# marqo-ai/marqo

Hardware: AMD Instinct MI355X
Metric: embeddings/sec (higher is better)
Workload: dtype bf16; 1 GPU; open_clip ViT-B/32 image tower, uint8 224x224 resident in HBM (tower-only), batch 256/GPU; global_batch=256, parallelism=dp1 (replicated weights, sharded items, RCCL all_gather of embeddings), weights=random-init (seed 0) ViT-B-32, last_block_rows=pooled

## Files before the change

### include/marqo_hip.h

```cpp
#ifndef MARQO_HIP_H
#define MARQO_HIP_H

#include <stddef.h>
#include <stdint.h>

#ifdef __cplusplus
extern "C" {
#endif

#define MQ_OK 0
#define MQ_ERR_INVALID (-1)
#define MQ_ERR_HIP (-2)
#define MQ_ERR_WORKSPACE (-3)
#define MQ_ERR_UNSUPPORTED (-4)

#define MQ_ABI_VERSION 15

#define MQ_ACT_NONE 0
#define MQ_ACT_GELU 1
#define MQ_ACT_QUICKGELU 2
#define MQ_ACT_SILU 3
#define MQ_ACT_RELU 4

#define MQ_MASK_NONE 0
// ... 8 lines not shown

#define MQ_VIT_POOL_CLS 0
#define MQ_VIT_POOL_MAP 1
#define MQ_VIT_POOL_AVG 2
#define MQ_VIT_POOL_QUERY 3

#define MQ_EPI_BIAS 1
#define MQ_EPI_GELU 2
#define MQ_EPI_QUICKGELU 4
#define MQ_EPI_RESIDUAL 8
#define MQ_EPI_OUT_F32 16
#define MQ_EPI_OUT_FP8 32


typedef struct mq_block_weights {
    const float* ln1_g; const float* ln1_b;
    const void*  qkv_w; const float* qkv_b;
    const void*  out_w; const float* out_b;
    const float* ln2_g; const float* ln2_b;
    const void*  fc1_w; const float* fc1_b;
    const void*  fc2_w; const float* fc2_b;
    const void*  qkv_w8; const float* qkv_ws;
    const void*  out_w8; const float* out_ws;
    const void*  fc1_w8; const float* fc1_ws;
    const void*  fc2_w8; const float* fc2_ws;
    const void*  qkv_wf; const float* qkv_sf; const float* qkv_bf;
    const void*  fc1_wf; const float* fc1_sf; const float* fc1_bf;
    const float* attn_ln_g; const float* attn_ln_b;
    const float* mlp_ln_g;  const float* mlp_ln_b;
    const void*  out_wf; const float* out_sf; const float* out_bf;
    const void*  fc2_wf; const float* fc2_sf; const float* fc2_bf;
} mq_block_weights;

typedef struct mq_encoder_cfg {
    int32_t width;
    int32_t layers;
    int32_t heads;
    int32_t mlp_dim;
    int32_t act;
    int32_t post_ln;
    int32_t mask;
    float   ln_eps;
    int32_t precision;
    int32_t attn_width;
    int32_t fp8_first_layer;
    int32_t mlp_glu;
    const float* d_fp8_act_scale;
    float*       d_fp8_act_amax;
    const float* d_rope_inv_freq;
    const float* d_rel_bias;
    int32_t      rel_span;
    int32_t      residual_stream;
    int32_t      fp8_mlp_extra;
    int32_t      rope_prefix;
    const float* d_rope_table;
    int32_t      mlp_ln_dim;
    int32_t      reserved2;
} mq_encoder_cfg;


typedef struct mq_map_head {
    const float* q;
    const void*  kv_w;   const float* kv_b;
    const void*  proj_w; const float* proj_b;
    const float* ln_g;   const float* ln_b;
    const void*  fc1_w;  const float* fc1_b;
    const void*  fc2_w;  const float* fc2_b;
} mq_map_head;

typedef struct mq_vit_weights {
    const void*  patch_w;
    const float* cls;
    const float* pos;
    const float* ln_pre_g; const float* ln_pre_b;
    const mq_block_weights* blocks;
    const float* ln_post_g; const float* ln_post_b;
    const void*  proj_w;
    const mq_map_head* map;
    const float* proj_b;
} mq_vit_weights;

typedef struct mq_vit_cfg {
    mq_encoder_cfg enc;
    int32_t image_size;
    int32_t patch_size;
    int32_t out_dim;
    float mean[3];
    float std[3];
    int32_t pool;
    int32_t map_mlp_dim;
    int32_t pool_dim;
    int32_t pool_heads;
} mq_vit_cfg;

typedef struct mq_clip_text_weights {
    const float* tok_emb;
    const float* pos;
    const mq_block_weights* blocks;
    const float* ln_final_g; const float* ln_final_b;
    const void*  proj_w;
    const float* proj_b;
} mq_clip_text_weights;

typedef struct mq_clip_text_cfg {
    mq_encoder_cfg enc;
    int32_t vocab;
    int32_t ctx;
    int32_t out_dim;
    int32_t cls_pos;
} mq_clip_text_cfg;

typedef struct mq_bert_weights {
    const float* word_emb;
    const float* pos_emb;
    const float* type_emb;
    const float* emb_ln_g; const float* emb_ln_b;
    const mq_block_weights* blocks;
    const void*  proj1_w;
    const float* proj1_b;
    const void*  proj2_w;
} mq_bert_weights;

typedef struct mq_bert_cfg {
    mq_encoder_cfg enc;
    int32_t vocab;
    int32_t max_pos;
    int32_t pool;
    int32_t proj_hidden;
    int32_t out_dim;
} mq_bert_cfg;

int         mq_abi_version(void);
const char* mq_last_error(void);
const char* mq_build_arch(void);
int mq_check_device(int device);

int mq_host_gather(const void* const* h_src, const int64_t* h_bytes, const int64_t* h_dst_off, int64_t n, void* h_dst, int32_t threads);
int mq_host_gather_checked(const void* const* h_src, const int64_t* h_bytes, const int64_t* h_dst_off, int64_t n, void* h_dst,
                           int64_t dst_bytes, int32_t threads);

size_t mq_encoder_workspace_bytes(const mq_encoder_cfg* cfg, int64_t rows, int64_t nseq);
size_t mq_vit_workspace_bytes(const mq_vit_cfg* cfg, int64_t n_images);
size_t mq_clip_text_workspace_bytes(const mq_clip_text_cfg* cfg, int64_t rows, int64_t nseq);
size_t mq_bert_workspace_bytes(const mq_bert_cfg* cfg, int64_t rows, int64_t nseq);


int mq_encode_image_u8(const mq_vit_cfg* cfg, const mq_vit_weights* w,
                       const uint8_t* d_pixels, int64_t n, float* d_out, int normalize,
                       void* d_workspace, size_t workspace_bytes, void* stream);

int mq_encode_image_f32(const mq_vit_cfg* cfg, const mq_vit_weights* w,
                        const float* d_pixels, int64_t n, float* d_out, int normalize,
                        void* d_workspace, size_t workspace_bytes, void* stream);

int mq_encode_clip_text(const mq_clip_text_cfg* cfg, const mq_clip_text_weights* w,
                        const int32_t* d_ids, const int32_t* d_cu_seqlens,
                        const int32_t* h_cu_seqlens, int64_t nseq,
                        const int32_t* d_pool_rows,
                        float* d_out, int normalize,
                        void* d_workspace, size_t workspace_bytes, void* stream);

int mq_encode_bert(const mq_bert_cfg* cfg, const mq_bert_weights* w,
                   const int32_t* d_ids, const int32_t* d_cu_seqlens,
                   const int32_t* h_cu_seqlens, int64_t nseq,
                   float* d_out, int normalize,
                   void* d_workspace, size_t workspace_bytes, void* stream);


size_t mq_clip_resize_workspace_bytes(const int32_t* h_heights, const int32_t* h_widths, int64_t n, int32_t S);
int mq_clip_resize_crop_u8(const uint8_t* d_src, const int64_t* h_src_off, const int32_t* h_heights,
                           const int32_t* h_widths, int64_t n, int32_t S, uint8_t* d_out,
                           void* d_workspace, size_t workspace_bytes, void* stream);

size_t mq_resize_workspace_bytes(const int32_t* h_heights, const int32_t* h_widths, int64_t n, int32_t out_h, int32_t out_w);
int mq_resize_u8(const uint8_t* d_src, const int64_t* h_src_off, const int32_t* h_heights, const int32_t* h_widths,
                 int64_t n, int32_t out_h, int32_t out_w, uint8_t* d_out, void* d_workspace, size_t workspace_bytes,
                 void* stream);

size_t mq_resize_filter_workspace_bytes(const int32_t* h_heights, const int32_t* h_widths, int64_t n, int32_t out_h, int32_t out_w,
                                        int32_t filter);
int mq_resize_filter_u8(const uint8_t* d_src, const int64_t* h_src_off, const int32_t* h_heights, const int32_t* h_widths,
                        int64_t n, int32_t out_h, int32_t out_w, int32_t filter, uint8_t* d_out, void* d_workspace,
                        size_t workspace_bytes, void* stream);

int    mq_chunk_grid_count(int32_t hn, int32_t wn, int32_t overlap);
size_t mq_chunk_grid_workspace_bytes(const int32_t* h_heights, const int32_t* h_widths, int64_t n,
                                     int32_t hn, int32_t wn, int32_t overlap, int32_t S);
int mq_chunk_grid_u8(const uint8_t* d_src, const int64_t* h_src_off, const int32_t* h_heights,
                     const int32_t* h_widths, int64_t n, int32_t hn, int32_t wn, int32_t overlap, int32_t S,
                     uint8_t* d_out, float* h_boxes, void* d_workspace, size_t workspace_bytes, void* stream);

#define MQ_IMG_RGB 0
#define MQ_IMG_NEAREST 1
#define MQ_IMG_RGBA 2
size_t mq_resize_mode_workspace_bytes(const int32_t* h_heights, const int32_t* h_widths, int64_t n, int32_t out_h, int32_t out_w,
                                      int32_t filter, int32_t crop, int32_t mode);
int mq_resize_mode_u8(const uint8_t* d_src, const int64_t* h_src_off, const int32_t* h_heights, const int32_t* h_widths, int64_t n,
                      int32_t out_h, int32_t out_w, int32_t filter, int32_t crop, int32_t mode, uint8_t* d_out,
                      void* d_workspace, size_t workspace_bytes, void* stream);

int mq_unpack_rgbx(const uint8_t* d_staging, int64_t jobs_off, int64_t n, int64_t max_npix, uint8_t* d_rgb, void* stream);

int mq_to_tensor_normalize(const uint8_t* d_u8, float* d_out, int64_t n, int32_t S,
                           const float* mean, const float* std, void* stream);

int mq_resample_ksize(int32_t in_size, int32_t out_size);
int mq_resample_coeffs(int32_t in_size, int32_t out_size, int32_t first, int32_t count,
                       int32_t* h_bounds, int32_t* h_kk);


int mq_gemm_fp8(const void* d_A8, int64_t lda, const void* d_W8, int64_t ldw, const float* d_a_scale,
                int a_scale_per_row, const float* d_w_scale, const float* d_bias, const float* d_residual,
                void* d_out, int64_t ldc, const float* d_out_scale, float* d_amax,
                int64_t M, int64_t N, int64_t K, int flags, void* stream);

int mq_quantize_weights_fp8(const void* d_W_bf16, int64_t ldw, void* d_W8, int64_t ld8, float* d_scale,
                            int64_t N, int64_t K, void* stream);

int mq_layernorm_fp8(const float* d_x, const float* d_g, const float* d_b, void* d_out_fp8, float* d_row_scale,
                     float* d_out_f32 ,
                     int64_t rows, int32_t W, float eps, void* stream);

int mq_layernorm_fp8_ex(const void* d_x, int x_bf16, const float* d_g, const float* d_b, void* d_out_fp8, float* d_row_scale,
                        float* d_out_f32, int64_t rows, int32_t W, float eps, void* stream);

int mq_rowquant_fp8(const float* d_x, void* d_out_fp8, float* d_row_scale, int64_t rows, int32_t W, void* stream);

int mq_gemm_bf16(const void* d_A, int64_t lda, const void* d_W, int64_t ldw,
                 const float* d_bias, const float* d_residual, void* d_out, int64_t ldc,
                 int64_t M, int64_t N, int64_t K, int flags, void* stream);

int mq_gemm_small_bf16(const void* d_A, int64_t lda, const void* d_W, int64_t ldw, const float* d_bias, const void* d_residual,
                       void* d_out, int64_t ldc, int64_t M, int64_t N, int64_t K, int flags, void* stream);
int mq_ln_gemm_small_bf16(const void* d_x, int64_t ldx, int x_bf16, const float* d_ln_g, const float* d_ln_b, float eps, const void* d_W,
                          int64_t ldw, const float* d_bias, void* d_out, int64_t ldc, int64_t M, int64_t N, int64_t K, int flags,
                          float* d_ln_out, void* stream);

#define MQ_EPI_ROW_STATS 64
#define MQ_EPI_LN_APPLY 128
#define MQ_EPI_GLU 256
#define MQ_EPI_RELU 512
int mq_gemm_bf16_rs(const void* d_A, int64_t lda, const void* d_W, int64_t ldw, const float* d_bias, const void* d_residual, void* d_out, int64_t ldc,
                    int64_t M, int64_t N, int64_t K, int flags, float* d_partials, void* stream);
int mq_row_stats_finalize(const float* d_partials, int32_t nslots, float* d_stats, int64_t rows, int32_t W, float eps, void* stream);
int mq_gemm_bf16_lnrs(const void* d_A, int64_t lda, const void* d_W, int64_t ldw, const float* d_bias, const float* d_colsum, const float* d_rowstats,
                      const void* d_residual, void* d_out, int64_t ldc, int64_t M, int64_t N, int64_t K, int flags, float* d_partials, void* stream);
int mq_attention_stats(const void* d_qkv, void* d_out, const int32_t* d_cu_seqlens, int64_t nseq, int32_t fixed_len, int32_t max_len, int32_t W,
                       int32_t heads, int32_t mask, float* d_row_part, int64_t rows, void* stream);
int mq_attention_proj_ok(int64_t nseq, int32_t fixed_len, int32_t W, int32_t heads);
int mq_attention_proj(const void* d_qkv, const void* d_w, const float* d_bias, void* d_x, float* d_rowstats, int64_t nseq, int32_t fixed_len, int32_t W,
                      int32_t heads, float eps, const void* d_pf_a, size_t pf_a_bytes, const void* d_pf_b, size_t pf_b_bytes, void* stream);
int mq_panel_gemm_ln_ok(int64_t nseq, int32_t fixed_len, int64_t N, int64_t K);
int mq_panel_gemm_ln(const void* d_x, const void* d_W, const float* d_bias, const float* d_colsum, const float* d_rowstats, void* d_out, int64_t ldc,
                     int64_t nseq, int32_t fixed_len, int64_t N, int64_t K, int flags, void* stream);
int64_t mq_gemm_band_counters(int64_t M);
int mq_gemm_bf16_rsf(const void* d_A, int64_t lda, const void* d_W, int64_t ldw, const float* d_bias, const void* d_residual, void* d_out, int64_t ldc,
                     int64_t M, int64_t N, int64_t K, int flags, float* d_partials, float* d_stats, float eps, uint32_t* d_band_ctr,
                     const void* d_pf_a, size_t pf_a_bytes, const void* d_pf_b, size_t pf_b_bytes, void* stream);
int mq_row_stats(const void* d_x_bf16, float* d_stats, int64_t rows, int32_t W, float eps, void* stream);
int mq_gemm_bf16_ln(const void* d_A, int64_t lda, const void* d_W, int64_t ldw, const float* d_bias, const float* d_colsum, const float* d_rowstats,
                    void* d_out, int64_t ldc, int64_t M, int64_t N, int64_t K, int flags, void* stream);

int mq_layernorm(const float* d_x, const int32_t* d_row_idx, const float* d_g, const float* d_b,
                 void* d_out_bf16, float* d_out_f32, int64_t rows, int32_t W, float eps, void* stream);
int mq_layernorm_ex(const void* d_x, int x_bf16, const int32_t* d_row_idx, const float* d_g, const float* d_b,
                    void* d_out_bf16, float* d_out_f32, int64_t rows, int32_t W, float eps, void* stream);

int mq_attention(const void* d_qkv, void* d_out, const int32_t* d_cu_seqlens, int64_t nseq,
                 int32_t fixed_len, int32_t max_len, int32_t W, int32_t heads, int32_t mask,
                 void* stream);

int mq_attention_bias(const void* d_qkv, void* d_out, const int32_t* d_cu_seqlens, int64_t nseq, int32_t fixed_len,
                      int32_t max_len, int32_t W, int32_t heads, const float* d_rel_bias, int32_t rel_span, void* stream);

int mq_attention_ex(const void* d_qkv, void* d_out, const int32_t* d_cu_seqlens, int64_t nseq,
                    int32_t fixed_len, int32_t max_len, int32_t W, int32_t heads, int32_t mask,
                    int32_t out_fp8, const float* d_out_scale, float* d_amax, void* stream);

int mq_encoder_forward(const mq_encoder_cfg* cfg, const mq_block_weights* blocks,
                       float* d_x, int64_t rows, const int32_t* d_cu_seqlens, int64_t nseq,
                       int32_t fixed_len, int32_t max_len,
                       void* d_workspace, size_t workspace_bytes, void* stream);

int mq_encoder_forward_rows(const mq_encoder_cfg* cfg, const mq_block_weights* blocks,
                            float* d_x, int64_t rows, const int32_t* d_cu_seqlens, int64_t nseq,
                            int32_t fixed_len, int32_t max_len,
                            const int32_t* d_out_rows, int64_t n_out_rows,
                            void* d_workspace, size_t workspace_bytes, void* stream);

int mq_l2_normalize(const float* d_x, float* d_out, int64_t rows, int32_t D, void* stream);

int mq_patchify(const void* d_in, int32_t is_u8, void* d_out, int64_t n, int32_t S, int32_t P, int32_t Kp, const float* mean, const float* std,
                void* stream);
int mq_vit_assemble(const float* d_patch_out, const float* d_cls, const float* d_pos, const float* d_g, const float* d_b, void* d_x, int64_t n,
                    int32_t T, int32_t W, float eps, int32_t x_bf16, void* stream);
int mq_embed_tokens(const int32_t* d_ids, const int32_t* d_cu, int64_t nseq, const float* d_tok, const float* d_pos, const float* d_type0,
                    const float* d_g, const float* d_b, float* d_x, void* d_xb, int32_t W, int32_t vocab, float eps, int32_t last_pos, void* stream);
int mq_pool(const float* d_x, const int32_t* d_cu, int64_t nseq, float* d_out, int32_t W, int32_t pool, int32_t normalize, void* stream);
int mq_map_pool(const void* d_kv, const float* d_q, void* d_out, int64_t n, int32_t T, int32_t W, int32_t heads, void* stream);
int mq_avg_tokens(const void* d_x, int32_t x_bf16, float* d_out, int64_t n, int32_t T, int32_t first, int32_t W, void* stream);
int mq_move_rows(void* d_sparse, const int32_t* d_idx, void* d_dense, int64_t n, int64_t row_bytes, int32_t scatter, void* stream);
int mq_last_rows(const int32_t* d_cu, int32_t* d_rows, int64_t nseq, void* stream);
int mq_cls_rows(int32_t* d_rows, int64_t n, int32_t T, void* stream);
int mq_rope(void* d_qkv, const int32_t* d_cu, int64_t nseq, int32_t fixed_len, int32_t Wa, int32_t heads, const float* d_inv_freq, void* stream);
int mq_rope_table(void* d_qkv, int64_t rows, int32_t T, int32_t prefix, int32_t Wa, int32_t heads, const float* d_table, void* stream);
int mq_glu(void* d_buf, int64_t rows, int32_t F, int32_t act, int32_t interleaved, void* stream);
// ... 727 lines not shown
```

### marqo_amd/_lib.py

```python
from __future__ import annotations

import ctypes as C
import os
import re
import subprocess
import sys
import sysconfig
import threading
from typing import Optional
from pathlib import Path

PKG_DIR = Path(__file__).resolve().parent
CSRC_DIR = PKG_DIR / "csrc"
LIB_DIR = PKG_DIR / "lib"
LIB_PATH = Path(os.environ["MARQO_AMD_LIB"]) if os.environ.get("MARQO_AMD_LIB") else LIB_DIR / "libmarqo_hip.so"
HEADER_PATH = PKG_DIR.parent / "include" / "marqo_hip.h"
TORCH_OPS_SRC = CSRC_DIR / "torch_ops.cpp"
TORCH_OPS_PATH = LIB_DIR / "libmarqo_torch_ops.so"
STAGE_SRC = CSRC_DIR / "py_stage.cpp"
STAGE_PATH = LIB_DIR / "_mq_stage.so"

MQ_OK = 0
NO_SCRATCH_UNITS = ("rowops", "gemm_bf16", "gemm_wd", "gemm_fp8", "gemm_small", "attention", "attention_window", "attention_gqa", "attention_gqa256", "attention_gqa256_causal", "attention_relbias", "attention_alibi", "attention_disentangled", "attention_full", "lora", "attn_proj", "panel_gemm", "embed", "convnext", "resnet", "patch_attn", "rerank", "owl_head", "temporal", "audio", "video")
ABI_VERSION = 15
MQ_PREC_BF16, MQ_PREC_FP8 = 0, 1
MQ_ACT_GELU, MQ_ACT_QUICKGELU, MQ_ACT_SILU, MQ_ACT_RELU = 1, 2, 3, 4
MQ_MASK_NONE, MQ_MASK_CAUSAL, MQ_MASK_CAUSAL_CLS = 0, 1, 2
MQ_POOL_MEAN, MQ_POOL_CLS, MQ_POOL_LAST = 0, 1, 2
MQ_VIT_POOL_CLS, MQ_VIT_POOL_MAP, MQ_VIT_POOL_AVG, MQ_VIT_POOL_QUERY = 0, 1, 2, 3
MQ_EPI_BIAS, MQ_EPI_GELU, MQ_EPI_QUICKGELU, MQ_EPI_RESIDUAL, MQ_EPI_OUT_F32, MQ_EPI_OUT_FP8 = 1, 2, 4, 8, 16, 32
MQ_EPI_ROW_STATS, MQ_EPI_LN_APPLY = 64, 128
MQ_COMBINE_RAW, MQ_COMBINE_NORMALIZE, MQ_COMBINE_NORMALIZE_IF_NONZERO = 0, 1, 2
MQ_IMG_RGB, MQ_IMG_NEAREST, MQ_IMG_RGBA = 0, 1, 2
MQ_PROF_FAMILIES = 6
MQ_FBANK_WS_BYTES = 2048
MQ_RESAMPLE_MAX_TAPS = 1 << 21
PROF_FAMILY_NAMES = ("gemm", "layernorm", "attention", "embed", "pool_head", "preprocess")


class MarqoHipUnavailableError(RuntimeError):
    """The HIP extension is missing / unloadable.  There is deliberately no fallback."""


class MarqoHipError(RuntimeError):
    """A libmarqo_hip entry point returned an error code."""


class BlockWeights(C.Structure):
    _fields_ = [(n, C.c_void_p) for n in (
        "ln1_g", "ln1_b", "qkv_w", "qkv_b", "out_w", "out_b",
        "ln2_g", "ln2_b", "fc1_w", "fc1_b", "fc2_w", "fc2_b",
        "qkv_w8", "qkv_ws", "out_w8", "out_ws", "fc1_w8", "fc1_ws", "fc2_w8", "fc2_ws",
        "qkv_wf", "qkv_sf", "qkv_bf", "fc1_wf", "fc1_sf", "fc1_bf",
        "attn_ln_g", "attn_ln_b", "mlp_ln_g", "mlp_ln_b",
        "out_wf", "out_sf", "out_bf", "fc2_wf", "fc2_sf", "fc2_bf")]


class EncoderCfg(C.Structure):
    _fields_ = [("width", C.c_int32), ("layers", C.c_int32), ("heads", C.c_int32), ("mlp_dim", C.c_int32),
                ("act", C.c_int32), ("post_ln", C.c_int32), ("mask", C.c_int32), ("ln_eps", C.c_float),
                ("precision", C.c_int32), ("attn_width", C.c_int32), ("fp8_first_layer", C.c_int32), ("mlp_glu", C.c_int32),
                ("d_fp8_act_scale", C.c_void_p), ("d_fp8_act_amax", C.c_void_p), ("d_rope_inv_freq", C.c_void_p),
                ("d_rel_bias", C.c_void_p), ("rel_span", C.c_int32), ("residual_stream", C.c_int32),
                ("fp8_mlp_extra", C.c_int32), ("rope_prefix", C.c_int32), ("d_rope_table", C.c_void_p), ("mlp_ln_dim", C.c_int32),
                ("reserved2", C.c_int32)]


class MapHead(C.Structure):
    _fields_ = [("q", C.c_void_p), ("kv_w", C.c_void_p), ("kv_b", C.c_void_p), ("proj_w", C.c_void_p), ("proj_b", C.c_void_p),
                ("ln_g", C.c_void_p), ("ln_b", C.c_void_p), ("fc1_w", C.c_void_p), ("fc1_b", C.c_void_p),
                ("fc2_w", C.c_void_p), ("fc2_b", C.c_void_p)]


class VitWeights(C.Structure):
    _fields_ = [("patch_w", C.c_void_p), ("cls", C.c_void_p), ("pos", C.c_void_p),
                ("ln_pre_g", C.c_void_p), ("ln_pre_b", C.c_void_p), ("blocks", C.POINTER(BlockWeights)),
                ("ln_post_g", C.c_void_p), ("ln_post_b", C.c_void_p), ("proj_w", C.c_void_p), ("map", C.POINTER(MapHead)),
                ("proj_b", C.c_void_p)]


class VitCfg(C.Structure):
    _fields_ = [("enc", EncoderCfg), ("image_size", C.c_int32), ("patch_size", C.c_int32), ("out_dim", C.c_int32),
                ("mean", C.c_float * 3), ("std", C.c_float * 3), ("pool", C.c_int32), ("map_mlp_dim", C.c_int32), ("pool_dim", C.c_int32),
                ("pool_heads", C.c_int32)]


class ClipTextWeights(C.Structure):
    _fields_ = [("tok_emb", C.c_void_p), ("pos", C.c_void_p), ("blocks", C.POINTER(BlockWeights)),
                ("ln_final_g", C.c_void_p), ("ln_final_b", C.c_void_p), ("proj_w", C.c_void_p), ("proj_b", C.c_void_p)]


class ClipTextCfg(C.Structure):
    _fields_ = [("enc", EncoderCfg), ("vocab", C.c_int32), ("ctx", C.c_int32), ("out_dim", C.c_int32), ("cls_pos", C.c_int32)]


class BertWeights(C.Structure):
    _fields_ = [("word_emb", C.c_void_p), ("pos_emb", C.c_void_p), ("type_emb", C.c_void_p),
                ("emb_ln_g", C.c_void_p), ("emb_ln_b", C.c_void_p), ("blocks", C.POINTER(BlockWeights)),
                ("proj1_w", C.c_void_p), ("proj1_b", C.c_void_p), ("proj2_w", C.c_void_p)]


class BertCfg(C.Structure):
    _fields_ = [("enc", EncoderCfg), ("vocab", C.c_int32), ("max_pos", C.c_int32), ("pool", C.c_int32),
                ("proj_hidden", C.c_int32), ("out_dim", C.c_int32)]


class ConvNextCfg(C.Structure):
    _fields_ = [("image_size", C.c_int32), ("depths", C.c_int32 * 4), ("dims", C.c_int32 * 4), ("ln_eps", C.c_float), ("head", C.c_int32),
                ("out_dim", C.c_int32), ("mean", C.c_float * 3), ("std", C.c_float * 3)]


class ConvNextBlockWeights(C.Structure):
    _fields_ = [(n, C.c_void_p) for n in ("dw_w", "dw_b", "fc1_w", "fc1_b", "fc1_s", "fc2_w", "fc2_b")]


class ConvNextWeights(C.Structure):
    _fields_ = [("stem_w", C.c_void_p), ("stem_b", C.c_void_p), ("stem_ln_g", C.c_void_p), ("stem_ln_b", C.c_void_p),
                ("ds_ln_g", C.c_void_p * 4), ("ds_ln_b", C.c_void_p * 4), ("ds_w", C.c_void_p * 4), ("ds_b", C.c_void_p * 4),
                ("blocks", C.POINTER(ConvNextBlockWeights)), ("head_ln_g", C.c_void_p), ("head_ln_b", C.c_void_p),
                ("proj_w", C.c_void_p), ("proj_b", C.c_void_p), ("proj2_w", C.c_void_p), ("proj2_b", C.c_void_p)]


MQ_CONVNEXT_HEAD_LINEAR, MQ_CONVNEXT_HEAD_MLP = 0, 1
MQ_EPI_RELU = 512


class ResNetCfg(C.Structure):
    _fields_ = [("image_size", C.c_int32), ("layers", C.c_int32 * 4), ("width", C.c_int32), ("heads", C.c_int32), ("out_dim", C.c_int32),
                ("mean", C.c_float * 3), ("std", C.c_float * 3)]


class ResNetBlockWeights(C.Structure):
    _fields_ = [(n, C.c_void_p) for n in ("conv1_w", "conv1_b", "conv2_w", "conv2_b", "conv3_w", "conv3_b", "ds_w", "ds_b")]


class ResNetWeights(C.Structure):
    _fields_ = [("stem_w", C.c_void_p * 3), ("stem_b", C.c_void_p * 3), ("blocks", C.POINTER(ResNetBlockWeights)), ("pos", C.c_void_p),
                ("q_w", C.c_void_p), ("q_b", C.c_void_p), ("kv_w", C.c_void_p), ("kv_b", C.c_void_p), ("c_w", C.c_void_p), ("c_b", C.c_void_p)]


class WordPieceVocab(C.Structure):
    _fields_ = [("d_slots", C.c_void_p), ("d_pool", C.c_void_p), ("n_slots", C.c_uint32), ("unk_id", C.c_int32), ("cls_id", C.c_int32),
                ("sep_id", C.c_int32), ("pad_id", C.c_int32), ("lower", C.c_int32), ("max_word_chars", C.c_int32), ("d_unicode", C.c_void_p)]


class ClipBpeVocab(C.Structure):
    _fields_ = [("d_slots", C.c_void_p), ("d_byte_id", C.c_void_p), ("d_byte_end_id", C.c_void_p), ("n_slots", C.c_uint32),
                ("sot_id", C.c_int32), ("eot_id", C.c_int32), ("lower", C.c_int32), ("d_unicode", C.c_void_p)]


class ByteBpeVocab(C.Structure):
    _fields_ = [("d_slots", C.c_void_p), ("d_byte_id", C.c_void_p), ("d_unicode", C.c_void_p), ("n_slots", C.c_uint32), ("cls_id", C.c_int32),
                ("sep_id", C.c_int32), ("pad_id", C.c_int32)]


class SentencePieceVocab(C.Structure):
    _fields_ = [("d_slots", C.c_void_p), ("d_pool", C.c_void_p), ("d_score", C.c_void_p), ("d_nmap", C.c_void_p), ("d_npool", C.c_void_p),
                ("d_ccc", C.c_void_p), ("n_slots", C.c_uint32), ("unk_id", C.c_int32), ("unk_score", C.c_float), ("add_dummy_prefix", C.c_int32),
                ("remove_extra_ws", C.c_int32), ("max_piece_bytes", C.c_int32), ("prefix_id", C.c_int32), ("suffix_id", C.c_int32),
                ("pad_id", C.c_int32), ("id_offset", C.c_int32), ("unk_out", C.c_int32)]


class QueueCfg(C.Structure):
    _fields_ = [("kind", C.c_int32), ("device", C.c_int32), ("max_seqs", C.c_int32), ("max_rows", C.c_int32), ("normalize", C.c_int32),
                ("depth", C.c_int32), ("window_us", C.c_int32), ("graphs", C.c_int32), ("helper_seqs", C.c_int32), ("reserved", C.c_int32)]


class QueueStats(C.Structure):
    _fields_ = [("requests", C.c_uint64), ("calls", C.c_uint64), ("merged_calls", C.c_uint64), ("failed_calls", C.c_uint64),
                ("sequences", C.c_uint64), ("rows", C.c_uint64), ("max_call_sequences", C.c_uint64), ("graphs", C.c_uint64), ("graph_replays", C.c_uint64)]


QUEUE_CLIP_TEXT, QUEUE_BERT, QUEUE_IMAGE_F32 = 0, 1, 2


class ScoreHeadWeights(C.Structure):
# ... 6 lines not shown


class ModernBertWeights(C.Structure):
    _fields_ = [("tok_emb", C.c_void_p), ("emb_ln_g", C.c_void_p), ("final_ln_g", C.c_void_p), ("zeros", C.c_void_p), ("d_inv_freq_global", C.c_void_p),
                ("d_inv_freq_local", C.c_void_p), ("layers", C.POINTER(ModernBertLayer))]


class ModernBertCfg(C.Structure):
    _fields_ = [("width", C.c_int32), ("layers", C.c_int32), ("heads", C.c_int32), ("mlp_dim", C.c_int32), ("vocab", C.c_int32), ("max_pos", C.c_int32),
                ("half_window", C.c_int32), ("pool", C.c_int32), ("ln_eps", C.c_float), ("reserved", C.c_int32)]


class ScoreHeadLnWeights(C.Structure):
    _fields_ = [("dense_w", C.c_void_p), ("dense_b", C.c_void_p), ("norm_g", C.c_void_p), ("norm_b", C.c_void_p), ("cls_w", C.c_void_p),
                ("cls_b", C.c_float), ("ln_eps", C.c_float)]


class QwenLayer(C.Structure):
    _fields_ = [(n, C.c_void_p) for n in ("input_norm_g", "qkv_w", "qkv_b", "q_norm_g", "k_norm_g", "out_w", "post_norm_g", "ug_w", "down_w")]


class QwenWeights(C.Structure):
    _fields_ = [("tok_emb", C.c_void_p), ("final_norm_g", C.c_void_p), ("zeros", C.c_void_p), ("d_inv_freq", C.c_void_p), ("layers", C.POINTER(QwenLayer))]


class QwenCfg(C.Structure):
    _fields_ = [("width", C.c_int32), ("layers", C.c_int32), ("q_heads", C.c_int32), ("kv_heads", C.c_int32), ("head_dim", C.c_int32), ("mlp_dim", C.c_int32),
                ("vocab", C.c_int32), ("max_pos", C.c_int32), ("pool", C.c_int32), ("rms_eps", C.c_float)]


class GemmaLayer(C.Structure):
    _fields_ = [(n, C.c_void_p) for n in ("input_norm_g", "qkv_w", "q_norm_g", "k_norm_g", "out_w", "post_attn_norm_g", "pre_ffn_norm_g", "ug_w", "down_w",
                                          "post_ffn_norm_g")] + [("sliding", C.c_int32), ("reserved", C.c_int32)]


class GemmaWeights(C.Structure):
    _fields_ = [("tok_emb", C.c_void_p), ("final_norm_g", C.c_void_p), ("d_inv_freq_global", C.c_void_p), ("d_inv_freq_local", C.c_void_p),
                ("layers", C.POINTER(GemmaLayer))]


class GemmaCfg(C.Structure):
    _fields_ = [("width", C.c_int32), ("layers", C.c_int32), ("q_heads", C.c_int32), ("kv_heads", C.c_int32), ("head_dim", C.c_int32), ("mlp_dim", C.c_int32),
                ("vocab", C.c_int32), ("max_pos", C.c_int32), ("half_window", C.c_int32), ("pool", C.c_int32), ("rms_eps", C.c_float), ("attn_scale", C.c_float)]


class GemmaCausalLayer(C.Structure):
    _fields_ = [(n, C.c_void_p) for n in ("input_norm_g", "qkv_w", "out_w", "post_norm_g", "ug_w", "down_w")]


class GemmaCausalWeights(C.Structure):
    _fields_ = [("tok_emb", C.c_void_p), ("final_norm_g", C.c_void_p), ("zeros", C.c_void_p), ("d_inv_freq", C.c_void_p),
                ("layers", C.POINTER(GemmaCausalLayer))]


class GemmaCausalCfg(C.Structure):
    _fields_ = [("width", C.c_int32), ("layers", C.c_int32), ("q_heads", C.c_int32), ("kv_heads", C.c_int32), ("head_dim", C.c_int32), ("mlp_dim", C.c_int32),
                ("vocab", C.c_int32), ("max_pos", C.c_int32), ("rms_eps", C.c_float), ("attn_scale", C.c_float)]


class T5Layer(C.Structure):
    _fields_ = [(n, C.c_void_p) for n in ("attn_norm_g", "qkv_w", "out_w", "ff_norm_g", "wi_w", "wo_w")]


class T5Weights(C.Structure):
    _fields_ = [("tok_emb", C.c_void_p), ("final_norm_g", C.c_void_p), ("zeros", C.c_void_p), ("d_rel_bias", C.c_void_p), ("layers", C.POINTER(T5Layer))]


class T5Cfg(C.Structure):
    _fields_ = [("width", C.c_int32), ("layers", C.c_int32), ("heads", C.c_int32), ("head_dim", C.c_int32), ("mlp_dim", C.c_int32), ("vocab", C.c_int32),
                ("max_pos", C.c_int32), ("pool", C.c_int32), ("max_distance", C.c_int32), ("gated", C.c_int32), ("rms_eps", C.c_float), ("reserved", C.c_int32)]


class JinaBertLayer(C.Structure):
    _fields_ = [(n, C.c_void_p) for n in ("qkv_w", "qkv_b", "out_w", "out_b", "attn_ln_g", "attn_ln_b", "wg_w", "wo_w", "wo_b", "mlp_ln_g", "mlp_ln_b")]


class JinaBertWeights(C.Structure):
    _fields_ = [("tok_emb", C.c_void_p), ("type0", C.c_void_p), ("emb_ln_g", C.c_void_p), ("emb_ln_b", C.c_void_p), ("d_slopes", C.c_void_p),
                ("layers", C.POINTER(JinaBertLayer))]


class JinaBertCfg(C.Structure):
    _fields_ = [("width", C.c_int32), ("layers", C.c_int32), ("heads", C.c_int32), ("head_dim", C.c_int32), ("mlp_dim", C.c_int32), ("vocab", C.c_int32),
                ("max_pos", C.c_int32), ("pool", C.c_int32), ("ln_eps", C.c_float), ("reserved", C.c_int32)]


class DebertaLayer(C.Structure):
    _fields_ = [(n, C.c_void_p) for n in ("qkv_w", "qkv_b", "out_w", "out_b", "attn_ln_g", "attn_ln_b", "fc1_w", "fc1_b", "fc2_w", "fc2_b", "mlp_ln_g",
                                          "mlp_ln_b", "pos_key", "pos_query")]


class DebertaWeights(C.Structure):
    _fields_ = [("tok_emb", C.c_void_p), ("emb_ln_g", C.c_void_p), ("emb_ln_b", C.c_void_p), ("d_idx", C.c_void_p), ("h_idx", C.c_void_p),
                ("layers", C.POINTER(DebertaLayer))]


class DebertaCfg(C.Structure):
    _fields_ = [("width", C.c_int32), ("layers", C.c_int32), ("heads", C.c_int32), ("head_dim", C.c_int32), ("mlp_dim", C.c_int32), ("vocab", C.c_int32),
                ("max_pos", C.c_int32), ("pool", C.c_int32), ("span", C.c_int32), ("reach", C.c_int32), ("ln_eps", C.c_float), ("reserved", C.c_int32)]


class NomicBertLayer(C.Structure):
    _fields_ = [(n, C.c_void_p) for n in ("qkv_w", "out_w", "attn_ln_g", "attn_ln_b", "ug_w", "down_w", "mlp_ln_g", "mlp_ln_b")]


class NomicBertWeights(C.Structure):
    _fields_ = [("tok_emb", C.c_void_p), ("type0", C.c_void_p), ("emb_ln_g", C.c_void_p), ("emb_ln_b", C.c_void_p), ("zeros", C.c_void_p),
                ("d_inv_freq", C.c_void_p), ("layers", C.POINTER(NomicBertLayer))]


class NomicBertCfg(C.Structure):
    _fields_ = [("width", C.c_int32), ("layers", C.c_int32), ("heads", C.c_int32), ("head_dim", C.c_int32), ("mlp_dim", C.c_int32), ("vocab", C.c_int32),
                ("max_pos", C.c_int32), ("pool", C.c_int32), ("ln_eps", C.c_float), ("reserved", C.c_int32)]


MQ_LORA_ACCUM, MQ_LORA_WRITE, MQ_LORA_INPLACE = 0, 1, 2


class JinaV3Layer(C.Structure):
    _fields_ = [(n, C.c_void_p) for n in ("qkv_w", "qkv_b", "out_w", "out_b", "attn_ln_g", "attn_ln_b", "fc1_w", "fc1_b", "fc2_w", "fc2_b", "mlp_ln_g",
                                          "mlp_ln_b")]


class JinaV3Weights(C.Structure):
    _fields_ = [("tok_emb", C.c_void_p), ("type0", C.c_void_p), ("emb_ln_g", C.c_void_p), ("emb_ln_b", C.c_void_p), ("d_inv_freq", C.c_void_p),
                ("layers", C.POINTER(JinaV3Layer))]


class JinaV3LoraLayer(C.Structure):
    _fields_ = [(n, C.c_void_p) for n in ("qkv_a", "qkv_b", "out_a", "out_b", "fc1_a", "fc1_b", "fc2_a", "fc2_b")]


class JinaV3Lora(C.Structure):
    _fields_ = [("tasks", C.c_int32), ("rank", C.c_int32), ("d_scale", C.c_void_p), ("emb_a", C.c_void_p), ("emb_b", C.c_void_p),
                ("layers", C.POINTER(JinaV3LoraLayer))]


class JinaV3Cfg(C.Structure):
    _fields_ = [("width", C.c_int32), ("layers", C.c_int32), ("heads", C.c_int32), ("head_dim", C.c_int32), ("mlp_dim", C.c_int32), ("vocab", C.c_int32),
                ("max_pos", C.c_int32), ("pool", C.c_int32), ("ln_eps", C.c_float), ("reserved", C.c_int32)]


_P = C.c_void_p
_SIGNATURES = {
    "mq_abi_version": (C.c_int, []),
    "mq_last_error": (C.c_char_p, []),
    "mq_build_arch": (C.c_char_p, []),
    "mq_encoder_workspace_bytes": (C.c_size_t, [C.POINTER(EncoderCfg), C.c_int64, C.c_int64]),
    "mq_vit_workspace_bytes": (C.c_size_t, [C.POINTER(VitCfg), C.c_int64]),
    "mq_clip_text_workspace_bytes": (C.c_size_t, [C.POINTER(ClipTextCfg), C.c_int64, C.c_int64]),
    "mq_bert_workspace_bytes": (C.c_size_t, [C.POINTER(BertCfg), C.c_int64, C.c_int64]),
    "mq_encode_image_u8": (C.c_int, [C.POINTER(VitCfg), C.POINTER(VitWeights), _P, C.c_int64, _P, C.c_int, _P, C.c_size_t, _P]),
    "mq_encode_image_f32": (C.c_int, [C.POINTER(VitCfg), C.POINTER(VitWeights), _P, C.c_int64, _P, C.c_int, _P, C.c_size_t, _P]),
    "mq_encode_clip_text": (C.c_int, [C.POINTER(ClipTextCfg), C.POINTER(ClipTextWeights), _P, _P, _P, C.c_int64, _P, _P,
                                      C.c_int, _P, C.c_size_t, _P]),
    "mq_encode_bert": (C.c_int, [C.POINTER(BertCfg), C.POINTER(BertWeights), _P, _P, _P, C.c_int64, _P, C.c_int, _P,
                                 C.c_size_t, _P]),
    "mq_gemm_bf16": (C.c_int, [_P, C.c_int64, _P, C.c_int64, _P, _P, _P, C.c_int64, C.c_int64, C.c_int64, C.c_int64,
                               C.c_int, _P]),
    "mq_gemm_small_bf16": (C.c_int, [_P, C.c_int64, _P, C.c_int64, _P, _P, _P, C.c_int64, C.c_int64, C.c_int64, C.c_int64, C.c_int, _P]),
    "mq_ln_gemm_small_bf16": (C.c_int, [_P, C.c_int64, C.c_int, _P, _P, C.c_float, _P, C.c_int64, _P, _P, C.c_int64, C.c_int64, C.c_int64,
                                        C.c_int64, C.c_int, _P, _P]),
    "mq_gemm_bf16_ln": (C.c_int, [_P, C.c_int64, _P, C.c_int64, _P, _P, _P, _P, C.c_int64, C.c_int64, C.c_int64, C.c_int64, C.c_int, _P]),
    "mq_row_stats": (C.c_int, [_P, _P, C.c_int64, C.c_int32, C.c_float, _P]),
    "mq_row_stats_finalize": (C.c_int, [_P, C.c_int32, _P, C.c_int64, C.c_int32, C.c_float, _P]),
    "mq_gemm_bf16_lnrs": (C.c_int, [_P, C.c_int64, _P, C.c_int64, _P, _P, _P, _P, _P, C.c_int64, C.c_int64, C.c_int64, C.c_int64, C.c_int, _P, _P]),
    "mq_attention_stats": (C.c_int, [_P, _P, _P, C.c_int64, C.c_int32, C.c_int32, C.c_int32, C.c_int32, C.c_int32, _P, C.c_int64, _P]),
    "mq_attention_proj_ok": (C.c_int, [C.c_int64, C.c_int32, C.c_int32, C.c_int32]),
    "mq_panel_gemm_ln_ok": (C.c_int, [C.c_int64, C.c_int32, C.c_int64, C.c_int64]),
    "mq_panel_gemm_ln": (C.c_int, [_P, _P, _P, _P, _P, _P, C.c_int64, C.c_int64, C.c_int32, C.c_int64, C.c_int64, C.c_int, _P]),
    "mq_attention_proj": (C.c_int, [_P, _P, _P, _P, _P, C.c_int64, C.c_int32, C.c_int32, C.c_int32, C.c_float, _P, C.c_size_t, _P, C.c_size_t, _P]),
    "mq_gemm_bf16_rs": (C.c_int, [_P, C.c_int64, _P, C.c_int64, _P, _P, _P, C.c_int64, C.c_int64, C.c_int64, C.c_int64, C.c_int, _P, _P]),
    "mq_check_device": (C.c_int, [C.c_int]),
    "mq_gemm_band_counters": (C.c_int64, [C.c_int64]),
    "mq_gemm_bf16_rsf": (C.c_int, [_P, C.c_int64, _P, C.c_int64, _P, _P, _P, C.c_int64, C.c_int64, C.c_int64, C.c_int64, C.c_int, _P, _P, C.c_float, _P,
                                   _P, C.c_size_t, _P, C.c_size_t, _P]),
    "mq_gemm_fp8": (C.c_int, [_P, C.c_int64, _P, C.c_int64, _P, C.c_int, _P, _P, _P, _P, C.c_int64, _P, _P, C.c_int64, C.c_int64,
                              C.c_int64, C.c_int, _P]),
    "mq_quantize_weights_fp8": (C.c_int, [_P, C.c_int64, _P, C.c_int64, _P, C.c_int64, C.c_int64, _P]),
    "mq_layernorm_fp8": (C.c_int, [_P, _P, _P, _P, _P, _P, C.c_int64, C.c_int32, C.c_float, _P]),
    "mq_layernorm_fp8_ex": (C.c_int, [_P, C.c_int, _P, _P, _P, _P, _P, C.c_int64, C.c_int32, C.c_float, _P]),
    "mq_rowquant_fp8": (C.c_int, [_P, _P, _P, C.c_int64, C.c_int32, _P]),
    "mq_layernorm": (C.c_int, [_P, _P, _P, _P, _P, _P, C.c_int64, C.c_int32, C.c_float, _P]),
    "mq_layernorm_ex": (C.c_int, [_P, C.c_int, _P, _P, _P, _P, _P, C.c_int64, C.c_int32, C.c_float, _P]),
    "mq_attention_ex": (C.c_int, [_P, _P, _P, C.c_int64, C.c_int32, C.c_int32, C.c_int32, C.c_int32, C.c_int32, C.c_int32, _P, _P, _P]),
    "mq_attention_bias": (C.c_int, [_P, _P, _P, C.c_int64, C.c_int32, C.c_int32, C.c_int32, C.c_int32, _P, C.c_int32, _P]),
    "mq_attention": (C.c_int, [_P, _P, _P, C.c_int64, C.c_int32, C.c_int32, C.c_int32, C.c_int32, C.c_int32, _P]),
    "mq_encoder_forward": (C.c_int, [C.POINTER(EncoderCfg), C.POINTER(BlockWeights), _P, C.c_int64, _P, C.c_int64,
                                     C.c_int32, C.c_int32, _P, C.c_size_t, _P]),
    "mq_encoder_forward_rows": (C.c_int, [C.POINTER(EncoderCfg), C.POINTER(BlockWeights), _P, C.c_int64, _P, C.c_int64,
                                          C.c_int32, C.c_int32, _P, C.c_int64, _P, C.c_size_t, _P]),
    "mq_l2_normalize": (C.c_int, [_P, _P, C.c_int64, C.c_int32, _P]),
    "mq_clip_resize_workspace_bytes": (C.c_size_t, [_P, _P, C.c_int64, C.c_int32]),
    "mq_clip_resize_crop_u8": (C.c_int, [_P, _P, _P, _P, C.c_int64, C.c_int32, _P, _P, C.c_size_t, _P]),
    "mq_resize_workspace_bytes": (C.c_size_t, [_P, _P, C.c_int64, C.c_int32, C.c_int32]),
    "mq_resize_u8": (C.c_int, [_P, _P, _P, _P, C.c_int64, C.c_int32, C.c_int32, _P, _P, C.c_size_t, _P]),
    "mq_resize_filter_workspace_bytes": (C.c_size_t, [_P, _P, C.c_int64, C.c_int32, C.c_int32, C.c_int32]),
    "mq_resize_filter_u8": (C.c_int, [_P, _P, _P, _P, C.c_int64, C.c_int32, C.c_int32, C.c_int32, _P, _P, C.c_size_t, _P]),
    "mq_resize_mode_workspace_bytes": (C.c_size_t, [_P, _P, C.c_int64, C.c_int32, C.c_int32, C.c_int32, C.c_int32, C.c_int32]),
    "mq_resize_mode_u8": (C.c_int, [_P, _P, _P, _P, C.c_int64, C.c_int32, C.c_int32, C.c_int32, C.c_int32, C.c_int32, _P, _P, C.c_size_t, _P]),
    "mq_chunk_grid_count": (C.c_int, [C.c_int32, C.c_int32, C.c_int32]),
    "mq_chunk_grid_workspace_bytes": (C.c_size_t, [_P, _P, C.c_int64, C.c_int32, C.c_int32, C.c_int32, C.c_int32]),
    "mq_chunk_grid_u8": (C.c_int, [_P, _P, _P, _P, C.c_int64, C.c_int32, C.c_int32, C.c_int32, C.c_int32, _P, _P, _P,
                                   C.c_size_t, _P]),
    "mq_host_gather": (C.c_int, [_P, _P, _P, C.c_int64, _P, C.c_int32]),
    "mq_host_gather_checked": (C.c_int, [_P, _P, _P, C.c_int64, _P, C.c_int64, C.c_int32]),
    "mq_unpack_rgbx": (C.c_int, [_P, C.c_int64, C.c_int64, C.c_int64, _P, _P]),
    "mq_to_tensor_normalize": (C.c_int, [_P, _P, C.c_int64, C.c_int32, C.POINTER(C.c_float), C.POINTER(C.c_float), _P]),
    "mq_resample_ksize": (C.c_int, [C.c_int32, C.c_int32]),
    "mq_resample_coeffs": (C.c_int, [C.c_int32, C.c_int32, C.c_int32, C.c_int32, _P, _P]),
    "mq_tokenize_workspace_bytes": (C.c_size_t, [C.c_int64, C.c_int64, C.c_int32]),
    "mq_tokenize_wordpiece": (C.c_int, [C.POINTER(WordPieceVocab), _P, _P, C.c_int64, C.c_int64, C.c_int32, _P, C.c_int64, _P, _P, _P,
                                        C.c_size_t, _P]),
    "mq_tokenize_clip_bpe": (C.c_int, [C.POINTER(ClipBpeVocab), _P, _P, C.c_int64, C.c_int64, C.c_int32, _P, _P, _P, _P, C.c_size_t, _P]),
    "mq_tokenize_byte_bpe": (C.c_int, [C.POINTER(ByteBpeVocab), _P, _P, C.c_int64, C.c_int64, C.c_int32, _P, C.c_int64, _P, _P, _P, C.c_size_t, _P]),
    "mq_tokenize_sentencepiece_workspace_bytes": (C.c_size_t, [C.c_int64, C.c_int64, C.c_int32]),
    "mq_tokenize_sentencepiece": (C.c_int, [C.POINTER(SentencePieceVocab), _P, _P, C.c_int64, C.c_int64, C.c_int32, _P, C.c_int64, _P, _P, _P,
                                            C.c_size_t, _P]),
    "mq_tokenize_sentencepiece_bpe": (C.c_int, [C.POINTER(SentencePieceVocab), _P, _P, C.c_int64, C.c_int64, C.c_int32, _P, C.c_int64, _P, _P, _P,
                                                C.c_size_t, _P]),
    "mq_pack_ids": (C.c_int, [_P, C.c_int64, _P, C.c_int64, _P, _P]),
    "mq_weighted_combine": (C.c_int, [_P, C.c_int64, _P, _P, _P, C.c_int64, C.c_int32, C.c_int32, _P, _P]),
    "mq_queue_create": (C.c_int, [C.POINTER(QueueCfg), _P, _P, C.POINTER(_P)]),
    "mq_queue_encode": (C.c_int, [_P, _P, _P, C.c_int64, _P]),
    "mq_queue_encode_images": (C.c_int, [_P, _P, C.c_int64, _P]),
    "mq_queue_get_stats": (C.c_int, [_P, C.POINTER(QueueStats)]),
    "mq_queue_destroy": (C.c_int, [_P]),
    "mq_convnext_workspace_bytes": (C.c_size_t, [C.POINTER(ConvNextCfg), C.c_int64]),
    "mq_encode_convnext_u8": (C.c_int, [C.POINTER(ConvNextCfg), C.POINTER(ConvNextWeights), _P, C.c_int64, _P, C.c_int, _P, C.c_size_t, _P]),
    "mq_encode_convnext_f32": (C.c_int, [C.POINTER(ConvNextCfg), C.POINTER(ConvNextWeights), _P, C.c_int64, _P, C.c_int, _P, C.c_size_t, _P]),
    "mq_convnext_dwconv": (C.c_int, [_P, _P, _P, _P, _P, C.c_int64, C.c_int32, C.c_int32, C.c_int32, _P]),
    "mq_convnext_downsample": (C.c_int, [_P, _P, _P, _P, _P, C.c_int64, C.c_int32, C.c_int32, C.c_int32, _P]),
    "mq_convnext_pool_ln": (C.c_int, [_P, _P, _P, _P, _P, C.c_int64, C.c_int32, C.c_int32, C.c_float, _P]),
    "mq_resnet_workspace_bytes": (C.c_size_t, [C.POINTER(ResNetCfg), C.c_int64]),
    "mq_encode_resnet_u8": (C.c_int, [C.POINTER(ResNetCfg), C.POINTER(ResNetWeights), _P, C.c_int64, _P, C.c_int, _P, C.c_size_t, _P]),
    "mq_encode_resnet_f32": (C.c_int, [C.POINTER(ResNetCfg), C.POINTER(ResNetWeights), _P, C.c_int64, _P, C.c_int, _P, C.c_size_t, _P]),
    "mq_resnet_conv3x3": (C.c_int, [_P, _P, _P, _P, C.c_int64, C.c_int64, C.c_int32, C.c_int32, C.c_int32, C.c_int32, C.c_int32, _P]),
    "mq_resnet_stem_gather": (C.c_int, [_P, C.c_int32, _P, C.c_int64, C.c_int32, _P, _P, _P]),
    "mq_resnet_avgpool2": (C.c_int, [_P, _P, C.c_int64, C.c_int32, C.c_int32, C.c_int32, _P]),
    "mq_resnet_attnpool_tokens": (C.c_int, [_P, _P, _P, C.c_int64, C.c_int32, C.c_int32, _P]),
    "mq_resnet_attnpool_attend": (C.c_int, [_P, _P, _P, C.c_int64, C.c_int32, C.c_int32, _P]),
    "mq_attention_cls_probs": (C.c_int, [_P, _P, C.c_int64, C.c_int32, C.c_int32, C.c_int32, _P]),
    "mq_attn_boxes": (C.c_int, [_P, C.c_int64, C.c_int32, C.c_int32, C.c_int32, _P, _P, C.c_int32, _P]),
    "mq_patchify": (C.c_int, [_P, C.c_int32, _P, C.c_int64, C.c_int32, C.c_int32, C.c_int32, _P, _P, _P]),
    "mq_vit_assemble": (C.c_int, [_P, _P, _P, _P, _P, _P, C.c_int64, C.c_int32, C.c_int32, C.c_float, C.c_int32, _P]),
    "mq_embed_tokens": (C.c_int, [_P, _P, C.c_int64, _P, _P, _P, _P, _P, _P, _P, C.c_int32, C.c_int32, C.c_float, C.c_int32, _P]),
    "mq_pool": (C.c_int, [_P, _P, C.c_int64, _P, C.c_int32, C.c_int32, C.c_int32, _P]),
    "mq_map_pool": (C.c_int, [_P, _P, _P, C.c_int64, C.c_int32, C.c_int32, C.c_int32, _P]),
    "mq_avg_tokens": (C.c_int, [_P, C.c_int32, _P, C.c_int64, C.c_int32, C.c_int32, C.c_int32, _P]),
    "mq_move_rows": (C.c_int, [_P, _P, _P, C.c_int64, C.c_int64, C.c_int32, _P]),
    "mq_last_rows": (C.c_int, [_P, _P, C.c_int64, _P]),
    "mq_cls_rows": (C.c_int, [_P, C.c_int64, C.c_int32, _P]),
    "mq_rope": (C.c_int, [_P, _P, C.c_int64, C.c_int32, C.c_int32, C.c_int32, _P, _P]),
    "mq_rope_table": (C.c_int, [_P, C.c_int64, C.c_int32, C.c_int32, C.c_int32, C.c_int32, _P, _P]),
    "mq_glu": (C.c_int, [_P, C.c_int64, C.c_int32, C.c_int32, C.c_int32, _P]),
    "mq_glu_ln": (C.c_int, [_P, C.c_int64, C.c_int32, C.c_int32, C.c_int32, _P, _P, C.c_float, C.c_int32, _P]),
    "mq_pair_plan": (C.c_int, [C.c_int32, _P, C.c_int64, C.c_int32, C.c_int32, _P, _P, _P, _P]),
    "mq_pair_plan_n": (C.c_int, [C.c_int32, _P, C.c_int64, C.c_int32, C.c_int32, C.c_int32, _P, _P, _P, _P]),
    "mq_pack_pairs_xlmr": (C.c_int, [_P, C.c_int32, _P, C.c_int32, _P, _P, _P, C.c_int64, C.c_int32, C.c_int32, _P, C.c_int64, _P]),
    "mq_pack_pairs": (C.c_int, [_P, C.c_int32, _P, C.c_int32, _P, _P, _P, C.c_int64, C.c_int32, C.c_int32, _P, _P, C.c_int64, _P]),
    "mq_embed_tokens_typed": (C.c_int, [_P, _P, _P, C.c_int64, _P, _P, _P, C.c_int32, _P, _P, _P, _P, C.c_int32, C.c_int32, C.c_float, C.c_int32, _P]),
    "mq_score_head_workspace_bytes": (C.c_size_t, [C.c_int64, C.c_int32]),
    "mq_score_head": (C.c_int, [_P, C.c_int64, C.c_int32, C.POINTER(ScoreHeadWeights), _P, _P, _P, C.c_size_t, _P]),
    "mq_score_pairs_workspace_bytes": (C.c_size_t, [C.POINTER(BertCfg), C.c_int64, C.c_int64]),
    "mq_score_pairs_bert": (C.c_int, [C.POINTER(BertCfg), C.POINTER(BertWeights), C.POINTER(ScoreHeadWeights), _P, _P, _P, _P, C.c_int64, _P, _P, _P,
                                      _P, C.c_size_t, _P]),
    "mq_score_pairs_xlmr": (C.c_int, [C.POINTER(BertCfg), C.POINTER(BertWeights), C.POINTER(ScoreHeadWeights), _P, _P, _P, C.c_int64, _P, _P, _P, _P,
                                      C.c_size_t, _P]),
    "mq_owl_merge_ln": (C.c_int, [_P, _P, _P, _P, _P, _P, _P, C.c_int64, C.c_int32, C.c_int32, C.c_float, _P]),
    "mq_owl_class_head": (C.c_int, [_P, _P, _P, _P, C.c_int32, _P, C.c_float, _P, C.c_float, _P, _P, _P, C.c_int64, C.c_int32, C.c_int32, C.c_int32,
                                    C.c_int32, _P]),
    "mq_owl_box_head": (C.c_int, [_P, _P, _P, _P, _P, C.c_int64, C.c_int32, C.c_int32, C.c_float, C.c_float, _P]),
    "mq_owl_topk": (C.c_int, [_P, _P, C.c_int64, C.c_int32, C.c_int32, _P, _P, _P, _P]),
    "mq_temporal_embed_ln": (C.c_int, [_P, _P, _P, _P, _P, C.c_int64, C.c_int32, C.c_int32, C.c_int32, C.c_float, _P]),
    "mq_temporal_attention": (C.c_int, [_P, _P, C.c_int64, C.c_int32, C.c_int32, C.c_int32, C.c_int32, _P]),
    "mq_patchify_clip": (C.c_int, [_P, _P, C.c_int64, C.c_int32, C.c_int32, C.c_int32, C.c_int32, _P]),
    "mq_fbank": (C.c_int, [_P, C.c_int64, C.c_int64, C.c_int32, C.c_int32, _P, _P, _P]),
    "mq_mel_fusion": (C.c_int, [_P, C.c_int64, C.c_int32, C.c_int64, C.c_int64, C.c_int64, C.c_float, C.c_float, _P, C.c_int32, _P]),
    "mq_patchify_rect": (C.c_int, [_P, _P, C.c_int64, C.c_int32, C.c_int32, C.c_int32, C.c_int32, _P]),
    "mq_video_preprocess": (C.c_int, [_P, C.c_int64, C.c_int32, C.c_int32, _P, C.c_int32, C.c_int32, C.c_int32, C.c_int32, C.c_int32, C.c_int32,
                                      C.POINTER(C.c_float), C.POINTER(C.c_float), C.c_int32, _P, _P]),
    "mq_resample": (C.c_int, [_P, C.c_int64, C.c_int64, _P, C.c_int32, C.c_int32, C.c_int32, _P, _P]),
    "mq_attention_window": (C.c_int, [_P, _P, _P, C.c_int64, C.c_int32, C.c_int32, C.c_int32, C.c_int32, C.c_int32, _P]),
    "mq_modernbert_workspace_bytes": (C.c_size_t, [C.POINTER(ModernBertCfg), C.c_int64, C.c_int64]),
    "mq_encode_modernbert": (C.c_int, [C.POINTER(ModernBertCfg), C.POINTER(ModernBertWeights), _P, _P, _P, C.c_int64, _P, C.c_int, _P, C.c_size_t, _P]),
    "mq_score_head_ln_workspace_bytes": (C.c_size_t, [C.c_int64, C.c_int32]),
    "mq_score_head_ln": (C.c_int, [_P, C.c_int64, C.c_int32, C.POINTER(ScoreHeadLnWeights), _P, _P, _P, C.c_size_t, _P]),
    "mq_score_pairs_modernbert_workspace_bytes": (C.c_size_t, [C.POINTER(ModernBertCfg), C.c_int64, C.c_int64]),
    "mq_score_pairs_modernbert": (C.c_int, [C.POINTER(ModernBertCfg), C.POINTER(ModernBertWeights), C.POINTER(ScoreHeadLnWeights), _P, _P, _P, C.c_int64,
                                            _P, _P, _P, _P, C.c_size_t, _P]),
    "mq_attention_gqa": (C.c_int, [_P, _P, _P, C.c_int64, C.c_int32, C.c_int32, C.c_int32, C.c_int32, C.c_int32, C.c_int32, _P]),
    "mq_rmsnorm": (C.c_int, [_P, _P, _P, _P, _P, C.c_int64, C.c_int32, C.c_float, _P]),
    "mq_qk_norm_rope": (C.c_int, [_P, _P, C.c_int64, C.c_int32, C.c_int32, C.c_int32, C.c_int32, _P, _P, C.c_float, _P, _P]),
    "mq_qwen_workspace_bytes": (C.c_size_t, [C.POINTER(QwenCfg), C.c_int64, C.c_int64]),
    "mq_encode_qwen": (C.c_int, [C.POINTER(QwenCfg), C.POINTER(QwenWeights), _P, _P, _P, C.c_int64, _P, C.c_int, _P, C.c_size_t, _P]),
    "mq_attention_gqa_prefix": (C.c_int, [_P, _P, _P, C.c_int64, C.c_int32, C.c_int32, C.c_int32, C.c_int32, C.c_int32, _P]),
    "mq_qk_norm_rope_at": (C.c_int, [_P, _P, C.c_int64, C.c_int32, C.c_int32, C.c_int32, C.c_int32, _P, _P, C.c_float, _P, C.c_int32, _P]),
    "mq_score_dot": (C.c_int, [_P, _P, C.c_int64, C.c_int32, _P, _P, _P]),
    "mq_score_qwen_pairs_workspace_bytes": (C.c_size_t, [C.POINTER(QwenCfg), C.c_int64, C.c_int64]),
    "mq_score_qwen_pairs": (C.c_int, [C.POINTER(QwenCfg), C.POINTER(QwenWeights), _P, _P, _P, _P, C.c_int64, C.c_int32, _P, _P, _P, C.c_size_t, _P]),
    "mq_attention_gqa_band": (C.c_int, [_P, _P, _P, C.c_int64, C.c_int32, C.c_int32, C.c_int32, C.c_int32, C.c_int32, C.c_int32, C.c_float, _P]),
    "mq_rmsnorm_add_norm": (C.c_int, [_P, _P, _P, _P, _P, C.c_int64, C.c_int32, C.c_float, _P]),
    "mq_glu_tanh": (C.c_int, [_P, C.c_int64, C.c_int32, _P]),
    "mq_gemma_workspace_bytes": (C.c_size_t, [C.POINTER(GemmaCfg), C.c_int64, C.c_int64]),
    "mq_encode_gemma": (C.c_int, [C.POINTER(GemmaCfg), C.POINTER(GemmaWeights), _P, _P, _P, C.c_int64, _P, C.c_int, _P, C.c_size_t, _P]),
    "mq_attention_relbias": (C.c_int, [_P, _P, _P, C.c_int64, C.c_int32, C.c_int32, C.c_int32, C.c_int32, _P, C.c_int32, C.c_float, _P]),
# ... 291 lines not shown
```

### marqo_amd/csrc/knobs.h

```cpp
#pragma once
#include <atomic>
#include <stdint.h>

typedef std::atomic<int> mq_knob;

struct GemmTune { mq_knob mt, cgroup, nh, fp8_big, tail, wd, rs_fin; };
extern GemmTune g_tune;
extern std::atomic<uint64_t> mq_gemm_addr_limit;

extern mq_knob mq_tower_row_select, mq_tower_ln_fold, mq_tower_subln_fold, mq_tower_attn_proj, mq_tower_panel_gemm, mq_tower_residual_bf16,
    mq_tower_pool_strided, mq_tower_assemble_stats;
extern mq_knob mq_gemm_small_max_rows, mq_gemm_small_group_rows;
extern mq_knob mq_ln_prefetch, mq_ln_rows_per_wave, mq_ln_bf16_wide;
extern mq_knob mq_xcd_band;
extern mq_knob mq_attention_waves;
```

### marqo_amd/csrc/knobs.hip

```cpp
#include <stdlib.h>
#include <string.h>
#include "common.h"
#include "knobs.h"

GemmTune g_tune;
std::atomic<uint64_t> mq_gemm_addr_limit{0xffffffffull};
mq_knob mq_tower_row_select, mq_tower_ln_fold, mq_tower_subln_fold, mq_tower_attn_proj, mq_tower_panel_gemm, mq_tower_residual_bf16,
    mq_tower_pool_strided, mq_tower_assemble_stats;
mq_knob mq_gemm_small_max_rows, mq_gemm_small_group_rows;
mq_knob mq_ln_prefetch, mq_ln_rows_per_wave, mq_ln_bf16_wide;
mq_knob mq_xcd_band;
mq_knob mq_attention_waves;

namespace {

struct Knob { const char* key; const char* env; int def; mq_knob* var; };
const Knob g_knobs[] = {
    {"gemm_mt", "MQ_GEMM_MT", 0, &g_tune.mt},
    {"gemm_cgroup", "MQ_GEMM_CGROUP", 8, &g_tune.cgroup},
    {"gemm_nh", "MQ_GEMM_NH", 0, &g_tune.nh},
    {nullptr, "MQ_GEMM_FP8_NH", 0, &g_tune.fp8_big},
    {"gemm_tail", "MQ_GEMM_TAIL", 0, &g_tune.tail},
    {"gemm_wd", "MQ_GEMM_WD", 0, &g_tune.wd},
    {"rs_finalize", "MQ_GEMM_RS_FIN", 0, &g_tune.rs_fin},
    {"row_select", "MQ_ROW_SELECT", 1, &mq_tower_row_select},
    {"ln_fold", "MQ_LN_FOLD", 2, &mq_tower_ln_fold},
    {"subln_fold", "MQ_SUBLN_FOLD", 1, &mq_tower_subln_fold},
    {"attn_proj", "MQ_ATTN_PROJ", 128, &mq_tower_attn_proj},
    {"panel_gemm", "MQ_PANEL_GEMM", 0, &mq_tower_panel_gemm},
    {"residual_bf16", "MQ_RESIDUAL_BF16", 0, &mq_tower_residual_bf16},
    {"pool_strided", "MQ_POOL_STRIDED", 1, &mq_tower_pool_strided},
    {"assemble_stats", "MQ_ASSEMBLE_STATS", 1, &mq_tower_assemble_stats},
    {"small_m", "MQ_SMALL_M", 80, &mq_gemm_small_max_rows},
    {"small_m_grouped", "MQ_SMALL_M_GROUPED", 320, &mq_gemm_small_group_rows},
    {"ln_prefetch", "MQ_LN_PREFETCH", 1, &mq_ln_prefetch},
    {"ln_rows", "MQ_LN_ROWS", 2, &mq_ln_rows_per_wave},
    {"ln_bf16_wide", "MQ_LN_BF16_WIDE", 1, &mq_ln_bf16_wide},
    {"xcd_band", "MQ_XCD_BAND", 1, &mq_xcd_band},
    {"attn_waves", nullptr, 0, &mq_attention_waves},
    {"gemm_addr_limit_mb", nullptr, 0, nullptr},
};

const bool g_knobs_from_env = [] {
    for (const Knob& k : g_knobs) {
        const char* v = k.env ? getenv(k.env) : nullptr;
        if (k.var) *k.var = v ? atoi(v) : k.def;
    }
    return true;
}();

const Knob* find_knob(const char* who, const char* key) {
    for (const Knob& k : g_knobs)
        if (key && k.key && !strcmp(k.key, key)) return &k;
    mq_set_error("%s: unknown key %s", who, key ? key : "(null)");
    return nullptr;
}

}

extern "C" int mq_tune(const char* key, int value) {
    const Knob* k = find_knob("mq_tune", key);
    if (!k) return MQ_ERR_INVALID;
    if (k->var) *k->var = value;
    else mq_gemm_addr_limit = value > 0 ? ((uint64_t)value << 20) - 1 : 0xffffffffull;
    if (k->var == &g_tune.nh) g_tune.fp8_big = value == 4 ? 0 : value;
    return MQ_OK;
}

extern "C" int mq_tune_get(const char* key, int* value) {
    const Knob* k = find_knob("mq_tune_get", key);
    if (!k) return MQ_ERR_INVALID;
    MQ_CHECK_ARG(value, "mq_tune_get: null value");
    const uint64_t lim = mq_gemm_addr_limit;
    *value = k->var ? (int)*k->var : lim == 0xffffffffull ? 0 : (int)((lim + 1) >> 20);
    return MQ_OK;
}
```

### marqo_amd/csrc/torch_ops.cpp

```cpp
#include <Python.h>
#include <stdlib.h>

#include <ATen/ATen.h>
#include <c10/hip/HIPStream.h>
#include <torch/library.h>

#include "../../include/marqo_hip.h"

namespace {

void* stream_of(const at::Tensor& t) {
    return (void*)c10::hip::getCurrentHIPStream(t.device().index()).stream();
}

const bool g_release_gil = [] { const char* v = getenv("MARQO_AMD_OPS_RELEASE_GIL"); return v && v[0] == '1'; }();
struct NoGil {
    PyThreadState* st;
    NoGil() : st(g_release_gil && Py_IsInitialized() && PyGILState_Check() ? PyEval_SaveThread() : nullptr) {}
    ~NoGil() { if (st) PyEval_RestoreThread(st); }
    NoGil(const NoGil&) = delete;
    NoGil& operator=(const NoGil&) = delete;
};

void check_rc(int rc, const char* what) {
    TORCH_CHECK(rc == MQ_OK, "marqo_hip::", what, " failed (", rc, "): ", mq_last_error());
}

void need_dev(const at::Tensor& t, at::ScalarType dt, const char* name) {
    TORCH_CHECK(t.is_cuda(), "marqo_hip: ", name, " must live on the GPU (there is no CPU path)");
    TORCH_CHECK(t.scalar_type() == dt, "marqo_hip: ", name, " must be ", dt, ", got ", t.scalar_type());
    TORCH_CHECK(t.is_contiguous(), "marqo_hip: ", name, " must be contiguous");
}

template <typename T>
const T* blob(const at::Tensor& t, const char* name) {
    TORCH_CHECK(t.device().is_cpu() && t.scalar_type() == at::kByte && t.is_contiguous() && (size_t)t.numel() == sizeof(T),
                "marqo_hip: ", name, " must be a CPU uint8 tensor of ", sizeof(T), " bytes (the ", name, " struct of include/marqo_hip.h)");
    return (const T*)t.data_ptr();
}

void encode_image_u8(const at::Tensor& cfg, const at::Tensor& weights, const at::Tensor& pixels, at::Tensor out, bool normalize,
                     at::Tensor workspace) {
    need_dev(pixels, at::kByte, "pixels");
    need_dev(out, at::kFloat, "out");
    need_dev(workspace, at::kByte, "workspace");
    TORCH_CHECK(pixels.dim() == 4 && out.dim() == 2 && out.size(0) == pixels.size(0), "marqo_hip::encode_image_u8: pixels [n,S,S,3], out [n,D]");
    NoGil nogil;
    check_rc(mq_encode_image_u8(blob<mq_vit_cfg>(cfg, "mq_vit_cfg"), blob<mq_vit_weights>(weights, "mq_vit_weights"),
                                (const uint8_t*)pixels.data_ptr(), pixels.size(0), (float*)out.data_ptr(), normalize ? 1 : 0,
                                workspace.data_ptr(), (size_t)workspace.numel(), stream_of(pixels)), "encode_image_u8");
}

void encode_image_f32(const at::Tensor& cfg, const at::Tensor& weights, const at::Tensor& pixels, at::Tensor out, bool normalize,
                      at::Tensor workspace) {
    need_dev(pixels, at::kFloat, "pixels");
    need_dev(out, at::kFloat, "out");
    need_dev(workspace, at::kByte, "workspace");
    TORCH_CHECK(pixels.dim() == 4 && out.dim() == 2 && out.size(0) == pixels.size(0), "marqo_hip::encode_image_f32: pixels [n,3,S,S], out [n,D]");
    NoGil nogil;
    check_rc(mq_encode_image_f32(blob<mq_vit_cfg>(cfg, "mq_vit_cfg"), blob<mq_vit_weights>(weights, "mq_vit_weights"),
                                 (const float*)pixels.data_ptr(), pixels.size(0), (float*)out.data_ptr(), normalize ? 1 : 0,
                                 workspace.data_ptr(), (size_t)workspace.numel(), stream_of(pixels)), "encode_image_f32");
}

void check_packed(const at::Tensor& ids, const at::Tensor& cu, const at::Tensor& cu_host, const at::Tensor& out) {
    need_dev(ids, at::kInt, "ids");
    need_dev(cu, at::kInt, "cu_seqlens");
    need_dev(out, at::kFloat, "out");
    TORCH_CHECK(cu_host.device().is_cpu() && cu_host.scalar_type() == at::kInt && cu_host.is_contiguous() && cu_host.numel() == cu.numel(),
                "marqo_hip: cu_seqlens_host must be the CPU int32 copy of cu_seqlens");
    TORCH_CHECK(cu.numel() >= 1 && out.dim() == 2 && out.size(0) == cu.numel() - 1, "marqo_hip: out must be [nseq, D] with nseq = len(cu_seqlens) - 1");
}

void encode_clip_text(const at::Tensor& cfg, const at::Tensor& weights, const at::Tensor& ids, const at::Tensor& cu,
                      const at::Tensor& cu_host, const c10::optional<at::Tensor>& pool_rows, at::Tensor out, bool normalize,
                      at::Tensor workspace) {
    check_packed(ids, cu, cu_host, out);
    need_dev(workspace, at::kByte, "workspace");
    const int32_t* pr = nullptr;
    if (pool_rows.has_value()) {
        need_dev(*pool_rows, at::kInt, "pool_rows");
        pr = (const int32_t*)pool_rows->data_ptr();
    }
    NoGil nogil;
    check_rc(mq_encode_clip_text(blob<mq_clip_text_cfg>(cfg, "mq_clip_text_cfg"), blob<mq_clip_text_weights>(weights, "mq_clip_text_weights"),
                                 (const int32_t*)ids.data_ptr(), (const int32_t*)cu.data_ptr(), (const int32_t*)cu_host.data_ptr(),
                                 cu.numel() - 1, pr, (float*)out.data_ptr(), normalize ? 1 : 0, workspace.data_ptr(),
                                 (size_t)workspace.numel(), stream_of(ids)), "encode_clip_text");
}

void encode_bert(const at::Tensor& cfg, const at::Tensor& weights, const at::Tensor& ids, const at::Tensor& cu, const at::Tensor& cu_host,
                 at::Tensor out, bool normalize, at::Tensor workspace) {
    check_packed(ids, cu, cu_host, out);
    need_dev(workspace, at::kByte, "workspace");
    NoGil nogil;
    check_rc(mq_encode_bert(blob<mq_bert_cfg>(cfg, "mq_bert_cfg"), blob<mq_bert_weights>(weights, "mq_bert_weights"),
                            (const int32_t*)ids.data_ptr(), (const int32_t*)cu.data_ptr(), (const int32_t*)cu_host.data_ptr(),
                            cu.numel() - 1, (float*)out.data_ptr(), normalize ? 1 : 0, workspace.data_ptr(), (size_t)workspace.numel(),
                            stream_of(ids)), "encode_bert");
}

void clip_resize_crop_u8(const at::Tensor& packed, const at::Tensor& offsets, const at::Tensor& heights, const at::Tensor& widths,
                         int64_t S, at::Tensor out, at::Tensor workspace) {
    need_dev(packed, at::kByte, "packed");
    need_dev(out, at::kByte, "out");
    need_dev(workspace, at::kByte, "workspace");
    const int64_t n = heights.numel();
    TORCH_CHECK(offsets.device().is_cpu() && offsets.scalar_type() == at::kLong && offsets.is_contiguous() && offsets.numel() == n &&
                heights.device().is_cpu() && heights.scalar_type() == at::kInt && heights.is_contiguous() &&
                widths.device().is_cpu() && widths.scalar_type() == at::kInt && widths.is_contiguous() && widths.numel() == n,
                "marqo_hip::clip_resize_crop_u8: offsets int64 [n], heights / widths int32 [n] on the CPU (the resampling plan is host work)");
    TORCH_CHECK(out.dim() == 4 && out.size(0) == n && out.size(1) == S && out.size(2) == S && out.size(3) == 3, "marqo_hip::clip_resize_crop_u8: out uint8 [n,S,S,3]");
    NoGil nogil;
    check_rc(mq_clip_resize_crop_u8((const uint8_t*)packed.data_ptr(), (const int64_t*)offsets.data_ptr(), (const int32_t*)heights.data_ptr(),
                                    (const int32_t*)widths.data_ptr(), n, (int32_t)S, (uint8_t*)out.data_ptr(), workspace.data_ptr(),
                                    (size_t)workspace.numel(), stream_of(packed)), "clip_resize_crop_u8");
}

int64_t clip_resize_workspace_bytes(const at::Tensor& heights, const at::Tensor& widths, int64_t S) {
    TORCH_CHECK(heights.device().is_cpu() && heights.scalar_type() == at::kInt && heights.is_contiguous() && widths.device().is_cpu() &&
                widths.scalar_type() == at::kInt && widths.is_contiguous() && widths.numel() == heights.numel(), "heights / widths: CPU int32 [n]");
    return (int64_t)mq_clip_resize_workspace_bytes((const int32_t*)heights.data_ptr(), (const int32_t*)widths.data_ptr(), heights.numel(), (int32_t)S);
}

at::Tensor gemm_bf16(const at::Tensor& A, const at::Tensor& W, const c10::optional<at::Tensor>& bias,
                     const c10::optional<at::Tensor>& residual, int64_t flags) {
    need_dev(A, at::kBFloat16, "A");
    need_dev(W, at::kBFloat16, "W");
    TORCH_CHECK(A.dim() == 2 && W.dim() == 2 && A.size(1) == W.size(1), "marqo_hip::gemm_bf16: A [M,K], W [N,K]");
    const int64_t M = A.size(0), K = A.size(1), N = W.size(0);
    const bool f32 = (flags & MQ_EPI_OUT_F32) != 0;
    const float* b = nullptr;
    const void* r = nullptr;
    if (flags & MQ_EPI_BIAS) {
        TORCH_CHECK(bias.has_value(), "marqo_hip::gemm_bf16: MQ_EPI_BIAS without bias");
        need_dev(*bias, at::kFloat, "bias");
        TORCH_CHECK(bias->numel() == N, "bias must be [N]");
        b = (const float*)bias->data_ptr();
    }
    if (flags & MQ_EPI_RESIDUAL) {
        TORCH_CHECK(residual.has_value(), "marqo_hip::gemm_bf16: MQ_EPI_RESIDUAL without residual");
        need_dev(*residual, f32 ? at::kFloat : at::kBFloat16, "residual");
        TORCH_CHECK(residual->dim() == 2 && residual->size(0) == M && residual->size(1) == N, "residual must be [M,N]");
        r = residual->data_ptr();
    }
    at::Tensor out = at::empty({M, N}, A.options().dtype(f32 ? at::kFloat : at::kBFloat16));
    check_rc(mq_gemm_bf16(A.data_ptr(), K, W.data_ptr(), K, b, (const float*)r, out.data_ptr(), N, M, N, K, (int)flags, stream_of(A)), "gemm_bf16");
    return out;
}

at::Tensor layernorm(const at::Tensor& x, const at::Tensor& gamma, const at::Tensor& beta, double eps, bool out_bf16) {
    need_dev(x, at::kFloat, "x");
    need_dev(gamma, at::kFloat, "gamma");
    need_dev(beta, at::kFloat, "beta");
    TORCH_CHECK(x.dim() == 2 && gamma.numel() == x.size(1) && beta.numel() == x.size(1), "marqo_hip::layernorm: x [rows,W], gamma / beta [W]");
    at::Tensor out = at::empty_like(x, x.options().dtype(out_bf16 ? at::kBFloat16 : at::kFloat));
    check_rc(mq_layernorm((const float*)x.data_ptr(), nullptr, (const float*)gamma.data_ptr(), (const float*)beta.data_ptr(),
                          out_bf16 ? out.data_ptr() : nullptr, out_bf16 ? nullptr : (float*)out.data_ptr(), x.size(0), (int32_t)x.size(1),
                          (float)eps, stream_of(x)), "layernorm");
    return out;
}

at::Tensor attention(const at::Tensor& qkv, const c10::optional<at::Tensor>& cu_seqlens, int64_t nseq, int64_t fixed_len, int64_t max_len,
                     int64_t heads, int64_t mask) {
    need_dev(qkv, at::kBFloat16, "qkv");
    TORCH_CHECK(qkv.dim() == 2 && qkv.size(1) % 3 == 0, "marqo_hip::attention: qkv [rows, 3W]");
    const int64_t W = qkv.size(1) / 3;
    const int32_t* cu = nullptr;
    if (cu_seqlens.has_value()) {
        need_dev(*cu_seqlens, at::kInt, "cu_seqlens");
        TORCH_CHECK(cu_seqlens->numel() == nseq + 1, "cu_seqlens must be [nseq + 1]");
        cu = (const int32_t*)cu_seqlens->data_ptr();
    }
    at::Tensor out = at::empty({qkv.size(0), W}, qkv.options());
    check_rc(mq_attention(qkv.data_ptr(), out.data_ptr(), cu, nseq, (int32_t)fixed_len, (int32_t)max_len, (int32_t)W, (int32_t)heads,
                          (int32_t)mask, stream_of(qkv)), "attention");
    return out;
}

at::Tensor l2_normalize(const at::Tensor& x) {
    need_dev(x, at::kFloat, "x");
    TORCH_CHECK(x.dim() == 2, "marqo_hip::l2_normalize: x [rows, D]");
    at::Tensor out = at::empty_like(x);
    check_rc(mq_l2_normalize((const float*)x.data_ptr(), (float*)out.data_ptr(), x.size(0), (int32_t)x.size(1), stream_of(x)), "l2_normalize");
    return out;
}

const int32_t* check_lora_seqs(const at::Tensor& seq_task, const at::Tensor& seq_task_host, const c10::optional<at::Tensor>& cu_seqlens, int64_t fixed_len) {
    need_dev(seq_task, at::kInt, "seq_task");
    TORCH_CHECK(seq_task_host.device().is_cpu() && seq_task_host.scalar_type() == at::kInt && seq_task_host.is_contiguous() &&
                seq_task_host.numel() == seq_task.numel(), "marqo_hip: seq_task_host must be the CPU int32 copy of seq_task");
    if (!cu_seqlens.has_value()) {
        TORCH_CHECK(fixed_len > 0, "marqo_hip: packed sequences need cu_seqlens (or give fixed_len > 0)");
        return nullptr;
    }
    need_dev(*cu_seqlens, at::kInt, "cu_seqlens");
    TORCH_CHECK(cu_seqlens->numel() == seq_task.numel() + 1, "cu_seqlens must be [nseq + 1]");
    return (const int32_t*)cu_seqlens->data_ptr();
}

at::Tensor lora_down(const at::Tensor& x, const at::Tensor& A, const at::Tensor& scale, const at::Tensor& seq_task, const at::Tensor& seq_task_host,
                     const c10::optional<at::Tensor>& cu_seqlens, int64_t fixed_len) {
    need_dev(x, at::kBFloat16, "x");
    need_dev(A, at::kBFloat16, "A");
    need_dev(scale, at::kFloat, "scale");
    TORCH_CHECK(x.dim() == 2 && A.dim() == 3 && A.size(2) == x.size(1) && scale.numel() == A.size(0), "marqo_hip::mq_lora_down: x [rows,K], A [tasks,R,K], scale [tasks]");
    const int32_t* cu = check_lora_seqs(seq_task, seq_task_host, cu_seqlens, fixed_len);
    at::Tensor T = at::zeros({x.size(0), A.size(1)}, x.options().dtype(at::kFloat));
    check_rc(mq_lora_down(x.data_ptr(), x.size(1), A.data_ptr(), (const float*)scale.data_ptr(), (const int32_t*)seq_task.data_ptr(),
                          (const int32_t*)seq_task_host.data_ptr(), cu, seq_task.numel(), (int32_t)fixed_len, x.size(0), (int32_t)A.size(0),
                          (int32_t)A.size(1), (int32_t)x.size(1), (float*)T.data_ptr(), stream_of(x)), "mq_lora_down");
    return T;
}

void lora_up(const at::Tensor& T, const at::Tensor& B, int64_t nblocks, const at::Tensor& seq_task, const at::Tensor& seq_task_host,
             const c10::optional<at::Tensor>& cu_seqlens, int64_t fixed_len, at::Tensor out, int64_t mode, int64_t act) {
    need_dev(T, at::kFloat, "T");
    need_dev(B, at::kBFloat16, "B");
    need_dev(out, mode == MQ_LORA_INPLACE ? at::kBFloat16 : at::kFloat, "out");
    TORCH_CHECK(T.dim() == 2 && B.dim() == 3 && out.dim() == 2 && out.size(0) == T.size(0) && out.size(1) >= B.size(1),
                "marqo_hip::mq_lora_up: T [rows,R], B [tasks,N,r], out [rows, ldc >= N]");
    const int32_t* cu = check_lora_seqs(seq_task, seq_task_host, cu_seqlens, fixed_len);
    check_rc(mq_lora_up((const float*)T.data_ptr(), (int32_t)T.size(1), B.data_ptr(), (int32_t)B.size(2), (int32_t)nblocks, (const int32_t*)seq_task.data_ptr(),
                        (const int32_t*)seq_task_host.data_ptr(), cu, seq_task.numel(), (int32_t)fixed_len, T.size(0), (int32_t)B.size(0), out.data_ptr(),
                        out.size(1), (int32_t)B.size(1), (int32_t)mode, (int32_t)act, stream_of(T)), "mq_lora_up");
}

void attention_gqa_prefix(const at::Tensor& qkv, const at::Tensor& cu_seqlens, int64_t prefix_len, int64_t max_len, int64_t q_heads, int64_t kv_heads,
                          int64_t head_dim, at::Tensor out) {
    need_dev(qkv, at::kBFloat16, "qkv");
    need_dev(out, at::kBFloat16, "out");
    need_dev(cu_seqlens, at::kInt, "cu_seqlens");
    TORCH_CHECK(q_heads >= 1 && kv_heads >= 1 && head_dim >= 1 && qkv.dim() == 2 && out.dim() == 2 && cu_seqlens.numel() >= 1 &&
                qkv.size(1) == (q_heads + 2 * kv_heads) * head_dim && out.size(0) == qkv.size(0) && out.size(1) == q_heads * head_dim,
                "marqo_hip::mq_attention_gqa_prefix: qkv [rows, (Q + 2 KV) hd], out [rows, Q hd], cu_seqlens [nseq + 1]");
    check_rc(mq_attention_gqa_prefix(qkv.data_ptr(), out.data_ptr(), (const int32_t*)cu_seqlens.data_ptr(), cu_seqlens.numel() - 1, (int32_t)prefix_len,
                                     (int32_t)max_len, (int32_t)q_heads, (int32_t)kv_heads, (int32_t)head_dim, stream_of(qkv)), "mq_attention_gqa_prefix");
}

void qk_norm_rope_at(at::Tensor qkv, const c10::optional<at::Tensor>& cu_seqlens, int64_t nseq, int64_t fixed_len, int64_t q_heads, int64_t kv_heads,
                     int64_t head_dim, const c10::optional<at::Tensor>& q_norm, const c10::optional<at::Tensor>& k_norm, double eps, const at::Tensor& inv_freq,
                     int64_t offset) {
    need_dev(qkv, at::kBFloat16, "qkv");
    need_dev(inv_freq, at::kFloat, "inv_freq");
    TORCH_CHECK(q_heads >= 1 && kv_heads >= 1 && head_dim >= 2 && qkv.dim() == 2 && qkv.size(1) == (q_heads + 2 * kv_heads) * head_dim &&
                inv_freq.numel() == head_dim / 2, "marqo_hip::mq_qk_norm_rope_at: qkv [rows, (Q + 2 KV) hd], inv_freq [hd / 2]");
    const int32_t* cu = nullptr;
    if (cu_seqlens.has_value()) {
        need_dev(*cu_seqlens, at::kInt, "cu_seqlens");
        TORCH_CHECK(cu_seqlens->numel() == nseq + 1, "cu_seqlens must be [nseq + 1]");
        cu = (const int32_t*)cu_seqlens->data_ptr();
    } else {
        TORCH_CHECK(fixed_len > 0 && nseq * fixed_len <= qkv.size(0), "marqo_hip::mq_qk_norm_rope_at: nseq * fixed_len rows must lie in qkv");
    }
    const float *qg = nullptr, *kg = nullptr;
    if (q_norm.has_value()) { need_dev(*q_norm, at::kFloat, "q_norm"); TORCH_CHECK(q_norm->numel() == head_dim, "q_norm must be [head_dim]"); qg = (const float*)q_norm->data_ptr(); }
    if (k_norm.has_value()) { need_dev(*k_norm, at::kFloat, "k_norm"); TORCH_CHECK(k_norm->numel() == head_dim, "k_norm must be [head_dim]"); kg = (const float*)k_norm->data_ptr(); }
    check_rc(mq_qk_norm_rope_at(qkv.data_ptr(), cu, nseq, (int32_t)fixed_len, (int32_t)q_heads, (int32_t)kv_heads, (int32_t)head_dim, qg, kg, (float)eps,
                                (const float*)inv_freq.data_ptr(), (int32_t)offset, stream_of(qkv)), "mq_qk_norm_rope_at");
}

void attention_gqa256_prefix(const at::Tensor& qkv, const at::Tensor& cu_seqlens, int64_t prefix_len, int64_t max_len, int64_t q_heads, int64_t kv_heads,
                             int64_t head_dim, double scale, at::Tensor out) {
    need_dev(qkv, at::kBFloat16, "qkv");
    need_dev(out, at::kBFloat16, "out");
    need_dev(cu_seqlens, at::kInt, "cu_seqlens");
    TORCH_CHECK(q_heads >= 1 && kv_heads >= 1 && head_dim >= 1 && qkv.dim() == 2 && out.dim() == 2 && cu_seqlens.numel() >= 1 &&
                qkv.size(1) == (q_heads + 2 * kv_heads) * head_dim && out.size(0) == qkv.size(0) && out.size(1) == q_heads * head_dim,
                "marqo_hip::mq_attention_gqa256_prefix: qkv [rows, (Q + 2 KV) hd], out [rows, Q hd], cu_seqlens [nseq + 1]");
    check_rc(mq_attention_gqa256_prefix(qkv.data_ptr(), out.data_ptr(), (const int32_t*)cu_seqlens.data_ptr(), cu_seqlens.numel() - 1, (int32_t)prefix_len,
                                        (int32_t)max_len, (int32_t)q_heads, (int32_t)kv_heads, (int32_t)head_dim, (float)scale, stream_of(qkv)),
             "mq_attention_gqa256_prefix");
}

int64_t abi_version() { return mq_abi_version(); }

}

TORCH_LIBRARY(marqo_hip, m) {
    m.def("encode_image_u8(Tensor cfg, Tensor weights, Tensor pixels, Tensor(a!) out, bool normalize, Tensor(b!) workspace) -> ()");
    m.def("encode_image_f32(Tensor cfg, Tensor weights, Tensor pixels, Tensor(a!) out, bool normalize, Tensor(b!) workspace) -> ()");
    m.def("encode_clip_text(Tensor cfg, Tensor weights, Tensor ids, Tensor cu_seqlens, Tensor cu_seqlens_host, Tensor? pool_rows, "
          "Tensor(a!) out, bool normalize, Tensor(b!) workspace) -> ()");
    m.def("encode_bert(Tensor cfg, Tensor weights, Tensor ids, Tensor cu_seqlens, Tensor cu_seqlens_host, Tensor(a!) out, bool normalize, "
          "Tensor(b!) workspace) -> ()");
    m.def("clip_resize_crop_u8(Tensor packed, Tensor offsets, Tensor heights, Tensor widths, int S, Tensor(a!) out, Tensor(b!) workspace) -> ()");
    m.def("clip_resize_workspace_bytes(Tensor heights, Tensor widths, int S) -> int", &clip_resize_workspace_bytes);
    m.def("gemm_bf16(Tensor A, Tensor W, Tensor? bias, Tensor? residual, int flags) -> Tensor");
    m.def("layernorm(Tensor x, Tensor gamma, Tensor beta, float eps, bool out_bf16) -> Tensor");
    m.def("attention(Tensor qkv, Tensor? cu_seqlens, int nseq, int fixed_len, int max_len, int heads, int mask) -> Tensor");
    m.def("l2_normalize(Tensor x) -> Tensor");
    m.def("mq_lora_down(Tensor x, Tensor A, Tensor scale, Tensor seq_task, Tensor seq_task_host, Tensor? cu_seqlens, int fixed_len) -> Tensor");
    m.def("mq_lora_up(Tensor T, Tensor B, int nblocks, Tensor seq_task, Tensor seq_task_host, Tensor? cu_seqlens, int fixed_len, Tensor(a!) out, "
          "int mode, int act) -> ()");
    m.def("mq_attention_gqa_prefix(Tensor qkv, Tensor cu_seqlens, int prefix_len, int max_len, int q_heads, int kv_heads, int head_dim, "
          "Tensor(a!) out) -> ()");
    m.def("mq_qk_norm_rope_at(Tensor(a!) qkv, Tensor? cu_seqlens, int nseq, int fixed_len, int q_heads, int kv_heads, int head_dim, Tensor? q_norm, "
          "Tensor? k_norm, float eps, Tensor inv_freq, int offset) -> ()");
    m.def("mq_attention_gqa256_prefix(Tensor qkv, Tensor cu_seqlens, int prefix_len, int max_len, int q_heads, int kv_heads, int head_dim, float scale, "
          "Tensor(a!) out) -> ()");
    m.def("abi_version() -> int", &abi_version);
}

TORCH_LIBRARY_IMPL(marqo_hip, CUDA, m) {
    m.impl("encode_image_u8", &encode_image_u8);
    m.impl("encode_image_f32", &encode_image_f32);
    m.impl("encode_clip_text", &encode_clip_text);
    m.impl("encode_bert", &encode_bert);
    m.impl("clip_resize_crop_u8", &clip_resize_crop_u8);
    m.impl("gemm_bf16", &gemm_bf16);
    m.impl("layernorm", &layernorm);
    m.impl("attention", &attention);
    m.impl("l2_normalize", &l2_normalize);
    m.impl("mq_lora_down", &lora_down);
    m.impl("mq_lora_up", &lora_up);
    m.impl("mq_attention_gqa_prefix", &attention_gqa_prefix);
    m.impl("mq_qk_norm_rope_at", &qk_norm_rope_at);
    m.impl("mq_attention_gqa256_prefix", &attention_gqa256_prefix);
}
```

### marqo_amd/csrc/towers.hip

```cpp
#include "packed_text.h"
#include "knobs.h"

int mq_cast_bf16(const float* d_x, void* d_out, int64_t n, hipStream_t s);
extern "C" int mq_rowquant_fp8(const float* d_x, void* d_out_fp8, float* d_row_scale, int64_t rows, int32_t W, void* stream);

static_assert(sizeof(mq_block_weights) == 36 * 8, "mq_block_weights layout");
static_assert(sizeof(mq_encoder_cfg) == 112, "mq_encoder_cfg layout");
static_assert(sizeof(mq_vit_cfg) == 168 && sizeof(mq_clip_text_cfg) == 128 && sizeof(mq_bert_cfg) == 136, "tower cfg layouts");
static_assert(sizeof(mq_vit_weights) == 11 * 8 && sizeof(mq_map_head) == 11 * 8 && sizeof(mq_clip_text_weights) == 7 * 8, "tower weight layouts");

static bool attn_proj_fill_ok(int64_t nseq) {
    const int64_t rounds = (nseq + 255) / 256;
    return mq_tower_attn_proj > 0 && nseq >= mq_tower_attn_proj && (rounds == 1 || nseq * 4 >= rounds * 256 * 3);
}
static bool panel_fill_ok(int64_t nseq) {
    const int64_t rounds = (nseq + 255) / 256;
    return mq_tower_panel_gemm > 0 && nseq >= mq_tower_panel_gemm && nseq * 4 >= rounds * 256 * 3;
}
extern "C" int mq_layernorm_ex(const void* d_x, int x_bf16, const int32_t* d_row_idx, const float* d_g, const float* d_b, void* d_out_bf16,
                               float* d_out_f32, int64_t rows, int32_t W, float eps, void* stream);
bool mq_gemm_small_ok(int64_t M, int64_t N, int64_t K, bool ln);
int mq_ln_gemm_small(const void* d_x, int64_t ldx, int x_bf16, const float* ln_g, const float* ln_b, float eps, const void* d_W, int64_t ldw,
                     const float* d_bias, void* d_out, int64_t ldc, int64_t M, int64_t N, int64_t K, int flags, float* d_ln_out,
                     const int32_t* d_rows, hipStream_t s);
// ... 444 lines not shown
    const bool feeds_selected = select_last && l == cfg->layers - 2;
    MQ_TRY(mq_layernorm_pf(h, 1, nullptr, b.ln2_g, b.ln2_b, last ? nullptr : h, last || feeds_selected ? d_x : nullptr, rows, W, cfg->ln_eps,
                           pf(nb ? nb->qkv_w : nullptr), (size_t)3 * Wa * W * 2, pf(nb ? nb->out_w : nullptr), (size_t)W * Wa * 2, s));
    return MQ_OK;
}

int EncoderPass::block_post_ln(const mq_block_weights& b, int l) {
    MQ_TRY(mq_gemm_bf16(h, W, b.qkv_w, W, b.qkv_b, nullptr, qf, 3 * Wa, rows, 3 * Wa, W, MQ_EPI_BIAS, s));
    if (cfg->d_rope_inv_freq) MQ_TRY(mq_rope(qf, d_cu_seqlens, nseq, fixed_len, Wa, cfg->heads, cfg->d_rope_inv_freq, s));
    MQ_TRY(attn_bf16(cfg, qf, a, d_cu_seqlens, nseq, fixed_len, max_len, Wa, s));
    MQ_TRY(mq_gemm_bf16(a, Wa, b.out_w, Wa, b.out_b, d_x, d_x, W, rows, W, Wa, res_flags, s));
    MQ_TRY(mq_layernorm_pf(d_x, 0, nullptr, b.ln1_g, b.ln1_b, h, d_x, rows, W, cfg->ln_eps, pf(b.fc1_w), (size_t)(cfg->mlp_glu ? 2 : 1) * F * W * 2,
                           pf(b.fc2_w), (size_t)W * F * 2, s));
    if (cfg->mlp_glu) {
        MQ_TRY(mq_gemm_bf16(h, W, b.fc1_w, W, b.fc1_b, nullptr, qf, 2 * F, rows, 2 * F, W, b.fc1_b ? MQ_EPI_BIAS : 0, s));
        MQ_TRY(mq_glu(qf, rows, F, cfg->act, 0, s));
        MQ_TRY(mq_gemm_bf16(qf, 2 * F, b.fc2_w, F, b.fc2_b, d_x, d_x, W, rows, W, F, res_flags, s));
    } else {
        MQ_TRY(mq_gemm_bf16(h, W, b.fc1_w, W, b.fc1_b, nullptr, qf, F, rows, F, W, MQ_EPI_BIAS | act_flag, s));
        MQ_TRY(mq_gemm_bf16(qf, F, b.fc2_w, F, b.fc2_b, d_x, d_x, W, rows, W, F, res_flags, s));
    }
    const mq_block_weights* nb = l + 1 < cfg->layers && l + 1 < first8 ? &blocks[l + 1] : nullptr;
    MQ_TRY(mq_layernorm_pf(d_x, 0, nullptr, b.ln2_g, b.ln2_b, h, d_x, rows, W, cfg->ln_eps, pf(nb ? nb->qkv_w : nullptr), (size_t)3 * Wa * W * 2,
                           pf(nb ? nb->out_w : nullptr), (size_t)W * Wa * 2, s));
    return MQ_OK;
}

int encoder_forward_impl(const mq_encoder_cfg* cfg, const mq_block_weights* blocks, float* d_x, int64_t rows,
                         const int32_t* d_cu_seqlens, int64_t nseq, int32_t fixed_len, int32_t max_len,
                         const int32_t* d_sel, int64_t nsel, void* d_workspace, size_t workspace_bytes, hipStream_t s, int64_t sel_stride = 0,
                         const float* stats0 = nullptr) {
    MQ_TRY(check_encoder_cfg(cfg));
    MQ_CHECK_ARG(sel_stride == 0 || (sel_strided_ok(cfg, nsel, sel_stride) && (nsel - 1) * sel_stride < rows), "mq_encoder_forward: bad pooled-row pitch");
    const bool has_sel = (d_sel || sel_stride > 0) && nsel > 0;
    MQ_CHECK_ARG(d_x && (blocks || cfg->layers == 0), "mq_encoder_forward: null pointer");
    if (rows <= 0 || cfg->layers == 0) return MQ_OK;
    if (workspace_bytes < encoder_ws(cfg, rows)) {
        mq_set_error("mq_encoder_forward: workspace %zu < required %zu", workspace_bytes, encoder_ws(cfg, rows));
        return MQ_ERR_WORKSPACE;
    }
    const int W = cfg->width, F = cfg->mlp_dim, Wa = attn_width(cfg);
    const int fcols = cfg->mlp_glu ? 2 * F : F;
    const size_t big = (size_t)(3 * Wa > fcols ? 3 * Wa : fcols);
    Off cv;
    char* wsb = (char*)d_workspace;
    void* h = wsb + cv.take((size_t)rows * W * 2);
    void* a = wsb + cv.take((size_t)rows * Wa * 2);
    void* qf = wsb + cv.take((size_t)rows * big * 2);
    float* row_scale = (float*)(wsb + cv.take((size_t)rows * 4));
    float* row_stats = (float*)(wsb + cv.take((size_t)rows * 8));
    float* row_part = (float*)(wsb + cv.take((size_t)rows * part_slots(cfg) * 8));
    float* xn = (float*)(wsb + cv.take((size_t)(rows < SMALL_LN_ROWS ? rows : SMALL_LN_ROWS) * W * 4));
    uint32_t* band_ctr = (uint32_t*)(wsb + cv.take((size_t)mq_gemm_band_counters(rows) * 4));
    if (stream_bf16(cfg) && mq_gemm_rs_in_launch()) MQ_CHECK_HIP(hipMemsetAsync(band_ctr, 0, (size_t)mq_gemm_band_counters(rows) * 4, s));
    else band_ctr = nullptr;

    const size_t xsel_off = align_up((size_t)(nsel > 0 ? nsel : 0) * F * 2, WS_ALIGN);
    const bool select_last = has_sel && nsel * 2 <= rows && mq_tower_row_select && !cfg->mlp_glu && !cfg->d_rope_inv_freq && !cfg->d_rope_table &&
                             !mq_gemm_small_ok(rows, W, W, false) &&
                             !(cfg->precision == MQ_PREC_FP8 && (cfg->d_fp8_act_amax || cfg->post_ln)) &&
                             xsel_off + (size_t)nsel * W * 4 <= (size_t)rows * big * 2;

    t_ln_prefetch = weights_outlive_cache(cfg, Wa);
    const int first8 = cfg->precision == MQ_PREC_FP8 ? (cfg->fp8_first_layer < cfg->layers ? cfg->fp8_first_layer : cfg->layers) : cfg->layers;

    const bool small_post_ln = cfg->post_ln && first8 >= cfg->layers && !cfg->mlp_glu && !cfg->d_rope_inv_freq && rows <= SMALL_LN_ROWS &&
                               mq_gemm_small_ok(rows, 3 * Wa, W, true) && mq_gemm_small_ok(rows, F, W, true) && mq_gemm_small_ok(rows, W, F, false);
    const bool post16 = stream_post16(cfg) && !small_post_ln && !mq_gemm_small_ok(rows, W, W, false);
    if (cfg->post_ln && first8 == 0) MQ_TRY(mq_rowquant_fp8(d_x, h, row_scale, rows, W, s));
    else if (cfg->post_ln) MQ_TRY(mq_cast_bf16(d_x, h, rows * W, s));

    EncoderPass p{cfg, blocks, d_x, rows, d_cu_seqlens, nseq, fixed_len, max_len, d_sel, nsel, s, W, F, Wa, h, a, qf, row_scale, row_stats, row_part, xn, band_ctr,
                   false, act_epi(cfg->act), MQ_EPI_BIAS | MQ_EPI_RESIDUAL | MQ_EPI_OUT_F32, first8, stats0, has_sel, select_last};
    for (int l = 0; l < cfg->layers; ++l) {
        const mq_block_weights& b = blocks[l];
        const bool f8 = l >= first8;
        MQ_CHECK_ARG(b.qkv_w && b.out_w && b.fc1_w && b.fc2_w && b.ln1_g && b.ln2_g, "mq_encoder_forward: layer %d has null weights", l);
        if (f8)
            MQ_CHECK_ARG(b.qkv_w8 && b.qkv_ws && b.out_w8 && b.out_ws && b.fc1_w8 && b.fc1_ws && b.fc2_w8 && b.fc2_ws,
                         "mq_encoder_forward: layer %d has no fp8 weights", l);
        if (cfg->post_ln && f8 && l == first8 && l > 0) MQ_TRY(mq_rowquant_fp8(d_x, h, row_scale, rows, W, s));
        if (select_last && l == cfg->layers - 1) {
            MQ_TRY(last_block_selected(cfg, b, l, d_x, rows, d_cu_seqlens, nseq, fixed_len, max_len, d_sel, sel_stride, nsel, h, a, qf, row_scale, row_stats,
                                       p.x_has_partials, (float*)((char*)qf + xsel_off), f8, s));
            break;
        }
        if (f8) MQ_TRY(p.block_fp8(b, l));
        else if (eva_form(cfg)) MQ_TRY(p.block_eva(b, l));
        else if (!cfg->post_ln) MQ_TRY(p.block_pre_ln(b, l));
        else if (small_post_ln) MQ_TRY(p.block_post_ln_small(b, l));
        else if (post16) MQ_TRY(p.block_post_ln_bf16(b, l));
        else MQ_TRY(p.block_post_ln(b, l));
    }
    return MQ_OK;
}
}

extern "C" int mq_encoder_forward(const mq_encoder_cfg* cfg, const mq_block_weights* blocks, float* d_x, int64_t rows,
                                  const int32_t* d_cu_seqlens, int64_t nseq, int32_t fixed_len, int32_t max_len,
                                  void* d_workspace, size_t workspace_bytes, void* stream) {
    return encoder_forward_impl(cfg, blocks, d_x, rows, d_cu_seqlens, nseq, fixed_len, max_len, nullptr, 0, d_workspace, workspace_bytes,
                                (hipStream_t)stream);
}

extern "C" int mq_encoder_forward_rows(const mq_encoder_cfg* cfg, const mq_block_weights* blocks, float* d_x, int64_t rows,
                                       const int32_t* d_cu_seqlens, int64_t nseq, int32_t fixed_len, int32_t max_len,
                                       const int32_t* d_out_rows, int64_t n_out_rows, void* d_workspace, size_t workspace_bytes,
                                       void* stream) {
    MQ_CHECK_ARG(d_out_rows && n_out_rows > 0, "mq_encoder_forward_rows: empty row selection");
    return encoder_forward_impl(cfg, blocks, d_x, rows, d_cu_seqlens, nseq, fixed_len, max_len, d_out_rows, n_out_rows, d_workspace,
                                workspace_bytes, (hipStream_t)stream);
}

namespace {
struct VitPlan {
    int T, np, Kp; int64_t rows;
    size_t off_x, off_rows, off_cls, off_stats0, off_enc, off_patches, off_patch_out, total;
    size_t off_map_y, off_map_z, off_map_h, off_tok, off_kv;
};
VitPlan vit_plan(const mq_vit_cfg* c, int64_t n) {
    VitPlan p;
    const int G = c->image_size / c->patch_size;
    const bool map = c->pool == MQ_VIT_POOL_MAP || c->pool == MQ_VIT_POOL_QUERY;
    p.np = G * G; p.T = p.np + (c->pool == MQ_VIT_POOL_MAP ? 0 : 1); p.Kp = ceil64(3 * c->patch_size * c->patch_size); p.rows = n * p.T;
    const int W = c->enc.width;
    Off cv;
    p.off_x = cv.take((size_t)p.rows * W * 4);
    p.off_rows = cv.take((size_t)n * 4);
    p.off_cls = cv.take((size_t)n * W * 2);
    p.off_stats0 = cv.take((size_t)p.rows * 8);
    p.off_map_y = p.off_map_z = p.off_map_h = p.off_tok = p.off_kv = 0;
    if (map) {
        p.off_map_y = cv.take((size_t)n * W * 4);
        p.off_map_z = cv.take((size_t)n * W * 2);
        p.off_map_h = cv.take((size_t)n * c->map_mlp_dim * 2);
    }
    p.off_enc = cv.end();
    size_t enc = encoder_ws(&c->enc, p.rows);
    if (map) {
        Off mv;
        p.off_tok = p.off_enc + mv.take((size_t)p.rows * W * 2);
        p.off_kv = p.off_enc + mv.take((size_t)p.rows * 2 * W * 2);
        if (mv.end() > enc) enc = mv.end();
    }
    Off pv;
    p.off_patches = p.off_enc + pv.take((size_t)n * p.np * p.Kp * 2);
    p.off_patch_out = p.off_enc + pv.take((size_t)n * p.np * W * 4);
    const size_t patches = pv.end();
    p.total = p.off_enc + (enc > patches ? enc : patches);
    return p;
}

int encode_image_impl(const mq_vit_cfg* cfg, const mq_vit_weights* w, const void* d_pixels, bool is_u8, int64_t n,
                      float* d_out, int normalize, void* ws, size_t ws_bytes, hipStream_t s) {
    MQ_CHECK_ARG(cfg && w && d_out, "mq_encode_image: null pointer");
    MQ_TRY(check_encoder_cfg(&cfg->enc));
    MQ_CHECK_ARG(cfg->patch_size > 0 && cfg->image_size >= cfg->patch_size, "mq_encode_image: image %d smaller than patch %d",
                 cfg->image_size, cfg->patch_size);
    MQ_CHECK_ARG(cfg->out_dim >= 4 && cfg->out_dim % 4 == 0, "mq_encode_image: out_dim %d must be a multiple of 4", cfg->out_dim);
    const bool map = cfg->pool == MQ_VIT_POOL_MAP;
    const bool avg = cfg->pool == MQ_VIT_POOL_AVG;
    const bool qpool = cfg->pool == MQ_VIT_POOL_QUERY;
    MQ_CHECK_ARG(cfg->pool == MQ_VIT_POOL_CLS || map || avg || qpool, "mq_encode_image: bad pool %d", cfg->pool);
    MQ_CHECK_ARG(w->patch_w && w->pos && w->ln_post_g && w->ln_post_b, "mq_encode_image: null weight pointer");
    const int W = cfg->enc.width;
    if (map) {
        const mq_map_head* m = w->map;
        MQ_CHECK_ARG(m && m->q && m->kv_w && m->kv_b && m->proj_w && m->proj_b && m->ln_g && m->ln_b && m->fc1_w && m->fc1_b && m->fc2_w && m->fc2_b,
                     "mq_encode_image: MQ_VIT_POOL_MAP needs the attention-pool head's weights");
        MQ_CHECK_ARG(!w->cls && !w->ln_pre_g && !w->ln_pre_b, "mq_encode_image: MQ_VIT_POOL_MAP has no class token / ln_pre");
        MQ_CHECK_ARG(cfg->map_mlp_dim >= 64 && cfg->map_mlp_dim % 64 == 0, "mq_encode_image: map_mlp_dim %d must be a multiple of 64", cfg->map_mlp_dim);
        MQ_CHECK_ARG(w->proj_w || cfg->out_dim == W, "mq_encode_image: without a projection out_dim (%d) must equal the width (%d)", cfg->out_dim, W);
    } else {
        MQ_CHECK_ARG(w->cls && w->proj_w && (avg || eva_form(&cfg->enc) || (w->ln_pre_g && w->ln_pre_b)) && (!w->ln_pre_g == !w->ln_pre_b),
                     "mq_encode_image: null weight pointer (ln_pre may be absent only with MQ_VIT_POOL_AVG and in the EVA02 form)");
        MQ_CHECK_ARG(!w->proj_b || cfg->pool == MQ_VIT_POOL_CLS, "mq_encode_image: proj_b goes with MQ_VIT_POOL_CLS");
    }
    if (qpool) {
        const mq_map_head* m = w->map;
        MQ_CHECK_ARG(m && m->q && m->kv_w && m->kv_b && m->proj_w && m->proj_b && m->ln_g && m->ln_b, "mq_encode_image: MQ_VIT_POOL_QUERY needs the pooler's weights");
        MQ_CHECK_ARG(cfg->pool_dim >= 64 && cfg->pool_dim % 64 == 0 && cfg->pool_dim <= W && cfg->pool_heads >= 1 && cfg->pool_dim % cfg->pool_heads == 0,
                     "mq_encode_image: pool_dim %d / pool_heads %d unsupported (pool_dim a multiple of 64, <= the width %d)", cfg->pool_dim, cfg->pool_heads, W);
    }
    if (n <= 0) return MQ_OK;
    MQ_CHECK_ARG(d_pixels && ws, "mq_encode_image: null input / workspace");
    const VitPlan p = vit_plan(cfg, n);
    if (ws_bytes < p.total) { mq_set_error("mq_encode_image: workspace %zu < required %zu", ws_bytes, p.total); return MQ_ERR_WORKSPACE; }
    char* base = (char*)ws;
    float* x = (float*)(base + p.off_x);
    int32_t* rows_idx = (int32_t*)(base + p.off_rows);
    void* cls_ln = base + p.off_cls;
    void* patches = base + p.off_patches;
    float* patch_out = (float*)(base + p.off_patch_out);

    MQ_TRY(mq_patchify(d_pixels, is_u8, patches, n, cfg->image_size, cfg->patch_size, p.Kp, cfg->mean, cfg->std, s));
    MQ_TRY(mq_gemm_bf16(patches, p.Kp, w->patch_w, p.Kp, nullptr, nullptr, patch_out, W, n * p.np, W, p.Kp, MQ_EPI_OUT_F32, s));
    const int xb = stream_bf16(&cfg->enc) ? 1 : 0;
    const float* stats0 = nullptr;
    if (mq_tower_assemble_stats && xb && w->ln_pre_g && cfg->pool == MQ_VIT_POOL_CLS && cfg->enc.precision == MQ_PREC_BF16 && !cfg->enc.post_ln &&
        !eva_form(&cfg->enc) && cfg->enc.layers >= 2 && mq_tower_ln_fold && mq_tower_panel_gemm == 0 && mq_vit_assemble_stats_ok(W) && w->blocks &&
        fold_ok(xb, w->blocks[0].qkv_wf, w->blocks[0].qkv_bf, w->blocks[0].qkv_sf, p.rows, 3 * attn_width(&cfg->enc), W) &&
        !mq_gemm_small_ok(p.rows, 3 * attn_width(&cfg->enc), W, true))
        stats0 = (const float*)(base + p.off_stats0);
    if (stats0) {
        const int Wa = attn_width(&cfg->enc);
        const bool wpf = weights_outlive_cache(&cfg->enc, Wa);
        MQ_TRY(mq_vit_assemble_stats(patch_out, w->cls, w->pos, w->ln_pre_g, w->ln_pre_b, x, const_cast<float*>(stats0), n, p.T, W, cfg->enc.ln_eps,
                                     wpf ? w->blocks[0].qkv_wf : nullptr, (size_t)3 * Wa * W * 2, wpf ? w->blocks[0].out_w : nullptr, (size_t)W * Wa * 2, s));
    }
    else MQ_TRY(mq_vit_assemble(patch_out, w->cls, w->pos, w->ln_pre_g, w->ln_pre_b, x, n, p.T, W, cfg->enc.ln_eps, xb, s));
    if (map) {
        const mq_map_head* m = w->map;
        const int F = cfg->map_mlp_dim;
        MQ_TRY(encoder_forward_impl(&cfg->enc, w->blocks, x, p.rows, nullptr, n, p.T, p.T, nullptr, 0, base + p.off_enc,
                                    ws_bytes - p.off_enc, s));
        void* tok = base + p.off_tok;
        void* kv = base + p.off_kv;
        float* y = (float*)(base + p.off_map_y);
        void* z = base + p.off_map_z;
        void* hmid = base + p.off_map_h;
        MQ_TRY(mq_layernorm_ex(x, xb, nullptr, w->ln_post_g, w->ln_post_b, tok, nullptr, p.rows, W, cfg->enc.ln_eps, s));
        MQ_TRY(mq_gemm_bf16(tok, W, m->kv_w, W, m->kv_b, nullptr, kv, 2 * W, p.rows, 2 * W, W, MQ_EPI_BIAS, s));
        MQ_TRY(mq_map_pool(kv, m->q, cls_ln, n, p.T, W, cfg->enc.heads, s));
        MQ_CHECK_HIP(hipMemsetAsync(y, 0, (size_t)n * W * 4, s));
        MQ_TRY(mq_gemm_bf16(cls_ln, W, m->proj_w, W, m->proj_b, y, y, W, n, W, W, MQ_EPI_BIAS | MQ_EPI_RESIDUAL | MQ_EPI_OUT_F32, s));
        MQ_TRY(mq_layernorm(y, nullptr, m->ln_g, m->ln_b, z, nullptr, n, W, cfg->enc.ln_eps, s));
        MQ_TRY(mq_gemm_bf16(z, W, m->fc1_w, W, m->fc1_b, nullptr, hmid, F, n, F, W, MQ_EPI_BIAS | MQ_EPI_GELU, s));
        MQ_TRY(mq_gemm_bf16(hmid, F, m->fc2_w, F, m->fc2_b, y, y, W, n, W, F, MQ_EPI_BIAS | MQ_EPI_RESIDUAL | MQ_EPI_OUT_F32, s));
        if (w->proj_w) {
            MQ_TRY(mq_cast_bf16(y, z, (int64_t)n * W, s));
            MQ_TRY(mq_gemm_bf16(z, W, w->proj_w, W, nullptr, nullptr, d_out, cfg->out_dim, n, cfg->out_dim, W, MQ_EPI_OUT_F32, s));
            if (normalize) MQ_TRY(mq_l2_normalize(d_out, d_out, n, cfg->out_dim, s));
        } else if (normalize) {
            MQ_TRY(mq_l2_normalize(y, d_out, n, W, s));
        } else {
            MQ_CHECK_HIP(hipMemcpyAsync(d_out, y, (size_t)n * W * 4, hipMemcpyDeviceToDevice, s));
        }
        return MQ_OK;
    }
    if (qpool) {
        const mq_map_head* m = w->map;
        const int Dp = cfg->pool_dim;
        MQ_TRY(encoder_forward_impl(&cfg->enc, w->blocks, x, p.rows, nullptr, n, p.T, p.T, nullptr, 0, base + p.off_enc, ws_bytes - p.off_enc, s));
        void* tok = base + p.off_tok;
        void* kv = base + p.off_kv;
        float* y = (float*)(base + p.off_map_y);
        void* z = base + p.off_map_z;
        MQ_TRY(mq_layernorm_ex(x, xb, nullptr, w->ln_post_g, w->ln_post_b, tok, nullptr, p.rows, W, cfg->enc.ln_eps, s));
        MQ_TRY(mq_gemm_bf16(tok, W, m->kv_w, W, m->kv_b, nullptr, kv, 2 * Dp, p.rows, 2 * Dp, W, MQ_EPI_BIAS, s));
        MQ_TRY(mq_map_pool(kv, m->q, cls_ln, n, p.T, Dp, cfg->pool_heads, s));
        MQ_CHECK_HIP(hipMemsetAsync(y, 0, (size_t)n * Dp * 4, s));
        MQ_TRY(mq_gemm_bf16(cls_ln, Dp, m->proj_w, Dp, m->proj_b, y, y, Dp, n, Dp, Dp, MQ_EPI_BIAS | MQ_EPI_RESIDUAL | MQ_EPI_OUT_F32, s));
        MQ_TRY(mq_layernorm(y, nullptr, m->ln_g, m->ln_b, z, nullptr, n, Dp, cfg->enc.ln_eps, s));
        MQ_TRY(mq_gemm_bf16(z, Dp, w->proj_w, Dp, nullptr, nullptr, d_out, cfg->out_dim, n, cfg->out_dim, Dp, MQ_EPI_OUT_F32, s));
        if (normalize) MQ_TRY(mq_l2_normalize(d_out, d_out, n, cfg->out_dim, s));
        return MQ_OK;
    }
    if (avg) {
        MQ_TRY(encoder_forward_impl(&cfg->enc, w->blocks, x, p.rows, nullptr, n, p.T, p.T, nullptr, 0, base + p.off_enc, ws_bytes - p.off_enc, s));
        float* pooled = (float*)(base + p.off_enc);
        MQ_TRY(mq_avg_tokens(x, xb, pooled, n, p.T, 1, W, s));
        MQ_TRY(mq_layernorm(pooled, nullptr, w->ln_post_g, w->ln_post_b, cls_ln, nullptr, n, W, cfg->enc.ln_eps, s));
        MQ_TRY(mq_gemm_bf16(cls_ln, W, w->proj_w, W, nullptr, nullptr, d_out, cfg->out_dim, n, cfg->out_dim, W, MQ_EPI_OUT_F32, s));
        if (normalize) MQ_TRY(mq_l2_normalize(d_out, d_out, n, cfg->out_dim, s));
        return MQ_OK;
    }
    const int64_t pitch = sel_strided_ok(&cfg->enc, n, p.T) ? p.T : 0;
    if (!pitch) MQ_TRY(mq_cls_rows(rows_idx, n, p.T, s));
    else rows_idx = nullptr;
    MQ_TRY(encoder_forward_impl(&cfg->enc, w->blocks, x, p.rows, nullptr, n, p.T, p.T, rows_idx, n, base + p.off_enc,
                                ws_bytes - p.off_enc, s, pitch, stats0));
    if (mq_gemm_small_ok(n, cfg->out_dim, W, true))
        MQ_TRY(mq_ln_gemm_small(x, pitch ? pitch * W : W, xb, w->ln_post_g, w->ln_post_b, cfg->enc.ln_eps, w->proj_w, W, w->proj_b, d_out, cfg->out_dim, n, cfg->out_dim,
                                W, MQ_EPI_OUT_F32 | (w->proj_b ? MQ_EPI_BIAS : 0), nullptr, rows_idx, s));
    else {
        MQ_TRY(mq_layernorm_rows_pf(x, xb, rows_idx, pitch ? pitch : 1, w->ln_post_g, w->ln_post_b, cls_ln, nullptr, n, W, cfg->enc.ln_eps, nullptr, 0, nullptr, 0, s));
        MQ_TRY(mq_gemm_bf16(cls_ln, W, w->proj_w, W, w->proj_b, nullptr, d_out, cfg->out_dim, n, cfg->out_dim, W, MQ_EPI_OUT_F32 | (w->proj_b ? MQ_EPI_BIAS : 0), s));
    }
    if (normalize) MQ_TRY(mq_l2_normalize(d_out, d_out, n, cfg->out_dim, s));
    return MQ_OK;
}
}

extern "C" size_t mq_vit_workspace_bytes(const mq_vit_cfg* cfg, int64_t n_images) {
    if (!cfg || n_images <= 0 || cfg->patch_size <= 0) return 0;
    return vit_plan(cfg, n_images).total;
}

extern "C" int mq_encode_image_u8(const mq_vit_cfg* cfg, const mq_vit_weights* w, const uint8_t* d_pixels, int64_t n,
                                  float* d_out, int normalize, void* d_workspace, size_t workspace_bytes, void* stream) {
    return encode_image_impl(cfg, w, d_pixels, true, n, d_out, normalize, d_workspace, workspace_bytes, (hipStream_t)stream);
}

extern "C" int mq_encode_image_f32(const mq_vit_cfg* cfg, const mq_vit_weights* w, const float* d_pixels, int64_t n,
                                   float* d_out, int normalize, void* d_workspace, size_t workspace_bytes, void* stream) {
    return encode_image_impl(cfg, w, d_pixels, false, n, d_out, normalize, d_workspace, workspace_bytes, (hipStream_t)stream);
}

namespace {
struct TextPlan { size_t off_x, off_rows, off_pool, off_enc, total; };
TextPlan text_plan(const mq_encoder_cfg* enc, int64_t rows, int64_t nseq) {
    TextPlan p;
    Off cv;
    p.off_x = cv.take((size_t)rows * enc->width * 4);
    p.off_rows = cv.take((size_t)nseq * 4);
    p.off_pool = cv.take((size_t)nseq * enc->width * 4);
    p.off_enc = cv.end();
    p.total = p.off_enc + encoder_ws(enc, rows);
    return p;
}
}

extern "C" size_t mq_clip_text_workspace_bytes(const mq_clip_text_cfg* cfg, int64_t rows, int64_t nseq) {
    if (!cfg || rows <= 0 || nseq <= 0) return 0;
    return text_plan(&cfg->enc, rows, nseq).total;
}

extern "C" int mq_encode_clip_text(const mq_clip_text_cfg* cfg, const mq_clip_text_weights* w, const int32_t* d_ids,
                                   const int32_t* d_cu_seqlens, const int32_t* h_cu_seqlens, int64_t nseq,
                                   const int32_t* d_pool_rows, float* d_out, int normalize, void* d_workspace,
                                   size_t workspace_bytes, void* stream) {
    MQ_CHECK_ARG(cfg && w && d_out, "mq_encode_clip_text: null pointer");
    MQ_TRY(check_encoder_cfg(&cfg->enc));
    MQ_CHECK_ARG(cfg->out_dim >= 4 && cfg->out_dim % 4 == 0, "mq_encode_clip_text: out_dim %d must be a multiple of 4", cfg->out_dim);
    MQ_CHECK_ARG(w->tok_emb && w->pos && w->ln_final_g && w->ln_final_b && w->proj_w, "mq_encode_clip_text: null weight pointer");
    if (nseq <= 0) return MQ_OK;
    MQ_CHECK_ARG(d_ids && d_cu_seqlens && h_cu_seqlens && d_workspace, "mq_encode_clip_text: null input / workspace");
    MQ_CHECK_ARG(h_cu_seqlens[0] == 0, "mq_encode_clip_text: cu_seqlens[0] must be 0");
    int64_t rows = 0;
    const int maxl = max_seq_len(h_cu_seqlens, nseq, &rows);
    MQ_CHECK_ARG(maxl >= 1 && maxl <= cfg->ctx + (cfg->cls_pos > 0 ? 1 : 0), "mq_encode_clip_text: sequence lengths must be in [1, ctx=%d]", cfg->ctx);
    MQ_CHECK_ARG(cfg->cls_pos >= 0 && cfg->cls_pos < cfg->ctx, "mq_encode_clip_text: cls_pos %d outside the position table [0, %d)", cfg->cls_pos, cfg->ctx);
    const TextPlan p = text_plan(&cfg->enc, rows, nseq);
    MQ_TRY(packed_workspace("mq_encode_clip_text", workspace_bytes, p.total));
    hipStream_t s = (hipStream_t)stream;
    char* base = (char*)d_workspace;
    float* x = (float*)(base + p.off_x);
    int32_t* rows_idx = (int32_t*)(base + p.off_rows);
    void* pooled = base + p.off_pool;
    const int W = cfg->enc.width;

    const int xb = stream_bf16(&cfg->enc) ? 1 : 0;
    MQ_TRY(mq_embed_tokens(d_ids, d_cu_seqlens, nseq, w->tok_emb, w->pos, nullptr, nullptr, nullptr, xb ? nullptr : x, xb ? (void*)x : nullptr, W,
                           cfg->vocab, 0.f, cfg->cls_pos, s));
    const int32_t* pool_rows = d_pool_rows;
    if (!pool_rows) { MQ_TRY(mq_last_rows(d_cu_seqlens, rows_idx, nseq, s)); pool_rows = rows_idx; }
    MQ_TRY(encoder_forward_impl(&cfg->enc, w->blocks, x, rows, d_cu_seqlens, nseq, 0, maxl, pool_rows, nseq, base + p.off_enc,
                                workspace_bytes - p.off_enc, s));
    if (!w->proj_b && mq_gemm_small_ok(nseq, cfg->out_dim, W, true)) {
        MQ_TRY(mq_ln_gemm_small(x, W, xb, w->ln_final_g, w->ln_final_b, cfg->enc.ln_eps, w->proj_w, W, nullptr, d_out, cfg->out_dim, nseq,
                                cfg->out_dim, W, MQ_EPI_OUT_F32, nullptr, pool_rows, s));
        if (normalize) MQ_TRY(mq_l2_normalize(d_out, d_out, nseq, cfg->out_dim, s));
        return MQ_OK;
    }
    MQ_TRY(mq_layernorm_ex(x, xb, pool_rows, w->ln_final_g, w->ln_final_b, pooled, nullptr, nseq, W, cfg->enc.ln_eps, s));
    if (w->proj_b) {
        MQ_CHECK_HIP(hipMemsetAsync(d_out, 0, (size_t)nseq * cfg->out_dim * 4, s));
        MQ_TRY(mq_gemm_bf16(pooled, W, w->proj_w, W, w->proj_b, d_out, d_out, cfg->out_dim, nseq, cfg->out_dim, W,
                            MQ_EPI_BIAS | MQ_EPI_RESIDUAL | MQ_EPI_OUT_F32, s));
    } else
        MQ_TRY(mq_gemm_bf16(pooled, W, w->proj_w, W, nullptr, nullptr, d_out, cfg->out_dim, nseq, cfg->out_dim, W, MQ_EPI_OUT_F32, s));
    if (normalize) MQ_TRY(mq_l2_normalize(d_out, d_out, nseq, cfg->out_dim, s));
    return MQ_OK;
}

extern "C" size_t mq_bert_workspace_bytes(const mq_bert_cfg* cfg, int64_t rows, int64_t nseq) {
    if (!cfg || rows <= 0 || nseq <= 0) return 0;
    return text_plan(&cfg->enc, rows, nseq).total;
}

extern "C" int mq_encode_bert(const mq_bert_cfg* cfg, const mq_bert_weights* w, const int32_t* d_ids,
                              const int32_t* d_cu_seqlens, const int32_t* h_cu_seqlens, int64_t nseq, float* d_out,
                              int normalize, void* d_workspace, size_t workspace_bytes, void* stream) {
    MQ_CHECK_ARG(cfg && w && d_out, "mq_encode_bert: null pointer");
    MQ_TRY(check_encoder_cfg(&cfg->enc));
    MQ_CHECK_ARG(cfg->enc.post_ln == 1 && cfg->enc.mask == MQ_MASK_NONE, "mq_encode_bert: BERT is post-LN with full attention");
    MQ_CHECK_ARG(cfg->pool == MQ_POOL_MEAN || cfg->pool == MQ_POOL_CLS, "mq_encode_bert: bad pooling %d", cfg->pool);
    if (cfg->out_dim)
        MQ_CHECK_ARG(cfg->out_dim >= 4 && cfg->out_dim % 4 == 0 && w->proj1_w && w->proj1_b &&
                     (w->proj2_w ? (cfg->proj_hidden >= 64 && cfg->proj_hidden % 64 == 0 && cfg->proj_hidden <= 3 * cfg->enc.width) : cfg->proj_hidden == 0),
                     "mq_encode_bert: projection head needs out_dim %% 4 == 0, proj1_w / proj1_b, and either proj2_w with proj_hidden %% 64 == 0 "
                     "(<= 3 W: the MLP head) or neither (one biased Linear)");
    MQ_CHECK_ARG(w->word_emb && (w->pos_emb || cfg->enc.d_rope_inv_freq) && w->emb_ln_g && w->emb_ln_b, "mq_encode_bert: null weight pointer");
    if (nseq <= 0) return MQ_OK;
    int maxl = 0;
    int64_t rows = 0;
    MQ_TRY(packed_begin("mq_encode_bert", d_ids, d_cu_seqlens, h_cu_seqlens, nseq, cfg->max_pos, d_workspace, &maxl, &rows));
    const TextPlan p = text_plan(&cfg->enc, rows, nseq);
    MQ_TRY(packed_workspace("mq_encode_bert", workspace_bytes, p.total));
    hipStream_t s = (hipStream_t)stream;
    char* base = (char*)d_workspace;
    float* x = (float*)(base + p.off_x);
    const int W = cfg->enc.width;

    MQ_TRY(mq_embed_tokens(d_ids, d_cu_seqlens, nseq, w->word_emb, w->pos_emb, w->type_emb, w->emb_ln_g, w->emb_ln_b, x, nullptr, W,
                           cfg->vocab, cfg->enc.ln_eps, 0, s));
    const int32_t* sel = cfg->pool == MQ_POOL_CLS ? d_cu_seqlens : nullptr;
    MQ_TRY(encoder_forward_impl(&cfg->enc, w->blocks, x, rows, d_cu_seqlens, nseq, 0, maxl, sel, sel ? nseq : 0, base + p.off_enc,
                                workspace_bytes - p.off_enc, s));
    if (!cfg->out_dim) {
        MQ_TRY(mq_pool(x, d_cu_seqlens, nseq, d_out, W, cfg->pool, normalize, s));
        return MQ_OK;
    }
    float* pooled = (float*)(base + p.off_pool);
    bf16_t* pb = (bf16_t*)(base + p.off_enc);
    bf16_t* h1 = pb + (size_t)nseq * W;
    MQ_TRY(mq_pool(x, d_cu_seqlens, nseq, pooled, W, cfg->pool, 0, s));
    MQ_TRY(mq_cast_bf16(pooled, pb, (int64_t)nseq * W, s));
    if (!w->proj2_w) {
        MQ_TRY(mq_gemm_bf16(pb, W, w->proj1_w, W, w->proj1_b, nullptr, d_out, cfg->out_dim, nseq, cfg->out_dim, W, MQ_EPI_BIAS | MQ_EPI_OUT_F32, s));
    } else {
        MQ_TRY(mq_gemm_bf16(pb, W, w->proj1_w, W, w->proj1_b, nullptr, h1, cfg->proj_hidden, nseq, cfg->proj_hidden, W, MQ_EPI_BIAS | MQ_EPI_GELU, s));
        MQ_TRY(mq_gemm_bf16(h1, cfg->proj_hidden, w->proj2_w, cfg->proj_hidden, nullptr, nullptr, d_out, cfg->out_dim, nseq, cfg->out_dim,
                            cfg->proj_hidden, MQ_EPI_OUT_F32, s));
    }
    if (normalize) MQ_TRY(mq_l2_normalize(d_out, d_out, nseq, cfg->out_dim, s));
    return MQ_OK;
}
```

### marqo_amd/engine/towers.py

```python
from __future__ import annotations

import ctypes as C
import logging
import os
import threading
from typing import Dict, Optional, Sequence, Tuple

import numpy as np
import torch

from marqo_amd import _lib as L
from marqo_amd.engine import native_queue as NQ
from marqo_amd.engine.archs import BertArch, ClipTextArch, VitArch, OPENAI_DATASET_MEAN, OPENAI_DATASET_STD
from marqo_amd.engine.tower_weights import (
    EVA_GLU_EPILOGUE, KERNEL_HEAD_DIMS, LN_FOLD, RESNET_BN_EPS, _OPEN_CLIP_KEYS, _TIMM_KEYS, _Holder, _bert_blocks, _ceil64, _clip_blocks,
    _eva_blocks, _head_dim, _kernel_head_dim, _need, _pad_heads, _pad_mlp, convnext_downsample_gather, convnext_downsample_weight,
    convnext_dw_taps, convnext_fold_gamma_fc2, convnext_fold_ln_fc1, fold_layernorm, nllb_clip_state_dict, patch_embed_weight, resnet_attnpool_weights,
    resnet_conv1x1_weight, resnet_conv3x3_weight, resnet_fold_bn, resnet_pad64, resnet_pad_vec, resnet_stem_weight)

Tensor = torch.Tensor
_log = logging.getLogger(__name__)

MAX_ROWS_PER_CALL = 1 << 18

# ... 291 lines not shown
                else:
                    lo = mid
            first = hi
        extra = 0
        self.fp8_policy_trace = [(first, 0, e)]
        if not enc.post_ln and os.environ.get("MARQO_AMD_FP8_MLP_ONLY", "1") != "0":
            best = (self._fp8_share(layers, first, 0), first, 0, e)
            step = max(1, layers // 8)
            for s_ in sorted({min(layers, first + k * step) for k in range(0, 9)} | {layers}):
                if s_ == 0:
                    continue
                lo_x, hi_x = 0, s_
                e_s = err_split(s_, 0) if s_ != first else e
                if e_s > budget:
                    continue
                e_at = {0: e_s}
                while hi_x - lo_x > 0:
                    mid = (lo_x + hi_x + 1) // 2
                    em = err_split(s_, mid)
                    e_at[mid] = em
                    if em <= budget:
                        lo_x = mid
                    else:
                        hi_x = mid - 1
                share = self._fp8_share(layers, s_, lo_x)
                self.fp8_policy_trace.append((s_, lo_x, e_at[lo_x]))
                if share > best[0] + 1e-9:
                    best = (share, s_, lo_x, e_at[lo_x])
            _, first, extra, e = best
        enc.fp8_first_layer, enc.fp8_mlp_extra = first, extra
        self.fp8_first_layer, self.fp8_mlp_extra, self.fp8_calibration_error = first, extra, e
        self._fp8.calibrated = True
        _log.info("fp8 policy: blocks [%d, %d) on e4m3 + the MLP halves of blocks [%d, %d), %s residual stream, 1 - cos vs bf16 on the calibration "
                  "batch %.2e (all blocks: %.2e, budget %.1e)", first, layers, first - extra, first, self.residual_stream, e, e0, budget)
        return first

    def release_unused_folded(self) -> int:
        blocks = getattr(self, "_blocks", None)
        if blocks is None or not hasattr(blocks[0], "qkv_wf"):
            return 0
        enc = self.cfg.enc
        layers = len(blocks)
        bf16_stream = enc.residual_stream == 1
        fp8 = self.precision == "fp8"
        first = enc.fp8_first_layer if fp8 else layers
        first_mlp = first - (enc.fp8_mlp_extra if fp8 else 0)
        freed = 0
        for i in range(layers):
            b = blocks[i]
            for name, alive in (("qkv", bf16_stream and i < first), ("fc1", bf16_stream and i < first_mlp)):
                if alive:
                    continue
                for suffix in ("_wf", "_bf", "_sf"):
                    ptr = getattr(b, name + suffix)
                    if ptr:
                        freed += self._h.drop(ptr)
                        setattr(b, name + suffix, None)
        if freed:
            getattr(self, "_graphs", {}).clear()
            for _, q in (self._queues or {}).values():
                q.close()
            if self._queues:
                self._queues = {}
        return freed

    def _calibration_run(self):
        raise NotImplementedError(f"{type(self).__name__} has no calibration batch")

    def tune_residual_default(self) -> str:
        return self.tune_residual_stream(self._calibration_run())

    def tune_fp8_default(self, budget: Optional[float] = None) -> int:
        return self.tune_fp8(self._calibration_run(), budget=budget)

    pools_one_row = False

    def _fp8_share(self, layers: int, split: int, extra: int) -> float:
        share = (layers - split) + (2.0 / 3.0) * extra
        if self.pools_one_row:
            if split < layers:
                share -= 0.75
            elif extra >= 1:
                share -= 2.0 / 3.0
        return share

    def __init__(self, device: str):
        self.device = _require_gpu(device)
        self.lib = L.load()
        self._h = _Holder(self.device)
        self._tls = threading.local()
        self._lock = threading.Lock()
        self._graphs: Dict[tuple, "_GraphedCall"] = {}
        self._graphs_off = False
        self._ops = L.load_torch_ops() if L.boundary() == "torch_ops" else None
        self._blobs = None

    _queues: Optional[Dict[bool, tuple]] = None
    _queues_off = False

    def _cached_queue(self, normalize: bool, make, what: str, *how):
        sig = bytes(self.cfg)
        ent = (self._queues or {}).get(bool(normalize))
        if ent is not None and ent[0] == sig:
            return ent[1]
        with self._lock:
            if self._queues is None:
                self._queues = {}
            ent = self._queues.get(bool(normalize))
            if ent is not None and ent[0] == sig:
                return ent[1]
            if ent is not None:
                ent[1].close()
            try:
                q = make(self.device.index if self.device.index is not None else torch.cuda.current_device(), normalize, *how)
            except (L.MarqoHipUnavailableError, L.MarqoHipError) as e:
                self._queues_off = True
                _log.warning("native request queue unavailable (%s); small %s calls keep the direct path", e, what)
                return None
            self._queues[bool(normalize)] = (sig, q)
            return q

    def tune(self, key: str, value: int) -> None:
        L.check(self.lib.mq_tune(key.encode(), int(value)), "mq_tune")
        with self._lock:
            getattr(self, "_graphs", {}).clear()
            for ent in (self._queues or {}).values():
                ent[1].close()
            self._queues = None

    def _forget_queue(self, q) -> None:
        with self._lock:
            for k, ent in list((self._queues or {}).items()):
                if ent[1] is q:
                    del self._queues[k]

    def _through_queue(self, q, encode, *args):
        try:
            return encode(*args)
        except L.MarqoHipError as e:
            if NQ.gone(e):
                self._forget_queue(q)
                return None
            raise

    def queue_stats(self) -> Dict[bool, Dict[str, int]]:
        return {k: ent[1].stats() for k, ent in (self._queues or {}).items()}

    def _desc(self):
        if self._blobs is None:
            self._blobs = (L.struct_blob(self.cfg), L.struct_blob(self.w))
        return self._blobs

    def _call_image(self, kind: str, pixels: Tensor, n: int, out: Tensor, normalize: bool, ws: Tensor) -> None:
        if self._ops is not None:
            cfg, w = self._desc()
            (self._ops.encode_image_u8 if kind == "u8" else self._ops.encode_image_f32)(cfg, w, pixels, out, bool(normalize), ws)
            return
        fn = self.lib.mq_encode_image_u8 if kind == "u8" else self.lib.mq_encode_image_f32
        L.check(fn(C.byref(self.cfg), C.byref(self.w), pixels.data_ptr(), n, out.data_ptr(), 1 if normalize else 0, ws.data_ptr(),
                   ws.numel(), self._stream()), "mq_encode_image")

    def _call_text(self, clip: bool, d_packed: Tensor, d_cu: Tensor, cu: Tensor, nseq: int, d_pool: Optional[Tensor], out: Tensor,
                   normalize: bool, ws: Tensor) -> None:
        if self._ops is not None:
            cfg, w = self._desc()
            if clip:
                self._ops.encode_clip_text(cfg, w, d_packed, d_cu, cu, d_pool, out, bool(normalize), ws)
            else:
                self._ops.encode_bert(cfg, w, d_packed, d_cu, cu, out, bool(normalize), ws)
            return
        if clip:
            L.check(self.lib.mq_encode_clip_text(C.byref(self.cfg), C.byref(self.w), d_packed.data_ptr(), d_cu.data_ptr(), cu.data_ptr(), nseq,
                                                 L.ptr(d_pool), out.data_ptr(), 1 if normalize else 0, ws.data_ptr(), ws.numel(),
                                                 self._stream()), "mq_encode_clip_text")
        else:
            L.check(self.lib.mq_encode_bert(C.byref(self.cfg), C.byref(self.w), d_packed.data_ptr(), d_cu.data_ptr(), cu.data_ptr(), nseq,
                                            out.data_ptr(), 1 if normalize else 0, ws.data_ptr(), ws.numel(), self._stream()),
                    "mq_encode_bert")

    def _graphs_ok(self) -> bool:
        return GRAPHS and not self._graphs_off and (self._fp8 is None or self._fp8.calibrated)

    def _capture(self, key: tuple, make) -> Optional["_GraphedCall"]:
        g = self._graphs.get(key)
        if g is None:
            if len(self._graphs) >= MAX_GRAPHS_PER_TOWER:
                return None
            try:
                g = self._graphs[key] = make()
            except RuntimeError as e:
                self._graphs_off = True
                _log.warning("hipGraph capture failed (%s); this tower keeps launching eagerly", e)
                return None
        return g

    def _workspace(self, nbytes: int) -> Tensor:
        by_stream = getattr(self._tls, "ws", None)
        if by_stream is None:
            by_stream = self._tls.ws = {}
        key = torch.cuda.current_stream(self.device).cuda_stream
        ws = by_stream.get(key)
        if ws is None or ws.numel() < nbytes:
            if len(by_stream) >= 4:
                by_stream.clear()
            ws = by_stream[key] = torch.empty(int(nbytes * 1.25) + 256, dtype=torch.uint8, device=self.device)
        return ws

    def _stream(self) -> int:
        return torch.cuda.current_stream(self.device).cuda_stream

    def weight_bytes(self) -> int:
        return self._h.nbytes()


class _ImageTowerBase(_TowerBase):

    def _run_chunks(self, kind: str, pixels: Tensor, normalize: bool) -> Tensor:
        n = pixels.shape[0]
        out = torch.empty(n, self.arch.out_dim, dtype=torch.float32, device=self.device)
        for i in range(0, n, self.max_images_per_call):
            m = min(self.max_images_per_call, n - i)
            ws = self._workspace(self._image_workspace_bytes(m))
            self._launch_images(kind, pixels[i:i + m], m, out[i:i + m], normalize, ws)
        return out

    def _run(self, kind: str, pixels: Tensor, normalize: bool) -> Tensor:
        with torch.cuda.device(self.device):
            return self._run_chunks(kind, pixels, normalize)

    def _check_u8(self, images_u8: Tensor) -> Tensor:
        S = self.arch.image_size
        if images_u8.dtype != torch.uint8 or images_u8.ndim != 4 or tuple(images_u8.shape[1:]) != (S, S, 3):
            raise ValueError(f"expected uint8 [n, {S}, {S}, 3], got {images_u8.dtype} {tuple(images_u8.shape)}")
        return images_u8.to(self.device, non_blocking=True).contiguous()

    def encode_u8(self, images_u8: Tensor, normalize: bool = True) -> Tensor:
        return self._run("u8", self._check_u8(images_u8), normalize)

    def encode_f32(self, pixels: Tensor, normalize: bool = True) -> Tensor:
        S = self.arch.image_size
        if pixels.ndim != 4 or tuple(pixels.shape[1:]) != (3, S, S):
            raise ValueError(f"expected float [n, 3, {S}, {S}], got {tuple(pixels.shape)}")
        return self._run("f32", pixels.to(device=self.device, dtype=torch.float32, non_blocking=True).contiguous(), normalize)


class VitTower(_ImageTowerBase):

    def __init__(self, arch: VitArch, sd: Dict[str, Tensor], device: str,
                 mean: Sequence[float] = OPENAI_DATASET_MEAN, std: Sequence[float] = OPENAI_DATASET_STD,
                 precision: str = "bf16"):
        super().__init__(device)
        _check_precision(precision)
        self.precision = precision
        self.arch = arch
        W, P = arch.width, arch.patch_size
        if arch.image_size < P:
            raise ValueError("image_size must be at least one patch")
        h = self._h
        patch_w = patch_embed_weight(sd, "visual.trunk.patch_embed.proj.weight" if arch.pool == "map" or arch.eva else "visual.conv1.weight", W, P)
        if arch.pool == "map":
            t = "visual.trunk."
            F = arch.mlp_dim
            hd = _head_dim(W, arch.heads)
            if arch.out_dim != W:
                raise ValueError(f"SigLIP towers have no visual projection: out_dim {arch.out_dim} must equal the width {W}")
            pos = _need(sd, t + "pos_embed", (1, arch.tokens, W)).detach().to(torch.float32)[0] + \
                _need(sd, t + "patch_embed.proj.bias", (W,)).detach().to(torch.float32)
            self._blocks = _clip_blocks(h, sd, t, arch.layers, W, F, arch.heads, keys=_TIMM_KEYS)
            a = t + "attn_pool."
            f32 = lambda k, shape: _need(sd, a + k, shape).detach().to(torch.float32)
            q = (f32("latent", (1, 1, W)).reshape(W) @ f32("q.weight", (W, W)).t() + f32("q.bias", (W,))) * hd ** -0.5
            m1_w, m1_b, m2_w = _pad_mlp(f32("mlp.fc1.weight", (F, W)), f32("mlp.fc1.bias", (F,)), f32("mlp.fc2.weight", (W, F)))
            self._map = L.MapHead(q=h.f32(q), kv_w=h.bf16(f32("kv.weight", (2 * W, W))), kv_b=h.f32(f32("kv.bias", (2 * W,))),
                                  proj_w=h.bf16(f32("proj.weight", (W, W))), proj_b=h.f32(f32("proj.bias", (W,))),
                                  ln_g=h.f32(f32("norm.weight", (W,))), ln_b=h.f32(f32("norm.bias", (W,))),
                                  fc1_w=h.bf16(m1_w), fc1_b=h.f32(m1_b), fc2_w=h.bf16(m2_w), fc2_b=h.f32(f32("mlp.fc2.bias", (W,))))
            self.w = L.VitWeights(patch_w=h.bf16(patch_w), cls=None, pos=h.f32(pos), ln_pre_g=None, ln_pre_b=None, blocks=self._blocks,
                                  ln_post_g=h.f32(_need(sd, t + "norm.weight", (W,))), ln_post_b=h.f32(_need(sd, t + "norm.bias", (W,))),
                                  proj_w=None, map=C.pointer(self._map))
            pool, map_mlp = L.MQ_VIT_POOL_MAP, _ceil64(F)
        elif arch.pool == "query":
            D, Hp = arch.out_dim, arch.pool_heads
            if D % Hp or (D // Hp) % 8 or D // Hp > 128 or D % 64 or D > W:
                raise ValueError(f"attentional pooler of width {D} with {Hp} heads is not runnable (head dim a multiple of 8, <= 128; width a multiple of 64, <= {W})")
            self._blocks = _clip_blocks(h, sd, "visual.transformer.", arch.layers, W, arch.mlp_dim, arch.heads)
            a = "visual.attn_pool."
            f32 = lambda k, shape: _need(sd, a + k, shape).detach().to(torch.float32)
            bias = f32("attn.in_proj_bias", (3 * D,))
            query = _need(sd, a + "query", None).detach().to(torch.float32)
            if query.ndim != 2 or query.shape[1] != D:
                raise ValueError(f"checkpoint tensor '{a}query' has shape {tuple(query.shape)}, expected [n_queries, {D}]")
            q0 = torch.nn.functional.layer_norm(query[:1], (D,), f32("ln_q.weight", (D,)), f32("ln_q.bias", (D,)), arch.ln_eps)[0]
            q0 = (q0 @ f32("attn.q_proj_weight", (D, D)).t() + bias[:D]) * (D // Hp) ** -0.5
            kv_w = torch.cat([f32("attn.k_proj_weight", (D, W)), f32("attn.v_proj_weight", (D, W))], dim=0)
            self._map = L.MapHead(q=h.f32(q0), kv_w=h.bf16(kv_w), kv_b=h.f32(bias[D:]),
                                  proj_w=h.bf16(f32("attn.out_proj.weight", (D, D))), proj_b=h.f32(f32("attn.out_proj.bias", (D,))),
                                  ln_g=h.f32(_need(sd, "visual.ln_post.weight", (D,))), ln_b=h.f32(_need(sd, "visual.ln_post.bias", (D,))),
                                  fc1_w=None, fc1_b=None, fc2_w=None, fc2_b=None)
            self.w = L.VitWeights(
                patch_w=h.bf16(patch_w), cls=h.f32(_need(sd, "visual.class_embedding", (W,))),
                pos=h.f32(_need(sd, "visual.positional_embedding", (arch.tokens, W))),
                ln_pre_g=h.f32(_need(sd, "visual.ln_pre.weight", (W,))), ln_pre_b=h.f32(_need(sd, "visual.ln_pre.bias", (W,))),
                blocks=self._blocks, ln_post_g=h.f32(f32("ln_k.weight", (W,))), ln_post_b=h.f32(f32("ln_k.bias", (W,))),
                proj_w=h.bf16(_need(sd, "visual.proj", (D, D)).detach().to(torch.float32).t()), map=C.pointer(self._map))
            pool, map_mlp = L.MQ_VIT_POOL_QUERY, 0
        elif arch.eva:
            if precision != "bf16" or arch.pool != "cls":
                raise ValueError("EVA02 towers run on the bf16 path with the class-token head")
            t = "visual.trunk."
            f32 = lambda k, shape: _need(sd, t + k, shape).detach().to(torch.float32)
            pos = f32("pos_embed", (1, arch.tokens, W))[0].clone()
            pos[1:] += f32("patch_embed.proj.bias", (W,))
            self._blocks = _eva_blocks(h, sd, t, arch.layers, W, arch.mlp_dim, arch.heads)
            self._rope = h.f32(arch.rope_table())
            self.w = L.VitWeights(patch_w=h.bf16(patch_w), cls=h.f32(f32("cls_token", (1, 1, W)).reshape(W)), pos=h.f32(pos), ln_pre_g=None, ln_pre_b=None,
                                  blocks=self._blocks, ln_post_g=h.f32(f32("norm.weight", (W,))), ln_post_b=h.f32(f32("norm.bias", (W,))),
                                  proj_w=h.bf16(f32("head.weight", (arch.out_dim, W))), map=None, proj_b=h.f32(f32("head.bias", (arch.out_dim,))))
            pool, map_mlp = L.MQ_VIT_POOL_CLS, 0
        else:
            self._blocks = _clip_blocks(h, sd, "visual.transformer.", arch.layers, W, arch.mlp_dim, arch.heads)
            if arch.pool == "avg" and arch.ln_pre:
                raise ValueError("pool 'avg' is built for the no_ln_pre / final_ln_after_pool form (CLIPA)")
            self.w = L.VitWeights(
                patch_w=h.bf16(patch_w),
                cls=h.f32(_need(sd, "visual.class_embedding", (W,))),
                pos=h.f32(_need(sd, "visual.positional_embedding", (arch.tokens, W))),
                ln_pre_g=h.f32(_need(sd, "visual.ln_pre.weight", (W,))) if arch.ln_pre else None,
                ln_pre_b=h.f32(_need(sd, "visual.ln_pre.bias", (W,))) if arch.ln_pre else None,
                blocks=self._blocks,
                ln_post_g=h.f32(_need(sd, "visual.ln_post.weight", (W,))), ln_post_b=h.f32(_need(sd, "visual.ln_post.bias", (W,))),
                proj_w=h.bf16(_need(sd, "visual.proj", (W, arch.out_dim)).detach().to(torch.float32).t()), map=None)
            pool, map_mlp = (L.MQ_VIT_POOL_AVG if arch.pool == "avg" else L.MQ_VIT_POOL_CLS), 0
            self.pools_one_row = arch.pool != "avg"
        self.cfg = L.VitCfg(enc=_encoder_cfg(W, arch.layers, arch.heads, arch.mlp_dim, arch.quick_gelu, False,
                                             L.MQ_MASK_NONE, arch.ln_eps),
                            image_size=arch.image_size, patch_size=P, out_dim=arch.out_dim,
                            mean=(C.c_float * 3)(*mean), std=(C.c_float * 3)(*std), pool=pool, map_mlp_dim=map_mlp,
                            pool_dim=arch.out_dim if arch.pool == "query" else 0, pool_heads=arch.pool_heads if arch.pool == "query" else 0)
        if arch.eva:
            enc = self.cfg.enc
            enc.mlp_glu, enc.act, enc.mlp_ln_dim = (2 if EVA_GLU_EPILOGUE else 1), L.MQ_ACT_SILU, arch.mlp_dim
            enc.d_rope_table, enc.rope_prefix = self._rope, 1
        self.max_images_per_call = max(1, MAX_ROWS_PER_CALL // arch.tokens)
        if precision == "fp8":
            self._enable_fp8(self._blocks, arch.layers, W, _ceil64(arch.mlp_dim))
        self.cfg.enc.residual_stream = 2
        if precision == "bf16":
            self.tune_residual_default()

    def _calibration_run(self):
        u8 = self.calibration_images()
        return lambda: self.encode_u8(u8)

    def _image_workspace_bytes(self, m: int) -> int:
        return self.lib.mq_vit_workspace_bytes(C.byref(self.cfg), m)

    def _launch_images(self, kind: str, pixels: Tensor, m: int, out: Tensor, normalize: bool, ws: Tensor) -> None:
        self._call_image(kind, pixels, m, out, normalize, ws)

    def _run(self, kind: str, pixels: Tensor, normalize: bool) -> Tensor:
        n = pixels.shape[0]
        if n == 1 and self._graphs_ok():
            with self._lock, torch.cuda.device(self.device):
                def make():
                    inp = torch.empty_like(pixels)
                    o = torch.empty(1, self.arch.out_dim, dtype=torch.float32, device=self.device)
                    ws = torch.empty(self._image_workspace_bytes(1) + 256, dtype=torch.uint8, device=self.device)
                    inp.copy_(pixels)
                    return _GraphedCall(self.device, inp, o, (ws,), lambda: self._call_image(kind, inp, 1, o, normalize, ws))
                g = self._capture((pixels.dtype, bool(normalize)), make)
                if g is not None:
                    return g(pixels)
        with torch.cuda.device(self.device), _large_call(self.device, n * self.arch.tokens):
            return self._run_chunks(kind, pixels, normalize)

    def _queue(self, normalize: bool) -> Optional["NQ.ImageQueue"]:
        if not NQ.ENABLED or NQ.IMAGE_REQUEST_MAX <= 0 or self._queues_off or (self._fp8 is not None and not self._fp8.calibrated):
            return None
        return self._cached_queue(normalize, self._make_queue, "image")

    def _make_queue(self, idx: int, normalize: bool) -> "NQ.ImageQueue":
        return NQ.ImageQueue(self.lib, self.cfg, self.w, idx, self.arch.out_dim, bool(normalize))

    def queue_rows_images(self, tensors: Sequence[Tensor], normalize: bool = True) -> Optional[np.ndarray]:
        n = len(tensors)
        if n < 1 or n > NQ.IMAGE_REQUEST_MAX:
            return None
        q = self._queue(normalize)
        if q is None:
            return None
        S = self.arch.image_size
        ptrs = []
        for t in tensors:
            if t.dtype != torch.float32 or t.device != self.device or tuple(t.shape) != (3, S, S) or not t.is_contiguous():
                return None
            ptrs.append(t.data_ptr())
        return self._through_queue(q, q.encode_ptrs, ptrs)

    def calibration_images(self, n: int = 16, seed: int = 0) -> Tensor:
        S = self.arch.image_size
        g = torch.Generator().manual_seed(1000 + seed)
        noise = torch.randint(0, 256, (n - n // 2, S, S, 3), generator=g, dtype=torch.uint8)
        coarse = torch.rand(n // 2, 3, 8, 8, generator=g)
        smooth = torch.nn.functional.interpolate(coarse, size=(S, S), mode="bilinear", align_corners=False)
        smooth = (smooth * 255 + 12 * torch.randn(smooth.shape, generator=g)).clamp(0, 255).permute(0, 2, 3, 1).to(torch.uint8)
        return torch.cat([noise, smooth], dim=0).contiguous().to(self.device)


def _host_i64(t) -> np.ndarray:
    if isinstance(t, torch.Tensor):
        t = t.detach().cpu().numpy()
    return np.ascontiguousarray(t, dtype=np.int64)


def _pack(ids: np.ndarray, lengths: np.ndarray) -> Tuple[Tensor, Tensor]:
    n, S = ids.shape
    keep = np.arange(S)[None, :] < lengths[:, None]
    packed = np.ascontiguousarray(ids[keep], dtype=np.int32)
    cu = np.zeros(n + 1, dtype=np.int32)
    np.cumsum(lengths, out=cu[1:])
    return torch.from_numpy(packed), torch.from_numpy(cu)


def _ids_and_lengths(ids, attention_mask, max_pos: int) -> Tuple[np.ndarray, np.ndarray]:
    if ids.shape != attention_mask.shape or ids.ndim != 2:
        raise ValueError("ids and attention_mask must both be [n, S]")
    ids_h, mask_h = _host_i64(ids), _host_i64(attention_mask)
    n, S = ids_h.shape
    lengths = mask_h.sum(axis=1)
    if bool((lengths < 1).any()):
        raise ValueError("every sequence needs at least one unmasked token")
    if not bool(((mask_h != 0) == (np.arange(S)[None, :] < lengths[:, None])).all()):
        raise ValueError("attention_mask must be right-padded (a prefix of ones per row); left-padded input is not served")
    if n and int(lengths.max()) > max_pos:
        raise ValueError(f"sequence longer than max_position_embeddings={max_pos}")
    return ids_h, lengths


class _TextTowerBase(_TowerBase):
    max_rows_per_call = MAX_ROWS_PER_CALL

    def _chunks(self, lengths: np.ndarray):
        n = int(lengths.size)
        if n == 0:
            return
        cum = np.cumsum(lengths)
        total, limit = int(cum[-1]), int(self.max_rows_per_call)
        if total <= limit:
            yield 0, n
            return
        pieces = -(-total // limit)
        target = -(-total // pieces)
        start, base = 0, 0
        while start < n:
            stop = int(np.searchsorted(cum, base + target, side="right"))
            stop = max(stop, start + 1)
            if int(cum[stop - 1]) - base > limit and stop - 1 > start:
                stop -= 1
            yield start, stop
            base = int(cum[stop - 1])
            start = stop

    def _to_device(self, t: Tensor) -> Tensor:
        return t.pin_memory().to(self.device, non_blocking=True)

    _active = 0
    _active_lock = threading.Lock()
    pool_first = False

    def _small_call_enters(self) -> bool:
        with _TextTowerBase._active_lock:
            self._active += 1
            return self._active == 1

    def _small_call_leaves(self) -> None:
        with _TextTowerBase._active_lock:
            self._active -= 1

    def _queue(self, normalize: bool, clip: bool) -> Optional["NQ.TextQueue"]:
        if not NQ.ENABLED or self._queues_off or self.pool_first or (self._fp8 is not None and not self._fp8.calibrated):
            return None
        return self._cached_queue(normalize, self._make_queue, "text", clip)

    def _make_queue(self, idx: int, normalize: bool, clip: bool) -> "NQ.TextQueue":
        max_len = (self.arch.ctx + (1 if getattr(self.arch, "cls_embed", False) else 0)) if clip else self.arch.max_pos
        return NQ.TextQueue(self.lib, L.QUEUE_CLIP_TEXT if clip else L.QUEUE_BERT, self.cfg, self.w, idx,
                            self.arch.out_dim if clip else self.out_width, max_len, bool(normalize))

    def _small_call(self, ids_h: np.ndarray, lengths: np.ndarray, normalize: bool, clip: bool) -> Optional[Tensor]:
        n = int(lengths.size)
        if not getattr(_request_tls, "host_output", False) or n < 1 or n > NQ.MAX_SEQS:
            return None
        alone = self._small_call_enters()
        try:
            if n == 1 and alone and self._graphs_ok():
                one = self._encode_one(torch.from_numpy(ids_h[0, :int(lengths[0])]), normalize, clip)
                if one is not None:
                    return one
            q = self._queue(normalize, clip)
            if q is None or not q.takes(n, int(lengths.sum())):
                return None
            packed, _ = _pack(ids_h, lengths)
            rows = self._through_queue(q, q.encode, packed.numpy(), lengths)
            return None if rows is None else torch.from_numpy(rows)
        finally:
            self._small_call_leaves()

    def queue_rows(self, ids_h: np.ndarray, lengths: np.ndarray, normalize: bool, clip: bool) -> Optional[np.ndarray]:
        n = int(lengths.size)
        if n < 1 or n > NQ.MAX_SEQS:
            return None
        alone = self._small_call_enters()
        try:
            if n == 1 and alone and not NQ.GRAPHS and self._graphs_ok():
# ... 585 lines not shown
```

Measured before the change: 95170 embeddings/s.

## Fuse u8 patchify and normalization into patch-embedding GEMM with HWC weights

Adds a patch-embedding GEMM kernel that loads uint8 HWC pixels straight from the image, applies mean/std normalization in registers, converts to bf16 and writes to LDS. This replaces the separate patchify kernel and its bf16 patches buffer. To make the K dimension match the pixel order, the patch weights are permuted once to HWC layout and cached. The change removes one kernel launch and a round trip of the patch matrix through HBM, at the cost of a custom kernel with a more complex load schedule.

```diff
diff --git a/include/marqo_hip.h b/include/marqo_hip.h
--- a/include/marqo_hip.h
+++ b/include/marqo_hip.h
@@ -184,6 +184,14 @@
 int mq_encode_image_f32(const mq_vit_cfg* cfg, const mq_vit_weights* w,
                         const float* d_pixels, int64_t n, float* d_out, int normalize,
                         void* d_workspace, size_t workspace_bytes, void* stream);
+
+int mq_encode_image_u8_hwc(const mq_vit_cfg* cfg, const mq_vit_weights* w, const void* d_patch_w_hwc,
+                           const uint8_t* d_pixels, int64_t n, float* d_out, int normalize,
+                           void* d_workspace, size_t workspace_bytes, void* stream);
+
+int mq_patch_gemm_u8(const void* d_in, int64_t n, int32_t S, int32_t P, const float* mean, const float* std, const void* d_W, float* d_out,
+                     int64_t ldc, int64_t N, void* stream);
+int mq_patch_gemm_u8_ok(const void* d_in, int64_t n, int32_t S, int32_t P, int64_t N, const float* mean, const float* std);
 
 int mq_encode_clip_text(const mq_clip_text_cfg* cfg, const mq_clip_text_weights* w,
                         const int32_t* d_ids, const int32_t* d_cu_seqlens,
diff --git a/marqo_amd/_lib.py b/marqo_amd/_lib.py
--- a/marqo_amd/_lib.py
+++ b/marqo_amd/_lib.py
@@ -21,7 +21,7 @@
 STAGE_PATH = LIB_DIR / "_mq_stage.so"
 
 MQ_OK = 0
-NO_SCRATCH_UNITS = ("rowops", "gemm_bf16", "gemm_wd", "gemm_fp8", "gemm_small", "attention", "attention_window", "attention_gqa", "attention_gqa256", "attention_gqa256_causal", "attention_relbias", "attention_alibi", "attention_disentangled", "attention_full", "lora", "attn_proj", "panel_gemm", "embed", "convnext", "resnet", "patch_attn", "rerank", "owl_head", "temporal", "audio", "video")
+NO_SCRATCH_UNITS = ("rowops", "gemm_bf16", "gemm_wd", "gemm_fp8", "gemm_small", "patch_gemm_u8", "attention", "attention_window", "attention_gqa", "attention_gqa256", "attention_gqa256_causal", "attention_relbias", "attention_alibi", "attention_disentangled", "attention_full", "lora", "attn_proj", "panel_gemm", "embed", "convnext", "resnet", "patch_attn", "rerank", "owl_head", "temporal", "audio", "video")
 ABI_VERSION = 15
 MQ_PREC_BF16, MQ_PREC_FP8 = 0, 1
 MQ_ACT_GELU, MQ_ACT_QUICKGELU, MQ_ACT_SILU, MQ_ACT_RELU = 1, 2, 3, 4
@@ -334,6 +334,9 @@
     "mq_bert_workspace_bytes": (C.c_size_t, [C.POINTER(BertCfg), C.c_int64, C.c_int64]),
     "mq_encode_image_u8": (C.c_int, [C.POINTER(VitCfg), C.POINTER(VitWeights), _P, C.c_int64, _P, C.c_int, _P, C.c_size_t, _P]),
     "mq_encode_image_f32": (C.c_int, [C.POINTER(VitCfg), C.POINTER(VitWeights), _P, C.c_int64, _P, C.c_int, _P, C.c_size_t, _P]),
+    "mq_encode_image_u8_hwc": (C.c_int, [C.POINTER(VitCfg), C.POINTER(VitWeights), _P, _P, C.c_int64, _P, C.c_int, _P, C.c_size_t, _P]),
+    "mq_patch_gemm_u8": (C.c_int, [_P, C.c_int64, C.c_int32, C.c_int32, _P, _P, _P, _P, C.c_int64, C.c_int64, _P]),
+    "mq_patch_gemm_u8_ok": (C.c_int, [_P, C.c_int64, C.c_int32, C.c_int32, C.c_int64, _P, _P]),
     "mq_encode_clip_text": (C.c_int, [C.POINTER(ClipTextCfg), C.POINTER(ClipTextWeights), _P, _P, _P, C.c_int64, _P, _P,
                                       C.c_int, _P, C.c_size_t, _P]),
     "mq_encode_bert": (C.c_int, [C.POINTER(BertCfg), C.POINTER(BertWeights), _P, _P, _P, C.c_int64, _P, C.c_int, _P,
diff --git a/marqo_amd/csrc/knobs.h b/marqo_amd/csrc/knobs.h
--- a/marqo_amd/csrc/knobs.h
+++ b/marqo_amd/csrc/knobs.h
@@ -9,7 +9,7 @@
 extern std::atomic<uint64_t> mq_gemm_addr_limit;
 
 extern mq_knob mq_tower_row_select, mq_tower_ln_fold, mq_tower_subln_fold, mq_tower_attn_proj, mq_tower_panel_gemm, mq_tower_residual_bf16,
-    mq_tower_pool_strided, mq_tower_assemble_stats;
+    mq_tower_pool_strided, mq_tower_assemble_stats, mq_tower_patch_u8;
 extern mq_knob mq_gemm_small_max_rows, mq_gemm_small_group_rows;
 extern mq_knob mq_ln_prefetch, mq_ln_rows_per_wave, mq_ln_bf16_wide;
 extern mq_knob mq_xcd_band;
diff --git a/marqo_amd/csrc/knobs.hip b/marqo_amd/csrc/knobs.hip
--- a/marqo_amd/csrc/knobs.hip
+++ b/marqo_amd/csrc/knobs.hip
@@ -6,7 +6,7 @@
 GemmTune g_tune;
 std::atomic<uint64_t> mq_gemm_addr_limit{0xffffffffull};
 mq_knob mq_tower_row_select, mq_tower_ln_fold, mq_tower_subln_fold, mq_tower_attn_proj, mq_tower_panel_gemm, mq_tower_residual_bf16,
-    mq_tower_pool_strided, mq_tower_assemble_stats;
+    mq_tower_pool_strided, mq_tower_assemble_stats, mq_tower_patch_u8;
 mq_knob mq_gemm_small_max_rows, mq_gemm_small_group_rows;
 mq_knob mq_ln_prefetch, mq_ln_rows_per_wave, mq_ln_bf16_wide;
 mq_knob mq_xcd_band;
@@ -31,6 +31,7 @@
     {"residual_bf16", "MQ_RESIDUAL_BF16", 0, &mq_tower_residual_bf16},
     {"pool_strided", "MQ_POOL_STRIDED", 1, &mq_tower_pool_strided},
     {"assemble_stats", "MQ_ASSEMBLE_STATS", 1, &mq_tower_assemble_stats},
+    {"patch_u8", "MQ_PATCH_U8", 1, &mq_tower_patch_u8},
     {"small_m", "MQ_SMALL_M", 80, &mq_gemm_small_max_rows},
     {"small_m_grouped", "MQ_SMALL_M_GROUPED", 320, &mq_gemm_small_group_rows},
     {"ln_prefetch", "MQ_LN_PREFETCH", 1, &mq_ln_prefetch},
diff --git a/marqo_amd/csrc/patch_gemm_u8.hip b/marqo_amd/csrc/patch_gemm_u8.hip
--- /dev/null
+++ b/marqo_amd/csrc/patch_gemm_u8.hip
@@ -0,0 +1,428 @@
+#include <math.h>
+#include <string.h>
+#include <mutex>
+#include "common.h"
+#include "gemm_epilogue.h"
+#include "gemm_loop.h"
+#include "gemm_sched.h"
+
+int mq_device_ok();
+bool mq_gemm_small_ok(int64_t M, int64_t N, int64_t K, bool ln);
+bool mq_gemm_small_grouped_ok(int64_t M, int64_t N, int64_t K);
+
+namespace {
+
+struct PatchNorm { float a[3], b[3]; };
+
+__device__ __forceinline__ void gload_u8x16(i32x4& v, i32x4 rs, unsigned voff) {
+    asm volatile("buffer_load_dwordx4 %0, %1, %2, 0 offen" : "+v"(v) : "v"(voff), "s"(rs));
+}
+
+constexpr bool side_is_vm(int it, int nvm, int nside) { return ((it + 1) * nvm) / nside > (it * nvm) / nside; }
+constexpr bool side_order_ok(int nau, int npw, int nlr) {
+    const int nvm = npw + nau, nside = nvm + 2 * nau + nlr;
+    int last_write = -1, first_load = nside;
+    for (int it = 0; it < nside; ++it) {
+        const int vm_before = (it * nvm) / nside;
+        if (side_is_vm(it, nvm, nside)) { if (vm_before >= npw && it < first_load) first_load = it; }
+        else if (it - vm_before < 2 * nau) last_write = it;
+    }
+    return last_write < first_load;
+}
+template <int OFF>
+__device__ __forceinline__ void lds_write16(unsigned addr, i32x4 v) {
+    asm volatile("ds_write_b128 %0, %1 offset:%2" ::"v"(addr), "v"(v), "n"(OFF) : "memory");
+}
+
+template <int H>
+__device__ __forceinline__ i32x4 norm8(const i32x4& px, const float (&c)[3], const float (&d)[3]) {
+    i32x4 o;
+#pragma unroll
+    for (int p = 0; p < 4; ++p) {
+        const int e0 = 8 * H + 2 * p, e1 = e0 + 1;
+        const unsigned w = (unsigned)px[e0 >> 2];
+        const float f0 = __builtin_fmaf((float)((w >> (8 * (e0 & 3))) & 0xffu), c[e0 % 3], d[e0 % 3]);
+        const float f1 = __builtin_fmaf((float)((w >> (8 * (e1 & 3))) & 0xffu), c[e1 % 3], d[e1 % 3]);
+        o[p] = (int)pack_bf16x2(f0, f1);
+    }
+    return o;
+}
+
+template <int MT>
+__global__ __launch_bounds__(256, 2) void patch_gemm_u8_kernel(
+    const uint8_t* __restrict__ img, const bf16_t* __restrict__ Wt, float* out, int64_t ldc,
+    int M, int N, int K, int S, int P, int G, int tiles_n, int num_tiles, int cgroup, int band_rows,
+    unsigned a_bytes, unsigned w_bytes, PatchNorm nrm) {
+    constexpr int BM = 32 * MT, BN = 128;
+    constexpr int NTW = 4;
+    constexpr int A_TILE_BYTES = BM * BK * 2, W_TILE_BYTES = BN * BK * 2;
+    constexpr int STAGE_BYTES = A_TILE_BYTES + W_TILE_BYTES;
+    constexpr int NPW = 4;
+    constexpr int NAU = (MT + 1) / 2;
+    constexpr bool ODD = (MT & 1) != 0;
+    constexpr int NLR = MT + NTW;
+    constexpr int NM = NTW * MT;
+    extern __shared__ __attribute__((aligned(16))) char smem[];
+
+    const GemmTileMap<BM, BN> tile_map(num_tiles, tiles_n, M, cgroup, band_rows);
+
+    const int tid = threadIdx.x;
+    const int lane = tid & 63;
+    const int wave = __builtin_amdgcn_readfirstlane(tid >> 6);
+    const int wm = wave >> 1, wn = wave & 1;
+    const int l15 = lane & 15, g = lane >> 4;
+
+    const int srow = lane >> 3;
+    const unsigned chunk_off = (unsigned)(((lane & 7) ^ (srow & 7)) * 16);
+    unsigned w_vo[NPW];
+    auto set_w_sources = [&](int n0) {
+#pragma unroll
+        for (int i = 0; i < NPW; ++i) {
+            int gn = n0 + wave * (8 * NPW) + i * 8 + srow; gn = gn < N ? gn : N - 1;
+            w_vo[i] = (unsigned)gn * (unsigned)K * 2u + chunk_off;
+        }
+    };
+    const int q = lane & 3;
+    const int R = 3 * P, pitch = 3 * S;
+    const bool last_unit_ok = !ODD || lane < 32;
+    unsigned a_vo[NAU];
+    auto set_a_sources = [&](int m0) {
+        const int GG = G * G;
+#pragma unroll
+        for (int j = 0; j < NAU; ++j) {
+            int gm = m0 + wave * (8 * MT) + j * 16 + (lane >> 2);
+            if (ODD && j == NAU - 1 && !last_unit_ok) gm = m0;
+            gm = gm < M ? gm : M - 1;
+            const int im = gm / GG, pidx = gm - im * GG;
+            const int py = pidx / G, px = pidx - py * G;
+            a_vo[j] = ((unsigned)(im * S + py * P) * (unsigned)S + (unsigned)(px * P)) * 3u;
+        }
+    };
+    const int nk = K / BK;
+    int w_vbid = blockIdx.x, w_k = 0;
+    int a_vbid = blockIdx.x, a_k = 0;
+    unsigned a_rec = a_bytes, w_rec = w_bytes;
+    unsigned a_x = (unsigned)(16 * q), a_y = 0;
+    auto norm_a_xy = [&]() {
+        if (a_x >= (unsigned)R) { a_x -= (unsigned)R; a_y += (unsigned)pitch; }
+        if (a_x >= (unsigned)R) { a_x -= (unsigned)R; a_y += (unsigned)pitch; }
+    };
+    norm_a_xy();
+    {
+        int m0, n0;
+        tile_map.origin(w_vbid, m0, n0);
+        set_w_sources(n0);
+        set_a_sources(m0);
+    }
+    const unsigned lds0 = (unsigned)(uintptr_t)(__attribute__((address_space(3))) char*)smem;
+    const unsigned dma_w0 = lds0 + A_TILE_BYTES + (unsigned)wave * (8 * NPW * 128);
+    const unsigned i_lo = (unsigned)(uintptr_t)img, i_hi = (unsigned)((uintptr_t)img >> 32) & 0xffffu;
+    auto issue_w_piece = [&](int i, unsigned bufoff) {
+        dma16(__builtin_amdgcn_make_buffer_rsrc((void*)Wt, 0, w_rec, 0x00020000), w_vo[i], (unsigned)w_k * (BK * 2), dma_w0 + bufoff + (unsigned)i * 1024u);
+    };
+    auto advance_w = [&]() {
+        if (++w_k == nk) {
+            w_k = 0;
+            w_vbid += gridDim.x;
+            if (w_vbid < num_tiles) {
+                int m0, n0;
+                tile_map.origin(w_vbid, m0, n0);
+                set_w_sources(n0);
+            } else w_rec = 0;
+        }
+    };
+    auto load_a = [&](int j, i32x4& dst) {
+        const i32x4 rs = {(int)i_lo, (int)i_hi, (int)a_rec, 0x00020000};
+        gload_u8x16(dst, rs, a_vo[j] + a_y + a_x);
+    };
+    auto advance_a = [&]() {
+        a_x += 64u;
+        norm_a_xy();
+        if (++a_k == nk) {
+            a_k = 0;
+            a_x = (unsigned)(16 * q); a_y = 0;
+            norm_a_xy();
+            a_vbid += gridDim.x;
+            if (a_vbid < num_tiles) {
+                int m0, n0;
+                tile_map.origin(a_vbid, m0, n0);
+                set_a_sources(m0);
+            } else a_rec = 0;
+        }
+    };
+    unsigned a_wr[NAU];
+#pragma unroll
+    for (int j = 0; j < NAU; ++j) {
+        const int r = wave * (8 * MT) + j * 16 + (lane >> 2);
+        a_wr[j] = lds0 + (unsigned)(r * 128 + (((2 * q) ^ (r & 7)) << 4));
+    }
+    float nc[3], nd[3];
+    {
+        const int ph = q % 3;
+#pragma unroll
+        for (int i = 0; i < 3; ++i) {
+            const int c = (ph + i) % 3;
+            nc[i] = c == 0 ? nrm.a[0] : c == 1 ? nrm.a[1] : nrm.a[2];
+            nd[i] = c == 0 ? nrm.b[0] : c == 1 ? nrm.b[1] : nrm.b[2];
+        }
+    }
+    auto rotate_norm = [&]() {
+        const float c0 = nc[0], d0 = nd[0];
+        nc[0] = nc[1]; nc[1] = nc[2]; nc[2] = c0;
+        nd[0] = nd[1]; nd[1] = nd[2]; nd[2] = d0;
+    };
+    auto write_a_half = [&](auto j_tag, auto h_tag, const i32x4 (&px)[NAU], unsigned bufoff) {
+        constexpr int J = decltype(j_tag)::value, H = decltype(h_tag)::value;
+        const i32x4 v = norm8<H>(px[J], nc, nd);
+        const unsigned addr = (H == 0 ? a_wr[J] : (a_wr[J] ^ 16u)) + bufoff;
+        if constexpr (ODD && J == NAU - 1) {
+            if (last_unit_ok) lds_write16<0>(addr, v);
+        } else lds_write16<0>(addr, v);
+    };
+
+    const unsigned sw0 = (unsigned)((g ^ (l15 & 7)) << 4), sw1 = (unsigned)(((g + 4) ^ (l15 & 7)) << 4);
+    const unsigned a_row = lds0 + (unsigned)((wm * (16 * MT) + l15) * 128);
+    const unsigned w_row = lds0 + A_TILE_BYTES + (unsigned)((wn * (16 * NTW) + l15) * 128);
+    const unsigned aB0 = a_row + sw0, aB1 = a_row + sw1, wB0 = w_row + sw0, wB1 = w_row + sw1;
+
+    f32x4 acc[1][MT][4];
+    bf16x8 wf0[NTW], af0[MT], wf1[NTW], af1[MT];
+    auto read_piece = [&](auto p_tag, unsigned wbase, unsigned abase, bf16x8 (&wf)[NTW], bf16x8 (&af)[MT]) {
+        constexpr int Pc = decltype(p_tag)::value;
+        if constexpr (Pc < NTW) wf[Pc] = lds_read16<Pc * 2048>(wbase);
+        else af[Pc - NTW] = lds_read16<(Pc - NTW) * 2048>(abase);
+    };
+
+    unsigned bufoff = 0;
+    i32x4 areg[NAU];
+    {
+        i32x4 p0[NAU], p1[NAU];
+#pragma unroll
+        for (int j = 0; j < NAU; ++j) { p0[j] = i32x4{0, 0, 0, 0}; p1[j] = i32x4{0, 0, 0, 0}; areg[j] = i32x4{0, 0, 0, 0}; }
+#pragma unroll
+        for (int j = 0; j < NAU; ++j) load_a(j, p0[j]);
+        advance_a();
+#pragma unroll
+        for (int j = 0; j < NAU; ++j) load_a(j, p1[j]);
+        advance_a();
+#pragma unroll
+        for (int j = 0; j < NAU; ++j) load_a(j, areg[j]);
+        advance_a();
+#pragma unroll
+        for (int i = 0; i < NPW; ++i) issue_w_piece(i, 0);
+        advance_w();
+#pragma unroll
+        for (int i = 0; i < NPW; ++i) issue_w_piece(i, STAGE_BYTES);
+        advance_w();
+        asm volatile("s_waitcnt vmcnt(0)" ::: "memory");
+#pragma unroll
+        for (int j = 0; j < NAU; ++j) { landed(p0[j]); landed(p1[j]); landed(areg[j]); }
+        static_for<2 * NAU>([&](auto t) {
+            write_a_half(std::integral_constant<int, decltype(t)::value / 2>{}, std::integral_constant<int, decltype(t)::value % 2>{}, p0, 0u);
+        });
+        rotate_norm();
+        static_for<2 * NAU>([&](auto t) {
+            write_a_half(std::integral_constant<int, decltype(t)::value / 2>{}, std::integral_constant<int, decltype(t)::value % 2>{}, p1, (unsigned)STAGE_BYTES);
+        });
+        rotate_norm();
+        asm volatile("s_waitcnt lgkmcnt(0)" ::: "memory");
+        __builtin_amdgcn_s_barrier();
+        asm volatile("" ::: "memory");
+        static_for<NLR>([&](auto p_tag) { read_piece(p_tag, wB0, aB0, wf0, af0); });
+    }
+
+    int c_vbid = blockIdx.x;
+
+    auto kstep = [&]() {
+        asm volatile("s_waitcnt lgkmcnt(0)" ::: "memory");
+#pragma unroll
+        for (int t = 0; t < NTW; ++t) landed(wf0[t]);
+#pragma unroll
+        for (int t = 0; t < MT; ++t) landed(af0[t]);
+        __builtin_amdgcn_sched_barrier(0);
+        {
+            const unsigned wb = wB1 + bufoff, ab = aB1 + bufoff;
+            static_for<NM>([&](auto idx_tag) {
+                constexpr int idx = decltype(idx_tag)::value, mt = idx / NTW, nt = idx % NTW;
+                acc[0][mt][nt] = __builtin_amdgcn_mfma_f32_16x16x32_bf16(wf0[nt], af0[mt], acc[0][mt][nt], 0, 0, 0);
+                constexpr int RG = NM / NLR > 0 ? NM / NLR : 1;
+                constexpr int lo = idx == 0 ? 0 : (idx / RG < NLR ? idx / RG : NLR);
+                constexpr int hi = idx == NM - 1 ? NLR : ((idx + 1) / RG < NLR ? (idx + 1) / RG : NLR);
+                static_for<hi - lo>([&](auto p_tag) {
+                    constexpr int it = lo + decltype(p_tag)::value;
+                    __builtin_amdgcn_sched_barrier(0);
+                    read_piece(std::integral_constant<int, it>{}, wb, ab, wf1, af1);
+                    __builtin_amdgcn_sched_barrier(0);
+                });
+            });
+        }
+        __builtin_amdgcn_sched_barrier(0);
+        __builtin_amdgcn_s_waitcnt(0x0F70);
+        asm volatile("s_waitcnt vmcnt(0) lgkmcnt(0)" ::: "memory");
+#pragma unroll
+        for (int t = 0; t < NTW; ++t) landed(wf1[t]);
+#pragma unroll
+        for (int t = 0; t < MT; ++t) landed(af1[t]);
+#pragma unroll
+        for (int j = 0; j < NAU; ++j) landed(areg[j]);
+        __builtin_amdgcn_s_barrier();
+        asm volatile("" ::: "memory");
+        __builtin_amdgcn_sched_barrier(0);
+        static_assert(side_order_ok(NAU, NPW, NLR), "a pixel load in front of a write pass of the same registers");
+        {
+            const unsigned nb = bufoff ^ (unsigned)STAGE_BYTES;
+            const unsigned wb = wB0 + nb, ab = aB0 + nb;
+            constexpr int NVM = NPW + NAU, NLDS = 2 * NAU + NLR, NSIDE = NVM + NLDS;
+            static_for<NM>([&](auto idx_tag) {
+                constexpr int idx = decltype(idx_tag)::value, mt = idx / NTW, nt = idx % NTW;
+                acc[0][mt][nt] = __builtin_amdgcn_mfma_f32_16x16x32_bf16(wf1[nt], af1[mt], acc[0][mt][nt], 0, 0, 0);
+                constexpr int lo = idx == 0 ? 0 : (idx * NSIDE) / NM;
+                constexpr int hi = idx == NM - 1 ? NSIDE : ((idx + 1) * NSIDE) / NM;
+                static_for<hi - lo>([&](auto it_tag) {
+                    constexpr int it = lo + decltype(it_tag)::value;
+                    __builtin_amdgcn_sched_barrier(0);
+                    constexpr int vm_before = (it * NVM) / NSIDE;
+                    constexpr bool is_vm = side_is_vm(it, NVM, NSIDE);
+                    constexpr int ord = is_vm ? vm_before : it - vm_before;
+                    if constexpr (is_vm) {
+                        if constexpr (ord < NPW) issue_w_piece(ord, bufoff);
+                        else load_a(ord - NPW, areg[ord - NPW]);
+                    } else {
+                        if constexpr (ord < 2 * NAU) write_a_half(std::integral_constant<int, ord / 2>{}, std::integral_constant<int, ord % 2>{}, areg, bufoff);
+                        else read_piece(std::integral_constant<int, ord - 2 * NAU>{}, wb, ab, wf0, af0);
+                    }
+                    __builtin_amdgcn_sched_barrier(0);
+                });
+            });
+        }
+        rotate_norm();
+        advance_w();
+        advance_a();
+        bufoff ^= (unsigned)STAGE_BYTES;
+    };
+
+    for (;;) {
+        int cm0, cn0;
+        tile_map.origin(c_vbid, cm0, cn0);
+#pragma unroll
+        for (int i = 0; i < MT; ++i)
+#pragma unroll
+            for (int j = 0; j < 4; ++j) acc[0][i][j] = f32x4{0.f, 0.f, 0.f, 0.f};
+        for (int kt = 0; kt < nk; ++kt) kstep();
+        asm volatile("s_waitcnt vmcnt(0) lgkmcnt(0)" ::: "memory");
+#pragma unroll
+        for (int t = 0; t < NTW; ++t) landed(wf0[t]);
+#pragma unroll
+        for (int t = 0; t < MT; ++t) landed(af0[t]);
+#pragma unroll
+        for (int j = 0; j < NAU; ++j) landed(areg[j]);
+
+        GemmLn ln{};
+        gemm_epilogue<MQ_EPI_OUT_F32, MT, MT, true>(acc[0], nullptr, nullptr, out, ldc, M, N, cm0 + wm * (16 * MT), cn0 + wn * (16 * NTW), l15, g, false, &ln, nullptr);
+
+        c_vbid += gridDim.x;
+        if (c_vbid >= num_tiles) break;
+    }
+    asm volatile("s_waitcnt vmcnt(0) lgkmcnt(0)" ::: "memory");
+}
+
+
+uint16_t host_bf16(float f) {
+    uint32_t u;
+    memcpy(&u, &f, 4);
+    u += 0x7fffu + ((u >> 16) & 1u);
+    return (uint16_t)(u >> 16);
+}
+
+bool patch_norm(const float* mean, const float* std, PatchNorm& out) {
+    static std::mutex mu;
+    static float last[6];
+    static PatchNorm last_nrm;
+    static int last_ok = -1;
+    std::lock_guard<std::mutex> lock(mu);
+    if (last_ok >= 0 && !memcmp(last, mean, 12) && !memcmp(last + 3, std, 12)) { out = last_nrm; return last_ok != 0; }
+    bool ok = true;
+    PatchNorm nrm;
+    for (int c = 0; c < 3 && ok; ++c) {
+        const float m = mean[c], s = std[c];
+        if (!(s != 0.f) || !isfinite(m) || !isfinite(s)) { ok = false; break; }
+        nrm.a[c] = (float)(1.0 / (255.0 * (double)s));
+        nrm.b[c] = (float)(-(double)m / (double)s);
+        for (int t = 0; t < 256; ++t) {
+            volatile float x = (float)t / 255.0f;
+            volatile float y = x - m;
+            volatile float want = y / s;
+            const float got = fmaf((float)t, nrm.a[c], nrm.b[c]);
+            if (!isfinite(want) || host_bf16(want) != host_bf16(got)) { ok = false; break; }
+        }
+    }
+    memcpy(last, mean, 12);
+    memcpy(last + 3, std, 12);
+    last_nrm = nrm;
+    last_ok = ok ? 1 : 0;
+    out = nrm;
+    return ok;
+}
+
+bool layout_ok(const void* d_in, int64_t n, int S, int P, int64_t N) {
+    if (n < 1 || P < 8 || S < P || N < 4 || N % 4) return false;
+    if ((3 * P) % 16 || (3 * P * P) % 64 || (3 * S) % 16 || ((uintptr_t)d_in & 15)) return false;
+    const int G = S / P;
+    const uint64_t bytes = (uint64_t)n * S * S * 3, rows = (uint64_t)n * G * G;
+    return bytes <= 0xffffffffull && rows < (1ull << 30) && N < (1 << 30) && (uint64_t)N * 3 * P * P * 2 <= 0xffffffffull;
+}
+
+template <int MT>
+int launch_patch(const uint8_t* d_in, const void* W, float* out, int64_t ldc, int M, int N, int K, int S, int P, int G, unsigned a_bytes,
+                 const PatchNorm& nrm, hipStream_t s) {
+    constexpr int BM = 32 * MT, BN = 128;
+    constexpr int LDS = 2 * (BM + BN) * BK * 2;
+    static std::atomic<uint64_t> attr_done{0};
+    auto kern = patch_gemm_u8_kernel<MT>;
+    if (hipError_t e = mq_ensure_dyn_lds((const void*)kern, LDS, attr_done); e != hipSuccess) {
+        mq_set_error("mq_patch_gemm_u8: hipFuncSetAttribute: %s", hipGetErrorString(e));
+        return MQ_ERR_HIP;
+    }
+    GemmGeom g;
+    g.tiles_n = (N + BN - 1) / BN;
+    g.set_tiles_m((M + BM - 1) / BM, RESIDENT_SLOTS);
+    g.a_bytes = a_bytes;
+    g.w_bytes = (unsigned)((uint64_t)N * K * 2);
+    hipLaunchKernelGGL(kern, dim3(g.grid), dim3(256), LDS, s, d_in, (const bf16_t*)W, out, ldc, M, N, K, S, P, G, g.tiles_n, g.num_tiles, g.cgroup,
+                       g.band_rows, g.a_bytes, g.w_bytes, nrm);
+    MQ_CHECK_LAUNCH("mq_patch_gemm_u8");
+    return MQ_OK;
+}
+
+}
+
+extern "C" int mq_patch_gemm_u8_ok(const void* d_in, int64_t n, int32_t S, int32_t P, int64_t N, const float* mean, const float* std) {
+    if (!mean || !std || !layout_ok(d_in, n, S, P, N)) return 0;
+    const int G = S / P;
+    const int64_t M = n * G * G, K = 3 * P * P;
+    if (mq_gemm_small_ok(M, N, K, false) || mq_gemm_small_grouped_ok(M, N, K)) return 0;
+    PatchNorm nrm;
+    return patch_norm(mean, std, nrm) ? 1 : 0;
+}
+
+extern "C" int mq_patch_gemm_u8(const void* d_in, int64_t n, int32_t S, int32_t P, const float* mean, const float* std, const void* d_W, float* d_out,
+                                int64_t ldc, int64_t N, void* stream) {
+    MQ_CHECK_ARG(d_in && d_W && d_out && mean && std, "mq_patch_gemm_u8: null pointer");
+    MQ_CHECK_ARG(layout_ok(d_in, n, S, P, N), "mq_patch_gemm_u8: n=%ld S=%d P=%d N=%ld unsupported (3 P and 3 S multiples of 16, 3 P^2 of 64, 16-byte aligned pixels, "
+                 "under 4 GiB of them)", (long)n, S, P, (long)N);
+    MQ_CHECK_ARG(ldc >= N && ldc % 4 == 0 && ((uintptr_t)d_out & 15) == 0, "mq_patch_gemm_u8: ldc=%ld must be a multiple of 4, at least N, the output 16-byte aligned", (long)ldc);
+    PatchNorm nrm;
+    MQ_CHECK_ARG(patch_norm(mean, std, nrm), "mq_patch_gemm_u8: one fma per pixel does not reproduce (b / 255 - mean) / std in bf16 for these constants");
+    MQ_TRY(mq_device_ok());
+    const hipStream_t s = (hipStream_t)stream;
+    const int G = S / P, M = (int)(n * G * G), K = 3 * P * P;
+    MqProfScope prof(0, s, 2.0 * (double)M * (double)N * (double)K);
+    const unsigned a_bytes = (unsigned)((uint64_t)n * S * S * 3);
+    const int knob_mt = g_tune.mt;
+    switch (knob_mt ? knob_mt : choose_mt(M, (int)N)) {
+        case 2: return launch_patch<2>((const uint8_t*)d_in, d_W, d_out, ldc, M, (int)N, K, S, P, G, a_bytes, nrm, s);
+        case 5: return launch_patch<5>((const uint8_t*)d_in, d_W, d_out, ldc, M, (int)N, K, S, P, G, a_bytes, nrm, s);
+        case 6: return launch_patch<6>((const uint8_t*)d_in, d_W, d_out, ldc, M, (int)N, K, S, P, G, a_bytes, nrm, s);
+        default: return launch_patch<4>((const uint8_t*)d_in, d_W, d_out, ldc, M, (int)N, K, S, P, G, a_bytes, nrm, s);
+    }
+}
diff --git a/marqo_amd/csrc/torch_ops.cpp b/marqo_amd/csrc/torch_ops.cpp
--- a/marqo_amd/csrc/torch_ops.cpp
+++ b/marqo_amd/csrc/torch_ops.cpp
@@ -49,6 +49,22 @@
     check_rc(mq_encode_image_u8(blob<mq_vit_cfg>(cfg, "mq_vit_cfg"), blob<mq_vit_weights>(weights, "mq_vit_weights"),
                                 (const uint8_t*)pixels.data_ptr(), pixels.size(0), (float*)out.data_ptr(), normalize ? 1 : 0,
                                 workspace.data_ptr(), (size_t)workspace.numel(), stream_of(pixels)), "encode_image_u8");
+}
+
+void encode_image_u8_hwc(const at::Tensor& cfg, const at::Tensor& weights, const at::Tensor& patch_w_hwc, const at::Tensor& pixels, at::Tensor out,
+                         bool normalize, at::Tensor workspace) {
+    need_dev(pixels, at::kByte, "pixels");
+    need_dev(patch_w_hwc, at::kBFloat16, "patch_w_hwc");
+    need_dev(out, at::kFloat, "out");
+    need_dev(workspace, at::kByte, "workspace");
+    TORCH_CHECK(pixels.dim() == 4 && out.dim() == 2 && out.size(0) == pixels.size(0), "marqo_hip::encode_image_u8_hwc: pixels [n,S,S,3], out [n,D]");
+    const mq_vit_cfg* c = blob<mq_vit_cfg>(cfg, "mq_vit_cfg");
+    TORCH_CHECK(patch_w_hwc.device() == pixels.device() && patch_w_hwc.numel() == (int64_t)c->enc.width * 3 * c->patch_size * c->patch_size,
+                "marqo_hip::encode_image_u8_hwc: patch_w_hwc must be bf16 [W, 3 P^2] on the pixels' device");
+    NoGil nogil;
+    check_rc(mq_encode_image_u8_hwc(c, blob<mq_vit_weights>(weights, "mq_vit_weights"), patch_w_hwc.data_ptr(), (const uint8_t*)pixels.data_ptr(),
+                                    pixels.size(0), (float*)out.data_ptr(), normalize ? 1 : 0, workspace.data_ptr(), (size_t)workspace.numel(),
+                                    stream_of(pixels)), "encode_image_u8_hwc");
 }
 
 void encode_image_f32(const at::Tensor& cfg, const at::Tensor& weights, const at::Tensor& pixels, at::Tensor out, bool normalize,
@@ -279,6 +295,7 @@
 
 TORCH_LIBRARY(marqo_hip, m) {
     m.def("encode_image_u8(Tensor cfg, Tensor weights, Tensor pixels, Tensor(a!) out, bool normalize, Tensor(b!) workspace) -> ()");
+    m.def("encode_image_u8_hwc(Tensor cfg, Tensor weights, Tensor patch_w_hwc, Tensor pixels, Tensor(a!) out, bool normalize, Tensor(b!) workspace) -> ()");
     m.def("encode_image_f32(Tensor cfg, Tensor weights, Tensor pixels, Tensor(a!) out, bool normalize, Tensor(b!) workspace) -> ()");
     m.def("encode_clip_text(Tensor cfg, Tensor weights, Tensor ids, Tensor cu_seqlens, Tensor cu_seqlens_host, Tensor? pool_rows, "
           "Tensor(a!) out, bool normalize, Tensor(b!) workspace) -> ()");
@@ -304,6 +321,7 @@
 
 TORCH_LIBRARY_IMPL(marqo_hip, CUDA, m) {
     m.impl("encode_image_u8", &encode_image_u8);
+    m.impl("encode_image_u8_hwc", &encode_image_u8_hwc);
     m.impl("encode_image_f32", &encode_image_f32);
     m.impl("encode_clip_text", &encode_clip_text);
     m.impl("encode_bert", &encode_bert);
diff --git a/marqo_amd/csrc/towers.hip b/marqo_amd/csrc/towers.hip
--- a/marqo_amd/csrc/towers.hip
+++ b/marqo_amd/csrc/towers.hip
@@ -620,7 +620,7 @@
 }
 
 int encode_image_impl(const mq_vit_cfg* cfg, const mq_vit_weights* w, const void* d_pixels, bool is_u8, int64_t n,
-                      float* d_out, int normalize, void* ws, size_t ws_bytes, hipStream_t s) {
+                      float* d_out, int normalize, void* ws, size_t ws_bytes, hipStream_t s, const void* patch_w_hwc = nullptr) {
     MQ_CHECK_ARG(cfg && w && d_out, "mq_encode_image: null pointer");
     MQ_TRY(check_encoder_cfg(&cfg->enc));
     MQ_CHECK_ARG(cfg->patch_size > 0 && cfg->image_size >= cfg->patch_size, "mq_encode_image: image %d smaller than patch %d",
@@ -661,8 +661,13 @@
     void* patches = base + p.off_patches;
     float* patch_out = (float*)(base + p.off_patch_out);
 
-    MQ_TRY(mq_patchify(d_pixels, is_u8, patches, n, cfg->image_size, cfg->patch_size, p.Kp, cfg->mean, cfg->std, s));
-    MQ_TRY(mq_gemm_bf16(patches, p.Kp, w->patch_w, p.Kp, nullptr, nullptr, patch_out, W, n * p.np, W, p.Kp, MQ_EPI_OUT_F32, s));
+    if (is_u8 && patch_w_hwc && mq_tower_patch_u8 && p.Kp == 3 * cfg->patch_size * cfg->patch_size &&
+        mq_patch_gemm_u8_ok(d_pixels, n, cfg->image_size, cfg->patch_size, W, cfg->mean, cfg->std)) {
+        MQ_TRY(mq_patch_gemm_u8(d_pixels, n, cfg->image_size, cfg->patch_size, cfg->mean, cfg->std, patch_w_hwc, patch_out, W, W, s));
+    } else {
+        MQ_TRY(mq_patchify(d_pixels, is_u8, patches, n, cfg->image_size, cfg->patch_size, p.Kp, cfg->mean, cfg->std, s));
+        MQ_TRY(mq_gemm_bf16(patches, p.Kp, w->patch_w, p.Kp, nullptr, nullptr, patch_out, W, n * p.np, W, p.Kp, MQ_EPI_OUT_F32, s));
+    }
     const int xb = stream_bf16(&cfg->enc) ? 1 : 0;
     const float* stats0 = nullptr;
     if (mq_tower_assemble_stats && xb && w->ln_pre_g && cfg->pool == MQ_VIT_POOL_CLS && cfg->enc.precision == MQ_PREC_BF16 && !cfg->enc.post_ln &&
@@ -760,6 +765,11 @@
     return encode_image_impl(cfg, w, d_pixels, true, n, d_out, normalize, d_workspace, workspace_bytes, (hipStream_t)stream);
 }
 
+extern "C" int mq_encode_image_u8_hwc(const mq_vit_cfg* cfg, const mq_vit_weights* w, const void* d_patch_w_hwc, const uint8_t* d_pixels, int64_t n,
+                                      float* d_out, int normalize, void* d_workspace, size_t workspace_bytes, void* stream) {
+    return encode_image_impl(cfg, w, d_pixels, true, n, d_out, normalize, d_workspace, workspace_bytes, (hipStream_t)stream, d_patch_w_hwc);
+}
+
 extern "C" int mq_encode_image_f32(const mq_vit_cfg* cfg, const mq_vit_weights* w, const float* d_pixels, int64_t n,
                                    float* d_out, int normalize, void* d_workspace, size_t workspace_bytes, void* stream) {
     return encode_image_impl(cfg, w, d_pixels, false, n, d_out, normalize, d_workspace, workspace_bytes, (hipStream_t)stream);
diff --git a/marqo_amd/engine/towers.py b/marqo_amd/engine/towers.py
--- a/marqo_amd/engine/towers.py
+++ b/marqo_amd/engine/towers.py
@@ -467,9 +467,17 @@
         return self._blobs
 
     def _call_image(self, kind: str, pixels: Tensor, n: int, out: Tensor, normalize: bool, ws: Tensor) -> None:
+        hwc = self._patch_w_hwc() if kind == "u8" else None
         if self._ops is not None:
             cfg, w = self._desc()
-            (self._ops.encode_image_u8 if kind == "u8" else self._ops.encode_image_f32)(cfg, w, pixels, out, bool(normalize), ws)
+            if hwc is not None:
+                self._ops.encode_image_u8_hwc(cfg, w, hwc, pixels, out, bool(normalize), ws)
+            else:
+                (self._ops.encode_image_u8 if kind == "u8" else self._ops.encode_image_f32)(cfg, w, pixels, out, bool(normalize), ws)
+            return
+        if hwc is not None:
+            L.check(self.lib.mq_encode_image_u8_hwc(C.byref(self.cfg), C.byref(self.w), hwc.data_ptr(), pixels.data_ptr(), n, out.data_ptr(),
+                                                    1 if normalize else 0, ws.data_ptr(), ws.numel(), self._stream()), "mq_encode_image")
             return
         fn = self.lib.mq_encode_image_u8 if kind == "u8" else self.lib.mq_encode_image_f32
         L.check(fn(C.byref(self.cfg), C.byref(self.w), pixels.data_ptr(), n, out.data_ptr(), 1 if normalize else 0, ws.data_ptr(),
@@ -492,6 +500,9 @@
             L.check(self.lib.mq_encode_bert(C.byref(self.cfg), C.byref(self.w), d_packed.data_ptr(), d_cu.data_ptr(), cu.data_ptr(), nseq,
                                             out.data_ptr(), 1 if normalize else 0, ws.data_ptr(), ws.numel(), self._stream()),
                     "mq_encode_bert")
+
+    def _patch_w_hwc(self) -> Optional[Tensor]:
+        return None
 
     def _graphs_ok(self) -> bool:
         return GRAPHS and not self._graphs_off and (self._fp8 is None or self._fp8.calibrated)
@@ -667,6 +678,23 @@
         u8 = self.calibration_images()
         return lambda: self.encode_u8(u8)
 
+    _hwc: Optional[Tensor] = None
+
+    def _patch_w_hwc(self) -> Optional[Tensor]:
+        P, W = self.arch.patch_size, self.arch.width
+        if (3 * P) % 16 or (3 * P * P) % 64:
+            return None
+        if self._hwc is None:
+            with self._lock:
+                if self._hwc is None:
+                    src = next(t for t in self._h.tensors if t.data_ptr() == self.w.patch_w)
+                    with torch.cuda.device(self.device):
+                        hwc = src.view(W, 3, P, P).permute(0, 2, 3, 1).contiguous().view(W, 3 * P * P)
+                        torch.cuda.current_stream(self.device).synchronize()
+                    self._h.tensors.append(hwc)
+                    self._hwc = hwc
+        return self._hwc
+
     def _image_workspace_bytes(self, m: int) -> int:
         return self.lib.mq_vit_workspace_bytes(C.byref(self.cfg), m)
 
@@ -675,6 +703,8 @@
 
     def _run(self, kind: str, pixels: Tensor, normalize: bool) -> Tensor:
         n = pixels.shape[0]
+        if kind == "u8":
+            self._patch_w_hwc()
         if n == 1 and self._graphs_ok():
             with self._lock, torch.cuda.device(self.device):
                 def make():
```

New measurement: 95120 embeddings/s (median of 2 runs). Within noise of the previous version (-0.1%).
